# bioinfologics/w2rap-contigger

Measured on AMD Instinct MI355X. Metric: step2_k60_canonical_kmers_per_s, higher is better.
Workload: dtype u64

## Files before the change

### w2rap_contigger_amd/csrc/ctx.h

```cpp
#pragma once
#include <hip/hip_runtime.h>
#include <stdint.h>
#include <stdio.h>
#include <stdlib.h>
#include <cstdlib>
#include <string>
#include <utility>
#include <vector>
#include "../../include/w2rap_step2.h"
#include "common.h"

namespace w2 {

struct Ctx;
}
struct w2rap_step2_ctx;
namespace w2 {
struct Ctx {
    int device = 0;
    hipStream_t stream = nullptr;
    hipStream_t stream2 = nullptr;
    unsigned long long* h_pinned = nullptr;
    std::string err;
    int sm_count = 256;

    uint64_t n = 0;
    const uint8_t* d_bases = nullptr;
    const uint64_t* d_boff = nullptr;
    const uint32_t* d_len = nullptr;
    const uint8_t* d_quals = nullptr;
    const uint64_t* d_qoff = nullptr;
    uint32_t max_len = 0;
    std::vector<void*> owned_reads;

    uint16_t* d_good = nullptr;
    uint32_t min_qual = 7, min_freq = 4;

    uint64_t M = 0, D = 0, S = 0;
    uint64_t hist[101] = {0};
    uint32_t NB = 0;
    uint32_t* d_bcount = nullptr;
    unsigned long long part_kmers[64] = {0};
    uint64_t* d_bbase = nullptr;
    uint32_t* d_recs = nullptr;
    uint64_t nrec = 0;
    uint64_t solid_cap = 0;
    uint64_t* d_shi = nullptr;
    uint64_t* d_slo = nullptr;
    uint32_t* d_scc = nullptr;
    Slot* d_table = nullptr;
    uint64_t tcap = 0;
    unsigned long long* d_filter32 = nullptr;
    uint64_t f32words = 0;
    uint8_t* d_sctx = nullptr;
    void* d_nbr = nullptr;
    bool wide_ids = false;
    uint64_t* d_chunk_start = nullptr;
    uint32_t* d_chunk_cnt = nullptr;
    uint64_t nchunks = 0;
    KRec* d_srec = nullptr;
    bool use_index = false;
    uint4* d_index = nullptr;
    uint64_t index_cap = 0, index_entries = 0;
    uint4* d_xindex = nullptr; uint64_t xindex_cap = 0, xindex_kmers = 0;
    bool index_prebuilt = false, bits_ready = false, filter_prebuilt = false;
    unsigned cs_ns = 0;
    unsigned cs_planned = 0;
    uint32_t cs_nbl = 0, cs_nseg = 0; const uint32_t* cs_recs = nullptr;
    bool cs_short_first = false;
    hipEvent_t cs_ev[16] = {};
    unsigned long long* cs_cnt = nullptr;
    uint64_t* cs_off = nullptr;
    uint32_t cs_chunk_cap = 0;
    uint8_t* d_unres = nullptr;
    bool fused_prune = false;
    std::vector<std::pair<uint64_t, uint64_t>> unfused_chunks;
    uint32_t* cs_defer = nullptr;
    uint64_t* g_hi = nullptr; uint64_t* g_lo = nullptr; uint32_t* g_cc = nullptr;
    uint64_t* g_cstart = nullptr; uint32_t* g_ccnt = nullptr;
    uint64_t g_cap = 0, g_n = 0, g_ccap = 0, g_nc = 0;
    bool g_open = false;
    hipEvent_t g_copied = nullptr;
    bool quality_done = false, counted = false, graphed = false, pathed_done = false;
    bool table_built = false;

    uint64_t E = 0;
    uint64_t rank_ends = 0;
    uint32_t* d_edge_nk = nullptr;
    uint64_t* d_edge_off = nullptr;
    uint8_t* d_edge_codes = nullptr;
    uint8_t* d_edge_bits = nullptr;
    uint64_t edge_bases = 0;
    uint64_t NO = 0, NV = 0;
    int32_t* d_fwdX = nullptr;
    int32_t* d_revX = nullptr;
    uint32_t* d_obj_edge = nullptr;
    ObjRec* d_otab = nullptr;
    int32_t* d_left = nullptr;
    int32_t* d_right = nullptr;
    uint64_t* d_from_off = nullptr;
    int32_t* d_from_v = nullptr;
    int32_t* d_from_e = nullptr;
    uint64_t* d_to_off = nullptr;
    int32_t* d_to_v = nullptr;
    int32_t* d_to_e = nullptr;
    int32_t* d_path_offset = nullptr;
    uint64_t* d_path_off = nullptr;
    int32_t* d_path_edges = nullptr;
    uint64_t path_total = 0;
    uint64_t n_pathed = 0, n_multipathed = 0;
    float ms_count = 0, ms_graph = 0, ms_path = 0;

    uint64_t ld_done = 0;
    void* shard = nullptr;
    std::vector<void*> owned;
    void* pump = nullptr;
    const uint32_t* d_qmask = nullptr;
    int qmask_min_qual = -1;
    int hint_min_qual = -1;
    bool hint_graph_only = false;
    bool quals_absent = false;
    uint8_t* d_qring = nullptr;
    void* pump2 = nullptr;
    hipStream_t copy_stream = nullptr;
    void* quals_job = nullptr;
    void* mask_job = nullptr; void* h_mask = nullptr; size_t h_mask_bytes = 0;
    uint32_t n_passes = 0;
    unsigned pass = 0, npass = 1;
    unsigned long long* pass_cnt = nullptr;

    struct ProfEv { const char* name; hipEvent_t a, b; };
    struct ProfSum { std::string name; double ms = 0; uint64_t launches = 0; };
    std::vector<ProfEv> prof_pending;
    std::vector<ProfSum> prof_sums;
    bool profiling = true;
    void pbegin(const char* name, hipStream_t st = nullptr) {
        if (!profiling) return;
        ProfEv e{name, nullptr, nullptr};
        (void)hipEventCreate(&e.a); (void)hipEventCreate(&e.b);
        (void)hipEventRecord(e.a, st ? st : stream);
        prof_pending.push_back(e);
    }
    void pend(hipStream_t st = nullptr) {
        if (!profiling || prof_pending.empty()) return;
        (void)hipEventRecord(prof_pending.back().b, st ? st : stream);
    }
    void presolve() {
        for (auto& e : prof_pending) {
            float ms = 0;
            if (hipEventElapsedTime(&ms, e.a, e.b) == hipSuccess) {
                ProfSum* s = nullptr;
                for (auto& x : prof_sums) if (x.name == e.name) { s = &x; break; }
                if (!s) { prof_sums.push_back(ProfSum{e.name, 0, 0}); s = &prof_sums.back(); }
                s->ms += ms; s->launches += 1;
            }
            (void)hipEventDestroy(e.a); (void)hipEventDestroy(e.b);
        }
        prof_pending.clear();
    }

    std::vector<std::pair<size_t, void*>> parked;
    std::vector<std::pair<void*, size_t>> sizes;
    int mem_trace = -1; uint64_t traced_peak = 0;
    uint64_t live_bytes = 0, peak_bytes = 0;
    static size_t size_class(size_t bytes) {
        size_t g = 256;
        if (bytes < (256u << 20)) { while ((g << 5) <= bytes) g <<= 1; }
        else { g = 1u << 20; while ((g << 8) <= bytes) g <<= 1; }
        return (bytes + g - 1) & ~(g - 1);
    }
    void trim() {
        for (auto& b : parked) (void)hipFree(b.second);
        parked.clear();
    }
    template <class T>
    T* alloc(size_t count, bool track = true) {
        void* p = nullptr;
        size_t bytes = (count ? count : 1) * sizeof(T);
        bytes = size_class(bytes);
        for (size_t i = 0; i < parked.size(); ++i)
            if (parked[i].first == bytes) { p = parked[i].second; parked[i] = parked.back(); parked.pop_back(); break; }
        if (!p) {
            hipError_t e = hipMalloc(&p, bytes);
            if (e != hipSuccess) { (void)hipGetLastError(); trim(); e = hipMalloc(&p, bytes); }
            if (e != hipSuccess) { (void)hipGetLastError(); if (w2rap_step2_trim_cached() > 0) { (void)hipSetDevice(device); e = hipMalloc(&p, bytes); } }
            if (e != hipSuccess) {
                err = std::string("hipMalloc(") + std::to_string(bytes) + " B): " + hipGetErrorString(e);
                return nullptr;
            }
        }
        sizes.emplace_back(p, bytes);
        live_bytes += bytes;
        if (live_bytes > peak_bytes) {
            peak_bytes = live_bytes;
            if (mem_trace < 0) mem_trace = getenv("W2RAP_TRACE_MEM") ? 1 : 0;
            if (mem_trace && live_bytes > traced_peak + (1ull << 30)) {
                traced_peak = live_bytes;
                std::string l;
                for (auto& x : sizes) if (x.second >= (64u << 20)) l += " " + std::to_string(x.second >> 20);
                fprintf(stderr, "[w2rap] device memory: new peak %.2f GB live; blocks (MiB):%s\n", live_bytes / 1e9, l.c_str());
            }
        }
        if (track) owned.push_back(p);
        return (T*)p;
    }
    void park(void* p) {
        for (size_t i = 0; i < sizes.size(); ++i)
            if (sizes[i].first == p) { live_bytes -= sizes[i].second; parked.emplace_back(sizes[i].second, p); sizes[i] = sizes.back(); sizes.pop_back(); return; }
        (void)hipFree(p);
    }
    void release(void* p) {
        if (!p) return;
        for (size_t i = 0; i < owned.size(); ++i)
            if (owned[i] == p) { owned[i] = owned.back(); owned.pop_back(); break; }
        park(p);
    }
    void free_all() {
        for (void* p : owned) park(p);
        owned.clear();
    }

    struct Kept3 {
        bool valid = false;
        unsigned K2 = 0; uint64_t E = 0, NV = 0, n = 0, path_ints = 0, edge_bytes = 0;
        uint8_t* ebits = nullptr;
        uint64_t* ebyte = nullptr; uint32_t* elen = nullptr;
        int32_t* left = nullptr; int32_t* right = nullptr;
        uint64_t* from_off = nullptr; int32_t* from_v = nullptr; int32_t* from_e = nullptr;
        uint64_t* to_off = nullptr; int32_t* to_v = nullptr; int32_t* to_e = nullptr;
        int32_t* inv2 = nullptr;
        int32_t* p_offset = nullptr; uint64_t* p_off = nullptr; int32_t* p_edges = nullptr;
        std::vector<void*> blocks() const {
            return {ebits, ebyte, elen, left, right, from_off, from_v, from_e, to_off, to_v, to_e, inv2, p_offset, p_off, p_edges};
        }
    };
    Kept3 kept;
    void drop_kept() {
        if (!kept.valid) return;
        for (void* p : kept.blocks()) release(p);
        kept = Kept3{};
    }
};

inline bool test_hook(const char* name) {
    if (!getenv(name)) return false;
    fprintf(stderr, "[w2rap] WARNING: test hook %s is set -- this is not a production configuration\n", name);
    return true;
}

#define W2_HIP(call)                                                                         \
    do {                                                                                     \
        hipError_t e__ = (call);                                                             \
        if (e__ != hipSuccess) {                                                             \
            c.err = std::string(#call) + ": " + hipGetErrorString(e__) + " (" + __FILE__ + ":" + \
                    std::to_string(__LINE__) + ")";                                          \
            return W2RAP_E_HIP;                                                              \
        }                                                                                    \
    } while (0)
#define W2_ALLOC(ptr, T, count)                          \
    do {                                                 \
        ptr = c.alloc<T>(count);                         \
        if (!ptr) return W2RAP_E_HIP;                    \
    } while (0)
#define W2_TRY(expr)                   \
    do {                               \
        int rc__ = (expr);             \
        if (rc__) return rc__;         \
    } while (0)

#define LAUNCH(c, name, kern, grid, block, lds, ...)                          \
    do {                                                                      \
        (c).pbegin(name);                                                     \
        hipLaunchKernelGGL(kern, grid, block, lds, (c).stream, __VA_ARGS__);  \
        (c).pend();                                                           \
    } while (0)

struct Timer {
    hipEvent_t a = nullptr, b = nullptr; hipStream_t st;
    explicit Timer(hipStream_t s) : st(s) { (void)hipEventCreate(&a); (void)hipEventCreate(&b); (void)hipEventRecord(a, st); }
    float stop() { float ms = 0; (void)hipEventRecord(b, st); (void)hipEventSynchronize(b); (void)hipEventElapsedTime(&ms, a, b); return ms; }
    ~Timer() { (void)hipEventDestroy(a); (void)hipEventDestroy(b); }
    Timer(const Timer&) = delete; Timer& operator=(const Timer&) = delete;
};
void* host_result_alloc(size_t bytes);
template <class T>
inline int dl(Ctx& c, T** host, const T* dev, uint64_t n) {
    *host = (T*)host_result_alloc((n ? n : 1) * sizeof(T));
    if (!*host) { c.err = "out of host memory"; return W2RAP_E_HIP; }
    if (n * sizeof(T) >= (8u << 20)) return pump_download(c, *host, dev, n * sizeof(T));
    if (n) W2_HIP(hipMemcpyAsync(*host, dev, n * sizeof(T), hipMemcpyDeviceToHost, c.stream));
    return 0;
}
template <class T>
inline int up_pooled(Ctx& c, T** dev, const T* host, uint64_t n, uint64_t pad = 0) {
    T* p = c.alloc<T>(n + pad + 1);
    if (!p) return W2RAP_E_HIP;
    W2_HIP(hipMemsetAsync(p + n, 0, (pad + 1) * sizeof(T), c.stream));
    if (n && !host) { c.err = "null host array"; return W2RAP_E_ARG; }
    if (host) { if (n) W2_HIP(hipMemcpyAsync(p, host, n * sizeof(T), hipMemcpyHostToDevice, c.stream)); }
    else W2_HIP(hipMemsetAsync(p, 0, sizeof(T), c.stream));
    *dev = p;
    return 0;
}

#define LAUNCH_ON(c, st, name, kern, grid, block, lds, ...)                   \
    do {                                                                      \
        (c).pbegin(name, st);                                                 \
        hipLaunchKernelGGL(kern, grid, block, lds, st, __VA_ARGS__);          \
        (c).pend(st);                                                         \
    } while (0)

int device_copy_async(Ctx& c, void* dst, const void* src, uint64_t nbytes, hipStream_t st);
int pump_upload(Ctx& c, void* d, const void* h, size_t bytes);
int pump_download(Ctx& c, void* h, const void* d, size_t bytes);
void pump_free(Ctx& c);
int quality_mask_begin(Ctx& c, const uint8_t* h_quals, uint64_t nq, uint32_t min_qual);
int quality_mask_upload(Ctx& c, uint32_t* d_mask);
void quality_mask_cancel(Ctx& c);
int quals_upload_begin(Ctx& c, uint8_t* d_quals, const uint8_t* h_quals, uint64_t nq, uint64_t prefix_bytes, uint64_t prefix_reads);
int quals_wait_prefix(Ctx& c, uint64_t* reads_covered);
int quals_wait(Ctx& c);
}
#include <functional>
namespace w2 {
void host_parallel_for(size_t n, const std::function<void(size_t)>& f);

int phase_count(Ctx& c, uint32_t min_qual, uint32_t min_freq);
int count_quality(Ctx& c, uint32_t min_qual);
uint32_t default_buckets(uint64_t total_kmers, uint32_t multiple_of);
int count_partition(Ctx& c, uint32_t nb, uint32_t n_parts, uint32_t pb_lo, uint32_t pb_hi);
int count_buckets(Ctx& c, uint32_t min_freq, uint32_t nbl, uint32_t nseg, const uint32_t* d_recs, const uint32_t* d_counts, uint64_t total_kmers,
                  bool build_table = false);
int count_buckets_launch(Ctx& c, uint32_t min_freq, uint32_t nbl, uint32_t nseg, const uint32_t* d_recs, const uint32_t* d_counts, uint64_t total_kmers,
                         unsigned n_slices, bool deferred);
int count_buckets_launch_slice(Ctx& c, unsigned k);
void count_slice_bounds(const Ctx& c, unsigned k, uint32_t* b_lo, uint32_t* b_hi);
int count_buckets_slice(Ctx& c, unsigned k, uint64_t* n_solid, uint64_t* n_chunks);
int count_buckets_finish(Ctx& c);
int dict_begin(Ctx& c, uint64_t kmer_cap, uint64_t chunk_cap);
int dict_append(Ctx& c, const uint64_t* d_hi, const uint64_t* d_lo, const uint32_t* d_cc, uint64_t n, const uint64_t* d_cstart, const uint32_t* d_ccnt, uint64_t nc,
                uint64_t chunk_bias = 0);
int dict_end(Ctx& c);
void dict_abort(Ctx& c);
int count_table(Ctx& c);
int phase_graph(Ctx& c, const w2rap_edge_hint* hint);
int phase_path(Ctx& c);
int local_dict_slice(Ctx& c, uint64_t n_solid, uint64_t expected_total);
int shard_begin(Ctx& c, unsigned rank, unsigned world, const uint64_t* solid_per_rank, uint32_t n_buckets, uint32_t n_passes, const w2rap_edge_hint* hint);
int shard_next(Ctx& c, w2rap_xchg* x);
int shard_recv(Ctx& c, const uint64_t* recv_count, uint32_t elem_bytes, void** d_recv);
int shard_host_words(Ctx& c, const uint64_t* words);
int shard_info(Ctx& c, uint64_t out[8]);
void shard_free(Ctx& c);
int index_hard_slice(Ctx& c, const uint4* d_all, uint64_t n_all, unsigned rank, unsigned world, uint4** d_hard, uint64_t* n_hard);
int index_hard_apply(Ctx& c, const uint4* d_hard, uint64_t n_hard);
int index_harden(Ctx& c);
int build_index(Ctx& c);
int index_entries_slice(Ctx& c, unsigned rank, unsigned world, uint4** d_list, uint64_t* n_list);
int index_from_entries(Ctx& c, const uint4* d_all, uint64_t n_all, bool harden = true);
uint64_t filter32_words(const Ctx& c);
int filter32_slice(Ctx& c, unsigned rank, unsigned world, unsigned long long** d_slice, uint64_t* n_words);
EdgeIndex edge_index(const Ctx& c);
int index_probe_all(Ctx& c, int32_t* d_edge, uint32_t* d_off);
int run_ranking(Ctx& c, uint64_t N, const uint32_t* nxt0, uint32_t* nxt, uint32_t* rnk, unsigned long long* w, uint8_t* cyc, uint8_t* mid,
                uint32_t* d_flags, const uint64_t* shi, const uint64_t* slo, bool use_chunks);
int decode_pq(Ctx& c, const uint8_t* d_pq, const uint64_t* d_pqoff, uint8_t* d_quals, const uint64_t* d_qoff);

int sort_pairs_u64(Ctx& c, uint64_t* keys, uint32_t* vals, uint64_t n, int begin_bit, int end_bit);
int exclusive_scan_u32_to_u64(Ctx& c, const uint32_t* in, uint64_t* out, uint64_t n);
int exclusive_scan_packed_bytes(Ctx& c, const uint32_t* len, uint64_t* out, uint64_t n);
int exclusive_scan_u64(Ctx& c, const uint64_t* in, uint64_t* out, uint64_t n);
int exclusive_scan_is_self(Ctx& c, const uint32_t* a, uint64_t* out, uint64_t n);
int max_u32(Ctx& c, const uint32_t* in, uint64_t n, uint32_t* result);
int inclusive_max_scan_u32(Ctx& c, const uint32_t* in, uint32_t* out, uint64_t n);

}

struct w2rap_step2_ctx { w2::Ctx c; };
extern "C" w2rap_step2_ctx* w2rap_step2_acquire(int device, char* err, size_t errlen);
extern "C" void w2rap_step2_release(w2rap_step2_ctx*);
```

### w2rap_contigger_amd/csrc/step2_capi.hip

```cpp
#include <algorithm>
#include <chrono>
#include <cstdlib>
#include <cstring>
#include "ctx.h"

using namespace w2;


namespace {

void set_err(char* err, size_t errlen, const std::string& m) {
    if (err && errlen) { std::snprintf(err, errlen, "%s", m.c_str()); }
}


__global__ void __launch_bounds__(256) k_obj_len(uint64_t NO, const uint32_t* __restrict__ obj_edge, const uint32_t* __restrict__ edge_nk,
                                                  uint32_t* __restrict__ len, uint32_t* __restrict__ nbytes) {
    uint64_t o = (uint64_t)blockIdx.x * blockDim.x + threadIdx.x;
    if (o >= NO) return;
    uint32_t l = edge_nk[obj_edge[o] >> 1] + (K - 1);
    len[o] = l; nbytes[o] = (l + 3) >> 2;
}
__global__ void __launch_bounds__(256) k_pack_objs(uint64_t total_bytes, uint64_t NO, const uint64_t* __restrict__ byte_off,
                                                    const uint32_t* __restrict__ obj_edge, const uint32_t* __restrict__ edge_nk,
                                                    const uint64_t* __restrict__ edge_off, const uint8_t* __restrict__ codes,
                                                    uint8_t* __restrict__ out) {
    uint64_t i = (uint64_t)blockIdx.x * blockDim.x + threadIdx.x;
    if (i >= total_bytes) return;
    uint64_t lo = 0, hi = NO;
    while (hi - lo > 1) { uint64_t m = (lo + hi) >> 1; if (byte_off[m] <= i) lo = m; else hi = m; }
    uint32_t oe = obj_edge[lo], e = oe >> 1; bool rc = oe & 1;
    uint32_t len = edge_nk[e] + (K - 1);
    uint64_t eo = edge_off[e];
    uint32_t t0 = (uint32_t)(i - byte_off[lo]) * 4;
    unsigned v = 0;
    for (unsigned j = 0; j < 4; ++j) {
        uint32_t t = t0 + j;
        if (t < len) {
            unsigned b = rc ? 3u - codes[eo + (len - 1 - t)] : codes[eo + t];
            v |= b << (2 * j);
        }
    }
    out[i] = (uint8_t)v;
}


}
namespace w2 {
void drop_reads(Ctx& c) {
    (void)quals_wait(c);
    if (c.copy_stream) (void)hipStreamSynchronize(c.copy_stream);
    c.d_qmask = nullptr; c.qmask_min_qual = -1; c.quals_absent = false;
    for (void* p : c.owned_reads) c.park(p);
    c.owned_reads.clear();
    c.d_bases = nullptr; c.d_boff = nullptr; c.d_len = nullptr; c.d_quals = nullptr; c.d_qoff = nullptr; c.n = 0;
}
void drop_results(Ctx& c) {
    if (c.stream) (void)hipStreamSynchronize(c.stream);
    if (c.stream2) (void)hipStreamSynchronize(c.stream2);
    shard_free(c);
    c.drop_kept();
    c.free_all();
    c.d_good = nullptr; c.d_bcount = nullptr; c.d_bbase = nullptr; c.d_recs = nullptr; c.d_shi = c.d_slo = nullptr; c.d_scc = nullptr;
    c.d_table = nullptr; c.d_filter32 = nullptr; c.f32words = 0; c.d_sctx = nullptr; c.d_nbr = nullptr; c.d_srec = nullptr; c.d_index = nullptr; c.index_cap = 0; c.d_xindex = nullptr; c.xindex_cap = 0; c.d_unres = nullptr; c.fused_prune = false; c.unfused_chunks.clear();
    c.d_chunk_start = nullptr; c.d_chunk_cnt = nullptr; c.nchunks = 0;
    for (unsigned k = 0; k < c.cs_ns; ++k) (void)hipEventDestroy(c.cs_ev[k]);
    c.cs_ns = 0; c.cs_planned = 0; c.cs_cnt = nullptr; c.cs_off = nullptr; c.cs_defer = nullptr; c.pass = 0; c.npass = 1; c.pass_cnt = nullptr;
    c.g_hi = c.g_lo = nullptr; c.g_cc = nullptr; c.g_cstart = nullptr; c.g_ccnt = nullptr; c.g_open = false; c.g_n = c.g_nc = 0;
    c.d_edge_nk = nullptr; c.d_edge_off = nullptr; c.d_edge_codes = nullptr; c.d_edge_bits = nullptr; c.d_fwdX = c.d_revX = nullptr; c.d_obj_edge = nullptr;
    c.d_otab = nullptr; c.d_left = c.d_right = nullptr; c.d_from_off = c.d_to_off = nullptr; c.d_from_v = c.d_from_e = c.d_to_v = c.d_to_e = nullptr;
    c.d_path_offset = nullptr; c.d_path_off = nullptr; c.d_path_edges = nullptr;
    c.quality_done = c.counted = c.graphed = c.pathed_done = false; c.table_built = false;
    c.M = c.D = c.S = c.E = c.NO = c.NV = 0; c.path_total = 0; c.n_pathed = c.n_multipathed = 0;
}
}
namespace {

template <class T>
int up(Ctx& c, const T** dev, const T* host, uint64_t n, uint64_t pad = 0) {
    T* p = c.alloc<T>(n + pad + 1, false);
    if (!p) return W2RAP_E_HIP;
    c.owned_reads.push_back(p);
    W2_HIP(hipMemsetAsync(p + n, 0, (pad + 1) * sizeof(T), c.stream));
    if (n) W2_TRY(pump_upload(c, p, host, n * sizeof(T)));
    *dev = (const T*)p;
    return 0;
}

}

extern "C" {

int w2rap_step2_abi_version(void) { return W2RAP_STEP2_ABI_VERSION; }

int w2rap_step2_device_count(void) {
    int n = 0;
    if (hipGetDeviceCount(&n) != hipSuccess) return 0;
    return n;
}

w2rap_step2_ctx* w2rap_step2_create(int device, char* err, size_t errlen) {
    int n = 0;
    if (hipGetDeviceCount(&n) != hipSuccess || n <= 0) { set_err(err, errlen, "no HIP device (libw2rap_step2 has no CPU fallback)"); return nullptr; }
    if (device < 0 || device >= n) { set_err(err, errlen, "device ordinal out of range"); return nullptr; }
    hipDeviceProp_t prop;
    if (hipGetDeviceProperties(&prop, device) != hipSuccess) { set_err(err, errlen, "hipGetDeviceProperties failed"); return nullptr; }
    if (std::strncmp(prop.gcnArchName, "gfx950", 6) != 0) {
        set_err(err, errlen, std::string("device is ") + prop.gcnArchName + "; this library is built for gfx950 (MI355X) only");
        return nullptr;
    }
    if (hipSetDevice(device) != hipSuccess) { set_err(err, errlen, "hipSetDevice failed"); return nullptr; }
    auto* h = new w2rap_step2_ctx;
    h->c.device = device;
    h->c.sm_count = prop.multiProcessorCount;
    int prio_lo = 0, prio_hi = 0;
    (void)hipDeviceGetStreamPriorityRange(&prio_lo, &prio_hi);
    if (hipStreamCreateWithPriority(&h->c.stream, hipStreamNonBlocking, prio_hi) != hipSuccess ||
        hipStreamCreateWithPriority(&h->c.stream2, hipStreamNonBlocking, prio_lo) != hipSuccess ||
        hipHostMalloc((void**)&h->c.h_pinned, 64 * sizeof(unsigned long long), hipHostMallocDefault) != hipSuccess) {
        set_err(err, errlen, "hipStreamCreate / hipHostMalloc failed"); delete h; return nullptr;
    }
    return h;
}

void w2rap_step2_destroy(w2rap_step2_ctx* h) {
    if (!h) return;
    (void)hipSetDevice(h->c.device);
    (void)hipStreamSynchronize(h->c.stream);
    if (h->c.stream2) (void)hipStreamSynchronize(h->c.stream2);
    drop_results(h->c);
    drop_reads(h->c);
    h->c.trim();
    pump_free(h->c);
    (void)hipStreamDestroy(h->c.stream);
    if (h->c.g_copied) (void)hipEventDestroy(h->c.g_copied);
    if (h->c.stream2) (void)hipStreamDestroy(h->c.stream2);
    if (h->c.h_pinned) (void)hipHostFree(h->c.h_pinned);
    delete h;
}

const char* w2rap_step2_last_error(const w2rap_step2_ctx* h) { return h ? h->c.err.c_str() : "null context"; }
void* w2rap_step2_stream(w2rap_step2_ctx* h) { return h ? (void*)h->c.stream : nullptr; }

int w2rap_step2_set_reads(w2rap_step2_ctx* h, const w2rap_reads* r) {
    if (!h || !r) return W2RAP_E_ARG;
    Ctx& c = h->c;
    W2_HIP(hipSetDevice(c.device));
    drop_results(c);
    drop_reads(c);
    const uint64_t n = r->n_reads;
    if (n && (!r->bases_packed || !r->base_byte_off || !r->read_len)) { c.err = "set_reads: null base arrays"; return W2RAP_E_ARG; }
    const bool raw = r->quals && r->qual_off, pq = r->pq && r->pq_off;
    if (n && raw == pq) { c.err = "set_reads: give exactly one of (quals, qual_off) and (pq, pq_off)"; return W2RAP_E_ARG; }
    if (r->mem == W2RAP_MEM_DEVICE) {
        W2_HIP(hipDeviceSynchronize());
        c.d_bases = r->bases_packed; c.d_boff = r->base_byte_off; c.d_len = r->read_len;
        if (raw || !n) { c.d_quals = r->quals; c.d_qoff = r->qual_off; }
        else {
            uint64_t* qoff = nullptr; W2_HIP(hipMalloc((void**)&qoff, (n + 1) * 8)); c.owned_reads.push_back(qoff);
            W2_TRY(exclusive_scan_u32_to_u64(c, c.d_len, qoff, n));
            uint64_t total = 0;
            W2_HIP(hipMemcpy(&total, qoff + n, 8, hipMemcpyDeviceToHost));
            uint8_t* q = nullptr; W2_HIP(hipMalloc((void**)&q, total ? total : 1)); c.owned_reads.push_back(q);
            c.n = n;
            W2_TRY(decode_pq(c, r->pq, r->pq_off, q, qoff));
            c.d_quals = q; c.d_qoff = qoff;
        }
    } else if (r->mem == W2RAP_MEM_HOST) {
        {
            const size_t nblk = (size_t)std::min<uint64_t>(64, (n + 65535) / 65536);
            std::vector<uint64_t> bad(nblk ? nblk : 1, ~0ull); std::vector<int> why(nblk ? nblk : 1, 0);
            host_parallel_for(nblk, [&](size_t b) {
                const uint64_t lo = n * b / nblk, hi = n * (b + 1) / nblk;
                for (uint64_t i = lo; i < hi; ++i) {
                    const uint64_t nb = r->base_byte_off[i + 1] - r->base_byte_off[i];
                    int w = 0;
                    if (r->base_byte_off[i + 1] < r->base_byte_off[i] || nb != ((uint64_t)r->read_len[i] + 3) / 4) w = 1;
                    else if (raw && (r->qual_off[i + 1] < r->qual_off[i] || r->qual_off[i + 1] - r->qual_off[i] != r->read_len[i])) w = 2;
                    else if (!raw && r->pq_off[i + 1] <= r->pq_off[i]) w = 3;
                    else if (r->read_len[i] > 65535u) w = 4;
                    if (w) { bad[b] = i; why[b] = w; return; }
                }
            });
            for (size_t b = 0; b < nblk; ++b) if (bad[b] != ~0ull) {
                const std::string at = " (read " + std::to_string(bad[b]);
                if (why[b] == 4) { c.err = "a read of more than 65,535 bases" + at + "): good lengths are 16-bit words"; return W2RAP_E_LIMIT; }
                c.err = why[b] == 1 ? "set_reads: base_byte_off does not match read_len" + at + ")" : why[b] == 2 ? "set_reads: qual_off does not match read_len" + at + ")"
                                    : "set_reads: pq_off is not ascending" + at + "; every PQVec ends with a 0 byte)";
                return W2RAP_E_ARG;
            }
        }
        if (n && (r->base_byte_off[0] != 0 || (raw ? r->qual_off[0] : r->pq_off[0]) != 0)) { c.err = "set_reads: offsets must start at 0"; return W2RAP_E_ARG; }
        const uint64_t nbytes = n ? r->base_byte_off[n] : 0;
        auto derived = [&](const uint64_t** dev, bool packed) -> int {
            uint64_t* p = c.alloc<uint64_t>(n + 2, false);
            if (!p) return W2RAP_E_HIP;
            c.owned_reads.push_back(p);
            W2_TRY(packed ? exclusive_scan_packed_bytes(c, c.d_len, p, n) : exclusive_scan_u32_to_u64(c, c.d_len, p, n));
            *dev = p;
            return 0;
        };
        const uint64_t nq_raw = (raw && n) ? r->qual_off[n] : 0;
        const bool late_quals = raw && c.hint_min_qual >= 0 && nq_raw >= (64ull << 20) && !getenv("W2RAP_NO_UPLOAD_OVERLAP");
        if (late_quals) W2_TRY(quality_mask_begin(c, r->quals, nq_raw, (uint32_t)c.hint_min_qual));
        struct MaskGuard { Ctx& c; ~MaskGuard() { quality_mask_cancel(c); } } mask_guard{c};
        const bool tr = getenv("W2RAP_TRACE") != nullptr;
        auto tnow = [] { return std::chrono::duration<double, std::milli>(std::chrono::steady_clock::now().time_since_epoch()).count(); };
        const double t_a = tnow();
        W2_TRY(up(c, &c.d_len, r->read_len, n));
        W2_TRY(up(c, &c.d_bases, r->bases_packed, nbytes, 32));
        W2_TRY(derived(&c.d_boff, true));
        const double t_b = tnow();
        if (raw || !n) {
            const uint64_t nq = n ? r->qual_off[n] : 0;
            if (late_quals) {
                uint8_t* q = c.alloc<uint8_t>(nq + 33, false);
                uint32_t* m = c.alloc<uint32_t>((nq + 31) / 32 + 17, false);
                if (!q || !m) return W2RAP_E_HIP;
                c.owned_reads.push_back(q); c.owned_reads.push_back(m);
                W2_HIP(hipMemsetAsync(q + nq, 0, 33, c.stream));
// ... 608 lines not shown
```

### w2rap_contigger_amd/csrc/step2_count.hip

```cpp
#include <algorithm>
#include <chrono>
#include <cstdlib>
#include <cstring>
#include <type_traits>
#include "ctx.h"

namespace w2 {

constexpr unsigned QSLOTS = 256;
template <bool MASK>
__global__ void __launch_bounds__(256) k_good_len(uint64_t n, const uint8_t* __restrict__ quals, const uint32_t* __restrict__ qmask,
                                                   const uint64_t* __restrict__ qoff, const uint32_t* __restrict__ len,
                                                   uint32_t min_qual, uint16_t* __restrict__ good,
                                                   unsigned long long* __restrict__ total_kmers,
                                                   uint32_t* __restrict__ max_len) {
    constexpr unsigned CH = 4096;
    __shared__ __attribute__((aligned(16))) uint16_t gbits[CH + 16];
    __shared__ unsigned long long s_sum[4];
    __shared__ uint32_t s_max[4];
    const uint64_t r0 = (uint64_t)blockIdx.x * blockDim.x;
    const uint64_t r = r0 + threadIdx.x;
    const uint64_t rend = r0 + blockDim.x < n ? r0 + blockDim.x : n;
    const uint64_t base0 = qoff[r0], endo = qoff[rend];
    const unsigned shift = MASK ? (unsigned)(base0 & 31) : (unsigned)((reinterpret_cast<uintptr_t>(quals) + base0) & 15);
// ... 130 lines not shown
    __shared__ uint2 dbuf_[4][128];
    __shared__ uint32_t spart_[4][64];
    const unsigned lane = threadIdx.x & 63, wv_ = threadIdx.x >> 6;
    if (part_kmers) { spart_[wv_][lane] = 0; wave_lds_fence(); }
    uint2* dbuf = dbuf_[wv_];
    auto win_load = [&](uint64_t first_byte, unsigned nbytes) -> uint32_t {
        const uintptr_t a = reinterpret_cast<uintptr_t>(bases) + first_byte;
        const unsigned sb = (unsigned)(a & 3);
        return 4 * lane < sb + nbytes ? reinterpret_cast<const uint32_t*>(a & ~uintptr_t(3))[lane & 15u] : 0u;
    };
    const uint64_t stride = 1;
    uint64_t r = ((uint64_t)blockIdx.x * 4 + wv_) * chunk;
    const uint64_t r_end = r + chunk < n ? r + chunk : n;
    unsigned gl_c = 0, gl_n = 0; uint64_t off_c = 0, off_n = 0; uint32_t win_c = 0;
    if (r < r_end) { gl_c = good[r]; off_c = boff[r]; }
    if (r + stride < r_end) { gl_n = good[r + stride]; off_n = boff[r + stride]; }
    if (r < r_end && lane < 16 && gl_c > K) win_c = win_load(off_c, (gl_c + 3) >> 2);
    for (; r < r_end; r += stride) {
        const unsigned gl = gl_c;
        const uint64_t off_cur = off_c;
        const uint32_t win0 = win_c;
        unsigned gl_nn = 0; uint64_t off_nn = 0;
        if (r + 2 * stride < r_end) { gl_nn = good[r + 2 * stride]; off_nn = boff[r + 2 * stride]; }
        win_c = 0;
        if (r + stride < r_end && lane < 16 && gl_n > K) win_c = win_load(off_n, (gl_n + 3) >> 2);
        gl_c = gl_n; off_c = off_n; gl_n = gl_nn; off_n = off_nn;
        if (gl <= K) continue;
        const unsigned nk_total = gl - (K - 1);
        const unsigned nbytes_read = (gl + 3) >> 2;
        for (unsigned c0 = 0; c0 < nk_total; c0 += 128) {
            const unsigned first_base = c0 ? c0 - 1 : 0;
            const unsigned b0a = (first_base >> 2) & ~3u;
            uint32_t wdw = win0;
            if (c0) wdw = lane < 16 ? win_load(off_cur + b0a, nbytes_read - b0a) : 0u;
            const unsigned sbit = 8u * (unsigned)((reinterpret_cast<uintptr_t>(bases) + off_cur) & 3);
            const unsigned sbase = 4 * b0a;
            uint32_t k0, k1, k2;
            {
                uint32_t kk[3];
#pragma unroll
                for (int h = 0; h < 3; ++h) {
                    const unsigned j = c0 + h * 64 + lane;
                    uint32_t key = 0xFFFFFFFFu;
                    const bool has = j + MMER <= gl && (h < 2 || lane < WIN - 1);
                    const unsigned o = has ? sbit + 2 * (j - sbase) : 0u, wi = o >> 5, sh = o & 31;
                    const uint32_t w0 = (uint32_t)__builtin_amdgcn_ds_bpermute((int)(wi << 2), (int)wdw);
                    const uint32_t w1 = (uint32_t)__builtin_amdgcn_ds_bpermute((int)((wi + 1) << 2), (int)wdw);
                    if (has) {
                        const uint32_t f = __funnelshift_r(w0, w1, sh) & 0x3FFFFFFFu;
                        uint32_t rc = __brev(~f & 0x3FFFFFFFu);
                        rc = (((rc & 0x55555555u) << 1) | ((rc >> 1) & 0x55555555u)) >> 2;
                        key = mmer_key(f < rc ? f : rc);
                    }
                    kk[h] = key;
                }
                k0 = kk[0]; k1 = kk[1]; k2 = kk[2];
            }
            constexpr uint32_t INF = 0xFFFFFFFFu;
            auto row_pref = [](uint32_t x) {
                x = min(x, (uint32_t)__builtin_amdgcn_update_dpp((int)0xFFFFFFFFu, (int)x, 0x111, 0xF, 0xF, false));
                x = min(x, (uint32_t)__builtin_amdgcn_update_dpp((int)0xFFFFFFFFu, (int)x, 0x112, 0xF, 0xF, false));
                x = min(x, (uint32_t)__builtin_amdgcn_update_dpp((int)0xFFFFFFFFu, (int)x, 0x114, 0xF, 0xF, false));
                x = min(x, (uint32_t)__builtin_amdgcn_update_dpp((int)0xFFFFFFFFu, (int)x, 0x118, 0xF, 0xF, false));
                return x;
            };
            auto row_suff = [](uint32_t x) {
                x = min(x, (uint32_t)__builtin_amdgcn_update_dpp((int)0xFFFFFFFFu, (int)x, 0x101, 0xF, 0xF, false));
                x = min(x, (uint32_t)__builtin_amdgcn_update_dpp((int)0xFFFFFFFFu, (int)x, 0x102, 0xF, 0xF, false));
                x = min(x, (uint32_t)__builtin_amdgcn_update_dpp((int)0xFFFFFFFFu, (int)x, 0x104, 0xF, 0xF, false));
                x = min(x, (uint32_t)__builtin_amdgcn_update_dpp((int)0xFFFFFFFFu, (int)x, 0x108, 0xF, 0xF, false));
                return x;
            };
            const uint32_t P0 = row_pref(k0), P1 = row_pref(k1), P2 = row_pref(k2), S0 = row_suff(k0), S1 = row_suff(k1);
            uint32_t F[12];
#pragma unroll
            for (int R = 0; R < 4; ++R) {
                F[R] = (uint32_t)__builtin_amdgcn_readlane((int)P0, 16 * R + 15);
                F[4 + R] = (uint32_t)__builtin_amdgcn_readlane((int)P1, 16 * R + 15);
                F[8 + R] = (uint32_t)__builtin_amdgcn_readlane((int)P2, 16 * R + 15);
            }
            const unsigned rowi = lane >> 4;
            const bool two = (lane & 15u) >= 3;
            uint32_t mkh[2];
#pragma unroll
            for (int h = 0; h < 2; ++h) {
                const uint32_t g1a = F[4 * h + 1], g1b = F[4 * h + 2], g1c = F[4 * h + 3], g1d = F[4 * h + 4];
                const uint32_t g2a = min(g1a, F[4 * h + 2]), g2b = min(g1b, F[4 * h + 3]), g2c = min(g1c, F[4 * h + 4]), g2d = min(g1d, F[4 * h + 5]);
                const uint32_t one_row = rowi == 0 ? g1a : rowi == 1 ? g1b : rowi == 2 ? g1c : g1d;
                const uint32_t two_rows = rowi == 0 ? g2a : rowi == 1 ? g2b : rowi == 2 ? g2c : g2d;
                const uint32_t pend = h ? lane_shift(P1, P2, lane, WIN - 1) : lane_shift(P0, P1, lane, WIN - 1);
                mkh[h] = min(min(h ? S1 : S0, pend), two ? two_rows : one_row);
            }
            const uint32_t mk0 = mkh[0], mk1 = mkh[1];
            unsigned nkh[2] = {0, 0}; uint32_t bkh[2] = {0, 0}; bool sth[2] = {false, false};
#pragma unroll
            for (int h = 0; h < 2; ++h) {
                const unsigned cc0 = c0 + 64 * h;
                const unsigned p = cc0 + lane;
                const bool valid = p < nk_total;
                const uint32_t bkt = valid ? bucket_of(h ? mk1 : mk0, nb) : 0xFFFFFFFFu;
                const uint32_t prev = (uint32_t)__builtin_amdgcn_update_dpp(0, (int)bkt, 0x138, 0xF, 0xF, false);
                bool start = valid && (lane == 0 || prev != bkt);
                unsigned long long smask = __ballot(start);
                unsigned nvalid = cc0 < nk_total ? nk_total - cc0 : 0; if (nvalid > 64) nvalid = 64;
                if (REC_MAXK < 64 && smask == 1ull && nvalid == 64) { start |= lane == 63; smask |= 1ull << 63; }
                unsigned long long rest = lane < 63 ? (smask >> (lane + 1)) : 0ull;
                unsigned nxt = rest ? lane + 1 + __builtin_ctzll(rest) : nvalid;
                const bool mine = bkt - pb_lo < pb_hi - pb_lo;
                sth[h] = start && mine; bkh[h] = bkt - pb_lo; nkh[h] = start ? nxt - lane : 0;
            }
            unsigned cnt = 0;
            const uint64_t slot0 = (pass_off[r] + c0 / 128) * spp;
            uint32_t rk[2] = {0, 0};
#pragma unroll
            for (int h = 0; h < 2; ++h) {
                if (sth[h]) {
                    rk[h] = atomicAdd(&bcount[bkh[h]], 1u);
                    if (part_kmers) {
                        uint32_t pt = nbl_part > 1 ? __umulhi(bkh[h], inv_nbl) : bkh[h];
                        if ((pt + 1) * nbl_part <= bkh[h]) ++pt;
                        atomicAdd(&spart_[wv_][pt & 63], nkh[h]);
                    }
                }
            }
#pragma unroll
            for (int h = 0; h < 2; ++h) {
                const unsigned long long m = __ballot(sth[h]);
                if (sth[h]) {
                    const unsigned p = c0 + 64 * h + lane, nk = nkh[h];
                    const uint32_t meta = p | ((nk - 1) << 16) | (p > 0 ? 1u << 22 : 0u) | ((p + nk - 1) < (nk_total - 1) ? 1u << 23 : 0u);
                    const unsigned j = cnt + (unsigned)__builtin_popcountll(m & ((1ull << lane) - 1));
                    if (j < spp && rk[h] < 65536u) dbuf[j] = make_uint2(bkh[h] | (rk[h] << 24), meta | ((rk[h] >> 8) << 24));
                    else {
                        if (j < spp) dbuf[j] = make_uint2(0u, NONE32);
                        const unsigned long long o = atomicAdd(ov_cursor, 1ull);
                        if (o < ov_cap) { o_read[o] = (uint32_t)r; o_bkt[o] = bkh[h]; o_meta[o] = meta; o_rank[o] = rk[h]; }
                    }
                }
                cnt += (unsigned)__builtin_popcountll(m);
            }
            wave_lds_fence();
            for (unsigned i = lane; i < spp; i += 64) s_desc[slot0 + i] = i < cnt ? dbuf[i] : make_uint2(0u, NONE32);
            wave_lds_fence();
        }
    }
    if (part_kmers) {
        wave_lds_fence();
        const uint32_t v = spart_[wv_][lane];
        if (v) atomicAdd(&part_kmers[(blockIdx.x & 63u) * 64u + lane], (unsigned long long)v);
    }
}


template <unsigned SMAX, bool ALIGN64>
__global__ void __launch_bounds__(256, 4) k_superkmers_lane(uint64_t n, const uint8_t* __restrict__ bases, const uint64_t* __restrict__ boff,
                                                            const uint16_t* __restrict__ good, uint32_t nb, uint32_t pb_lo, uint32_t pb_hi,
                                                            uint32_t* __restrict__ bcount, uint32_t nbl_part, uint32_t inv_nbl,
                                                            unsigned long long* __restrict__ part_kmers, uint2* __restrict__ s_desc, uint32_t S,
                                                            uint32_t* __restrict__ o_read, uint32_t* __restrict__ o_bkt, uint32_t* __restrict__ o_meta,
                                                            uint32_t* __restrict__ o_rank, uint64_t ov_cap, unsigned long long* __restrict__ ov_cursor) {
    __shared__ uint2 stage_[4][64 * SMAX];
    __shared__ uint32_t spart_[4][64];
    const unsigned lane = threadIdx.x & 63, wv_ = threadIdx.x >> 6;
    const uint64_t r0 = ((uint64_t)blockIdx.x * 4 + wv_) * 64;
    if (r0 >= n) return;
    uint2* stage = stage_[wv_];
    if (part_kmers) spart_[wv_][lane] = 0;
    for (unsigned u = 0; u < S; ++u) stage[lane + 64 * u] = make_uint2(0u, NONE32);
    wave_lds_fence();
    constexpr uint32_t INF = 0xFFFFFFFFu;
    const uint64_t r = r0 + lane;
    unsigned gl = r < n ? good[r] : 0;
    if (gl <= K) gl = 0;
    const unsigned nk = gl ? gl - (K - 1) : 0;
    unsigned maxgl = gl;
#pragma unroll
    for (int d = 32; d; d >>= 1) maxgl = max(maxgl, (unsigned)__shfl_xor((int)maxgl, d));
    maxgl = (unsigned)__builtin_amdgcn_readfirstlane((int)maxgl);
    if (maxgl) {
        const uint64_t off = gl ? boff[r] : 0;
        const unsigned mis = (unsigned)((reinterpret_cast<uintptr_t>(bases) + off) & 3);
        const unsigned sb8 = 8u * mis;
        const uint32_t* q = reinterpret_cast<const uint32_t*>(bases + ((int64_t)off - (int64_t)mis));
        const unsigned ulast = gl ? (mis + ((gl + 3) >> 2) - 1) >> 2 : 0;
        uint32_t dA, dB, W; unsigned un = 3;
        { const uint32_t d0 = q[0]; dA = q[min(1u, ulast)]; dB = q[min(2u, ulast)]; W = __funnelshift_r(d0, dA, sb8); }
        uint32_t f = 0, rc = 0;
        auto roll = [&]() {
            const uint32_t b = W & 3u; W >>= 2;
            f = (f >> 2) | (b << 28);
            rc = ((rc << 2) & 0x3FFFFFFFu) | (b ^ 3u);
        };
#pragma unroll
        for (unsigned s = 0; s < MMER - 1; ++s) roll();
        uint32_t X3[16], X2[16], X1[16], C[16];
#pragma unroll
        for (int t = 0; t < 16; ++t) { X3[t] = INF; X2[t] = INF; X1[t] = INF; C[t] = INF; }
        uint32_t cur = 0;
        unsigned p0 = 0, jrec = 0;
        auto block = [&](auto first, unsigned jb) {
            constexpr int FIRST = decltype(first)::value;
            uint32_t pref = INF;
            const uint32_t w21 = min(X2[0], X1[0]);
            uint32_t bk[16];
#pragma unroll
            for (int i = 0; i < 16; ++i) {
                const unsigned s = jb + (MMER - 1) + i;
                if (i == 2) { W = __funnelshift_r(dA, dB, sb8); dA = dB; dB = q[min(un, ulast)]; ++un; }
                roll();
                const uint32_t key = s < gl ? mmer_key(f < rc ? f : rc) : INF;
                C[i] = key; pref = min(pref, key);
                bk[i] = 0;
                if (i >= FIRST) {
                    const uint32_t mk = i <= 12 ? min(min(X3[i <= 12 ? i + 3 : 0], w21), pref) : min(min(X2[i >= 13 ? i - 13 : 0], X1[0]), pref);
                    bk[i] = bucket_of(mk, nb);
                }
            }
#pragma unroll
            for (int i = FIRST; i < 16; ++i) {
                const unsigned p = jb + i - (WIN - 1);
                const bool isk = p < nk;
                const uint32_t bkt = bk[i];
                const bool brk = isk && (!p || bkt != cur || (ALIGN64 ? !(p & 63u) || (REC_MAXK < 64 && p - p0 == REC_MAXK) : p - p0 == REC_MAXK));
                if ((brk && p) || (p == nk && nk)) {
                    const uint32_t rb = cur - pb_lo;
                    if (rb < pb_hi - pb_lo) {
                        const uint32_t meta = p0 | ((p - p0 - 1) << 16) | (p0 ? 1u << 22 : 0u) | (isk ? 1u << 23 : 0u);
                        if (jrec < S) stage[lane * S + jrec] = make_uint2(rb, meta);
                        else {
                            const uint32_t rk = atomicAdd(&bcount[rb], 1u);
                            if (part_kmers) {
                                uint32_t pt = nbl_part > 1 ? __umulhi(rb, inv_nbl) : rb;
                                if ((pt + 1) * nbl_part <= rb) ++pt;
                                atomicAdd(&spart_[wv_][pt & 63], p - p0);
                            }
                            const unsigned long long o = atomicAdd(ov_cursor, 1ull);
                            if (o < ov_cap) { o_read[o] = (uint32_t)r; o_bkt[o] = rb; o_meta[o] = meta; o_rank[o] = rk; }
                        }
                        ++jrec;
                    }
                }
                if (brk) { p0 = p; cur = bkt; }
            }
#pragma unroll
            for (int t = 14; t >= 0; --t) C[t] = min(C[t], C[t + 1]);
#pragma unroll
            for (int t = 0; t < 16; ++t) { X3[t] = X2[t]; X2[t] = X1[t]; X1[t] = C[t]; }
        };
        block(std::integral_constant<int, 16>{}, 0);
        block(std::integral_constant<int, 16>{}, 16);
        block(std::integral_constant<int, 13>{}, 32);
        for (unsigned jb = 48; jb + (MMER - 1) <= maxgl; jb += 16) block(std::integral_constant<int, 0>{}, jb);
    }
    wave_lds_fence();
    const uint64_t nflat = (uint64_t)((n - r0 < 64 ? n - r0 : 64)) * S;
    for (unsigned u0 = 0; u0 < S; u0 += 8) {
        uint2 d[8]; uint32_t rk[8];
#pragma unroll
        for (unsigned k = 0; k < 8; ++k) {
            const unsigned i = lane + 64 * (u0 + k);
            d[k] = u0 + k < S ? stage[i] : make_uint2(0u, NONE32);
            rk[k] = 0;
            if (d[k].y != NONE32) {
                rk[k] = atomicAdd(&bcount[d[k].x], 1u);
                if (part_kmers) {
                    uint32_t pt = nbl_part > 1 ? __umulhi(d[k].x, inv_nbl) : d[k].x;
                    if ((pt + 1) * nbl_part <= d[k].x) ++pt;
                    atomicAdd(&spart_[wv_][pt & 63], ((d[k].y >> 16) & 63u) + 1u);
                }
            }
        }
#pragma unroll
        for (unsigned k = 0; k < 8; ++k) {
            const unsigned i = lane + 64 * (u0 + k);
            if (u0 + k < S && i < nflat) {
                uint2 out = make_uint2(0u, NONE32);
                if (d[k].y != NONE32) {
                    if (rk[k] < 65536u) out = make_uint2(d[k].x | (rk[k] << 24), d[k].y | ((rk[k] >> 8) << 24));
                    else {
                        const unsigned long long o = atomicAdd(ov_cursor, 1ull);
                        if (o < ov_cap) { o_read[o] = (uint32_t)(r0 + i / S); o_bkt[o] = d[k].x; o_meta[o] = d[k].y; o_rank[o] = rk[k]; }
                    }
                }
                s_desc[r0 * S + i] = out;
            }
        }
    }
    if (part_kmers) {
        wave_lds_fence();
        const uint32_t v = spart_[wv_][lane];
        if (v) atomicAdd(&part_kmers[(blockIdx.x & 63u) * 64u + lane], (unsigned long long)v);
    }
}

template <bool PASS_OFF>
__global__ void __launch_bounds__(256) k_scatter_records(uint64_t nslots, uint32_t slots_per_read, const uint64_t* __restrict__ pass_off, uint64_t nreads,
                                                          const uint2* __restrict__ s_desc,
                                                          uint64_t nov, const uint32_t* __restrict__ o_read,
                                                          const uint32_t* __restrict__ o_bkt, const uint32_t* __restrict__ o_meta,
                                                          const uint32_t* __restrict__ o_rank,
                                                          const uint8_t* __restrict__ bases,
                                                          const uint64_t* __restrict__ boff, uint64_t bases_bytes,
                                                          const uint64_t* __restrict__ bbase,
                                                          uint32_t* __restrict__ recs) {
    __shared__ __attribute__((aligned(16))) uint32_t s_rec[4][64 * REC_DWORDS];
    __shared__ uint64_t s_dst[4][64];
    const unsigned lane = threadIdx.x & 63, wv = threadIdx.x >> 6;
    const uint64_t i = (uint64_t)blockIdx.x * blockDim.x + threadIdx.x;
    uint32_t r = 0, b = 0, meta = NONE32, slot = 0;
    if (i < nslots) {
        const uint2 d = s_desc[i];
        if (d.y != NONE32) { meta = d.y & 0xFFFFFFu; b = d.x & 0xFFFFFFu; slot = (d.x >> 24) | ((d.y >> 24) << 8); }
        if (PASS_OFF) {
            const uint64_t ps = i / slots_per_read;
            uint64_t lo = 0, hi = nreads;
            while (hi - lo > 1) { const uint64_t mid = (lo + hi) >> 1; if (pass_off[mid] <= ps) lo = mid; else hi = mid; }
            r = (uint32_t)lo;
        } else r = (uint32_t)(i / slots_per_read);
    } else if (i - nslots < nov) { r = o_read[i - nslots]; b = o_bkt[i - nslots]; meta = o_meta[i - nslots]; slot = o_rank[i - nslots]; }
    const bool valid = meta != NONE32;
    uint64_t dst = ~0ull;
    uint32_t out[REC_DWORDS] = {};
    if (valid) {
        const uint64_t base = bbase[b];
        const unsigned p = meta & 0xFFFFu, nk = ((meta >> 16) & 63u) + 1u;
        const bool hasL = (meta >> 22) & 1u, hasR = (meta >> 23) & 1u;
        const uint64_t ro = boff[r];
        const unsigned q = p ? p - 1 : 0;
        const uint64_t byte0 = ro + ((2 * q) >> 3);
        const unsigned sh = (2 * q) & 7;
        uint64_t W[5];
#pragma unroll
        for (unsigned j = 0; j < 5; ++j) {
            const uint64_t a = byte0 + 8 * j;
            uint64_t w = 0;
            if (a + 8 <= bases_bytes) w = reinterpret_cast<const U64u*>(bases + a)->v;
            else for (unsigned t = 0; t < 8; ++t) if (a + t < bases_bytes) w |= (uint64_t)bases[a + t] << (8 * t);
            W[j] = w;
        }
        uint64_t O[4];
#pragma unroll
        for (unsigned j = 0; j < 4; ++j) O[j] = sh ? (W[j] >> sh) | (W[j + 1] << (64 - sh)) : W[j];
        if (!p) {
            O[3] = (O[3] << 2) | (O[2] >> 62); O[2] = (O[2] << 2) | (O[1] >> 62); O[1] = (O[1] << 2) | (O[0] >> 62); O[0] <<= 2;
        }
        unsigned nbits = 2 * (nk + 61);
        if (!hasR) nbits -= 2;
#pragma unroll
        for (unsigned j = 0; j < 4; ++j) {
            if (nbits <= 64 * j) O[j] = 0;
            else if (nbits < 64 * (j + 1)) O[j] &= (1ull << (nbits - 64 * j)) - 1;
        }
        const uint32_t hdr = (nk - 1) | (hasL ? 64u : 0u) | (hasR ? 128u : 0u);
        if constexpr (REC_HB == 8) {
            O[3] = (O[3] << 8) | (O[2] >> 56); O[2] = (O[2] << 8) | (O[1] >> 56); O[1] = (O[1] << 8) | (O[0] >> 56);
            O[0] = (O[0] << 8) | (uint64_t)hdr;
#pragma unroll
            for (unsigned j = 0; j < 4; ++j) { out[2 * j] = (uint32_t)O[j]; out[2 * j + 1] = (uint32_t)(O[j] >> 32); }
        } else {
            out[0] = hdr;
#pragma unroll
            for (unsigned j = 0; j < 4; ++j) { out[(1 + 2 * j) % REC_DWORDS] = (uint32_t)O[j]; out[(2 + 2 * j) % REC_DWORDS] = (uint32_t)(O[j] >> 32); }
        }
        dst = (base + slot) * REC_DWORDS;
    }
    if constexpr (REC_DWORDS == 8) {
        reinterpret_cast<uint4*>(s_rec[wv])[2 * lane] = make_uint4(out[0], out[1], out[2], out[3]);
        reinterpret_cast<uint4*>(s_rec[wv])[2 * lane + 1] = make_uint4(out[4], out[5], out[6], out[7]);
    } else {
#pragma unroll
        for (unsigned j = 0; j < REC_DWORDS; ++j) s_rec[wv][lane * REC_DWORDS + j] = out[j];
    }
    s_dst[wv][lane] = dst;
    wave_lds_fence();
    if constexpr (REC_DWORDS == 8) {
#pragma unroll
        for (unsigned j = 0; j < 2; ++j) {
            const unsigned idx = j * 64 + lane, rec = idx >> 1;
            const uint64_t d = s_dst[wv][rec];
            if (d != ~0ull) reinterpret_cast<uint4*>(recs + d)[idx & 1u] = reinterpret_cast<const uint4*>(s_rec[wv])[idx];
        }
    } else {
#pragma unroll
        for (unsigned j = 0; j < REC_DWORDS; ++j) {
            const unsigned idx = j * 64 + lane, rec = idx / REC_DWORDS, qd = idx - rec * REC_DWORDS;
            const uint64_t d = s_dst[wv][rec];
            if (d != ~0ull) recs[d + qd] = s_rec[wv][idx];
        }
    }
}

template <unsigned CAP, unsigned THREADS, bool PARK = true>
struct K3Cfg {
    static constexpr unsigned NW = THREADS / 64;
    static constexpr unsigned RPL = !PARK ? 16 : NW >= 16 ? 32 : 64;
    static constexpr unsigned TILE = NW * RPL;
    static constexpr unsigned NPF = (TILE * REC_DWORDS + THREADS - 1) / THREADS;
    static constexpr unsigned SC = CAP / 8;
    static constexpr unsigned QCAP = PARK ? 128 : 0;
    static constexpr unsigned MAXSEG = 64;
    static constexpr unsigned LIMIT = CAP - THREADS - 8;
    static constexpr unsigned PER = CAP / THREADS;
    static constexpr unsigned LDS = CAP * 16 + SC * 16 + 3 * MAXSEG * 8 + NW * QCAP * 16 +
                                    (CAP + SC + TILE * REC_DWORDS + 4 + 3 * TILE + NW + NW * QCAP + 3 * (MAXSEG + 1) + 4 + 104 + 16 + 40 + 2 + 128) * 4;
};
enum { K3_FILL = 0, K3_OVF, K3_DEPTH, K3_CNT, K3_NPREV, K3_BASELO, K3_BASEHI, K3_B2LO, K3_B2HI, K3_WIN = 11  };

__device__ inline uint32_t ld32(const uint32_t* p) { return __hip_atomic_load(p, __ATOMIC_RELAXED, __HIP_MEMORY_SCOPE_WORKGROUP); }
__device__ inline void st32(uint32_t* p, uint32_t v) { __hip_atomic_store(p, v, __ATOMIC_RELAXED, __HIP_MEMORY_SCOPE_WORKGROUP); }
__device__ inline uint64_t ld64(const uint64_t* p) { return __hip_atomic_load(p, __ATOMIC_RELAXED, __HIP_MEMORY_SCOPE_WORKGROUP); }
__device__ inline void st64(uint64_t* p, uint64_t v) { __hip_atomic_store(p, v, __ATOMIC_RELAXED, __HIP_MEMORY_SCOPE_WORKGROUP); }
__device__ inline uint32_t row_scan16(uint32_t x) {
    x += (uint32_t)__builtin_amdgcn_update_dpp(0, (int)x, 0x111, 0xF, 0xF, false);
    x += (uint32_t)__builtin_amdgcn_update_dpp(0, (int)x, 0x112, 0xF, 0xF, false);
    x += (uint32_t)__builtin_amdgcn_update_dpp(0, (int)x, 0x114, 0xF, 0xF, false);
    x += (uint32_t)__builtin_amdgcn_update_dpp(0, (int)x, 0x118, 0xF, 0xF, false);
    return x;
}
__device__ inline uint32_t half_scan32(uint32_t x) {
    x = row_scan16(x);
    x += (uint32_t)__builtin_amdgcn_update_dpp(0, (int)x, 0x142, 0xA, 0xF, false);
    return x;
}
__device__ inline uint32_t wave_scan64(uint32_t x) {
    x = half_scan32(x);
    x += (uint32_t)__builtin_amdgcn_update_dpp(0, (int)x, 0x143, 0xC, 0xF, false);
    return x;
}
typedef uint32_t u32x4 __attribute__((ext_vector_type(4)));
__device__ inline u32x4 lds_read_b128(const uint32_t* p) {
    u32x4 v;
    const uint32_t a = (uint32_t)(uintptr_t)p;
    asm volatile("ds_read_b128 %0, %1\n\ts_waitcnt lgkmcnt(0)" : "=&v"(v) : "v"(a) : "memory");
    return v;
}

template <unsigned CAP, unsigned THREADS, bool PROF = false, bool PARK = true, unsigned MINW = 1>
__global__ void __launch_bounds__(THREADS, MINW) k_count_buckets(uint32_t nb, uint32_t b_lo, uint32_t b_hi ,
                                                            uint32_t nseg, const uint64_t* __restrict__ roff,
                                                            const uint32_t* __restrict__ recs, uint32_t min_freq,
                                                            uint32_t* __restrict__ queue,
                                                            uint64_t* __restrict__ shi, uint64_t* __restrict__ slo,
                                                            uint32_t* __restrict__ scc, uint64_t solid_cap,
                                                            unsigned long long* __restrict__ counters ,
                                                            unsigned long long* __restrict__ ghist,
                                                            uint64_t* __restrict__ chunk_start, uint32_t* __restrict__ chunk_cnt, uint32_t chunk_cap,
                                                            const uint32_t* __restrict__ blist , uint32_t blist_cap) {
    constexpr unsigned long long SMASK = (1ull << 40) - 1;
    using C = K3Cfg<CAP, THREADS, PARK>;
    constexpr unsigned NW = C::NW, RPL = C::RPL, TILE = C::TILE, NPF = C::NPF, SC = C::SC, MAXSEG = C::MAXSEG, PER = C::PER, QCAP = C::QCAP;
    constexpr unsigned LOG_CAP = CAP == 4096 ? 12 : CAP == 2048 ? 11 : CAP == 1024 ? 10 : 13;
    static_assert((1u << LOG_CAP) == CAP, "CAP");
    constexpr uint64_t EMPTY = ~0ull;
    extern __shared__ __attribute__((aligned(16))) unsigned char smem[];
    uint64_t* keys = reinterpret_cast<uint64_t*>(smem);
    uint64_t* sthi = keys + 2 * CAP;
    uint64_t* stlo = sthi + SC;
    uint64_t* segbase = stlo + SC;
    uint64_t* qhi = segbase + 3 * MAXSEG + (threadIdx.x >> 6) * QCAP;
    uint64_t* qlo = qhi + NW * QCAP;
    uint32_t* cc = reinterpret_cast<uint32_t*>(segbase + 3 * MAXSEG + 2 * NW * QCAP);
    uint32_t* stcc = cc + CAP;
    uint32_t* tile = stcc + SC;
    uint32_t* bv32 = tile + TILE * REC_DWORDS + 4;
    uint32_t* Bw = bv32 + 2 * TILE;
    uint32_t* wtot = Bw + TILE;
    uint32_t* qmeta = wtot + NW + (threadIdx.x >> 6) * QCAP;
    uint32_t* segdpre = wtot + NW + NW * QCAP;
    uint32_t* bq = segdpre + 3 * (MAXSEG + 1);
    uint32_t* lhist = bq + 4;
    uint32_t* misc = lhist + 104;
    uint32_t* stk = misc + 16;
    uint64_t* dummy64 = reinterpret_cast<uint64_t*>((reinterpret_cast<uintptr_t>(stk + 40) + 7) & ~uintptr_t(7));
    const unsigned tid = threadIdx.x, lane = tid & 63, wv = tid >> 6;
    const uint32_t nlist = blist ? (blist[0] < blist_cap ? blist[0] : blist_cap) : 0u;
    auto ticket = [&](uint32_t t) -> uint32_t { return blist ? (t < nlist ? blist[2 + t] : NONE32) : (t < b_hi - b_lo ? b_lo + t : NONE32); };

    auto seg_load = [&](uint32_t bb, uint64_t& r0, uint32_t& cnt) {
        r0 = 0; cnt = 0;
        if (tid < nseg && bb < b_hi) {
            const uint64_t a = roff[(uint64_t)tid * nb + bb], e = roff[(uint64_t)tid * nb + bb + 1];
            r0 = a; cnt = (uint32_t)(e - a);
            if (e - a >= (1ull << 26)) { cnt = 0; counters[3] = 2; }
        }
    };
    auto seg_store = [&](unsigned q, uint64_t r0, uint32_t cnt) {
        uint32_t incl = cnt;
#pragma unroll
        for (int o = 1; o < 64; o <<= 1) { uint32_t v = __shfl_up(incl, o); if ((int)lane >= o) incl += v; }
        uint32_t tot = (uint32_t)__builtin_amdgcn_readlane((int)incl, 63);
        if (tot >= (1u << 26)) { tot = 0; incl = 0; cnt = 0; if (lane == 0) counters[3] = 2; }
        const uint32_t ex = incl - cnt;
        if (lane < nseg) { segdpre[q * (MAXSEG + 1) + lane] = ex * REC_DWORDS; segbase[q * MAXSEG + lane] = (r0 - ex) * REC_DWORDS; }
        if (lane == 0) segdpre[q * (MAXSEG + 1) + nseg] = tot * REC_DWORDS;
    };
    auto tile_load = [&](unsigned q, uint32_t t, uint32_t (&v)[NPF]) {
        const uint32_t* dp = segdpre + q * (MAXSEG + 1);
        const uint32_t dall = dp[nseg];
        const uint32_t d0 = t * (TILE * REC_DWORDS);
        const uint32_t dend = dall - d0 < TILE * REC_DWORDS ? dall : d0 + TILE * REC_DWORDS;
        constexpr unsigned NB_REG = 7;
        uint32_t bnd[NB_REG];
#pragma unroll
        for (unsigned i = 0; i < NB_REG; ++i) bnd[i] = (i + 1 < nseg && nseg <= NB_REG + 1) ? dp[i + 1] : 0xFFFFFFFFu;
#pragma unroll
        for (unsigned j = 0; j < NPF; ++j) {
            const uint32_t d = d0 + j * THREADS + tid;
            uint32_t x = 0;
            if (d0 < dall && d < dend) {
                unsigned s = 0;
                if (nseg <= NB_REG + 1) {
#pragma unroll
                    for (unsigned i = 0; i < NB_REG; ++i) s += d >= bnd[i] ? 1u : 0u;
                } else while (d >= dp[s + 1]) ++s;
                x = recs[segbase[q * MAXSEG + s] + d];
            }
            v[j] = x;
        }
    };
    auto tile_store = [&](const uint32_t (&v)[NPF]) {
#pragma unroll
        for (unsigned j = 0; j < NPF; ++j) { const unsigned i = j * THREADS + tid; if (i < TILE * REC_DWORDS) tile[i] = v[j]; }
    };

    for (unsigned i = tid; i < CAP; i += THREADS) { keys[2 * i] = EMPTY; keys[2 * i + 1] = EMPTY; cc[i] = 0; }
    for (unsigned i = tid; i < 104; i += THREADS) lhist[i] = 0;
    if (tid < 4) tile[TILE * REC_DWORDS + tid] = 0;
    if (tid < 16) misc[tid] = 0;
    if (tid == 0) { const uint32_t t0 = atomicAdd(queue, 3u); bq[0] = ticket(t0); bq[1] = ticket(t0 + 1); bq[2] = ticket(t0 + 2); bq[3] = NONE32; }
    __syncthreads();
    if (wv == 0) {
        uint64_t r0; uint32_t cnt;
        seg_load(bq[0], r0, cnt); seg_store(0, r0, cnt);
        seg_load(bq[1], r0, cnt); seg_store(1, r0, cnt);
    }
    __syncthreads();
    uint32_t pf[NPF];
    tile_load(0, 0, pf);
    unsigned long long pend_base = 0, my_distinct = 0;
    unsigned long long pt[6] = {0, 0, 0, 0, 0, 0}, tp = 0, ptmax = 0, wt[5] = {0, 0, 0, 0, 0}, wtp = 0, wcount = 0;
    auto wtick = [&](int ph) { if (PROF && wv == 0) { const unsigned long long now = __builtin_amdgcn_s_memtime(); if (ph >= 0) wt[ph] += now - wtp; wtp = now; } };
    auto tick = [&](int ph) { if (PROF) { const unsigned long long now = __builtin_amdgcn_s_memtime(); if (ph >= 0) pt[ph] += now - tp; tp = now; } };

    unsigned qn = 0;
    bool big = false;
    auto probe = [&](bool live, Kmer k, unsigned s, unsigned ctx) -> bool {
        bool isnew = false;
        if (live) {
            bool ok = false;
            int budget = 2 * (int)CAP;
            for (;;) {
                bool emp;
                for (;;) {
                    const uint64_t khi = ld64(&keys[2 * s]), klo = ld64(&keys[2 * s + 1]);
                    const bool same_hi = khi == k.hi;
                    emp = khi == EMPTY;
                    const bool hit = same_hi & (klo == k.lo), busy = same_hi & (klo == EMPTY);
                    --budget;
                    if (hit | emp | (budget <= 0)) break;
                    s = busy ? s : ((s + 1) & (CAP - 1));
                }
                if (budget <= 0) break;
                if (!emp) { ok = true; break; }
                const uint64_t old = atomicCAS(reinterpret_cast<unsigned long long*>(&keys[2 * s]), (unsigned long long)EMPTY,
                                               (unsigned long long)k.hi);
                if (old == EMPTY) { st64(&keys[2 * s + 1], k.lo); isnew = true; ok = true; break; }
            }
            if (ok) {
                if (!big || (ld32(&cc[s]) & 0xFFFFFFu) < 0xFFF000u) atomicAdd(&cc[s], 1u);
                atomicOr(&cc[s], ctx << 24);
            } else st32(&misc[K3_OVF], 1u);
        }
        return isnew;
    };
    auto drain = [&](unsigned cnt) -> unsigned {
        wave_lds_fence();
        bool isnew = false;
        if (PARK) {
            const bool live = lane < cnt;
            const unsigned e = live ? qn - cnt + lane : 0u;
            Kmer k{0, 0}; uint32_t meta = 0;
            if (live) { k = Kmer{qhi[e], qlo[e]}; meta = qmeta[e]; }
            isnew = probe(live, k, meta & 0xFFFFu, meta >> 16);
        }
        qn -= cnt;
        wave_lds_fence();
        return (unsigned)__builtin_popcountll(__ballot(isnew));
    };

    for (uint32_t it = 0;; ++it) {
        const uint32_t b = (uint32_t)__builtin_amdgcn_readfirstlane((int)ld32(&bq[it & 3]));
        if (b >= b_hi) break;
        const unsigned q = it % 3;
        tick(-1);
        const uint32_t nrec = (uint32_t)__builtin_amdgcn_readfirstlane((int)segdpre[q * (MAXSEG + 1) + nseg]) / REC_DWORDS;
        const uint32_t ntiles = (nrec + TILE - 1) / TILE;
        big = nrec >= (1u << 18);
        tile_store(pf);
        uint32_t la_b = 0;
        if (tid == 0) la_b = ticket(atomicAdd(queue, 1u));
        uint64_t la_r0 = 0; uint32_t la_cnt = 0;
        if (wv == 0) seg_load(ld32(&bq[(it + 2) & 3]), la_r0, la_cnt);
        tile_load((it + 1) % 3, 0, pf);
        if (tid == 0) { stk[0] = 0; stk[1] = 1; misc[K3_DEPTH] = 1; }
        bool first_pass = true;
        __syncthreads();
        tick(0);
        unsigned long long tp0 = 0; if (PROF) tp0 = __builtin_amdgcn_s_memtime();
        for (;;) {
            const unsigned sp = ld32(&misc[K3_DEPTH]) - 1;
            const uint32_t cls = stk[2 * sp], P = stk[2 * sp + 1];
            for (uint32_t t = 0; t < ntiles; ++t) {
                if (t > 0 || (!first_pass && ntiles > 1)) {
                    uint32_t tmp[NPF];
                    tile_load(q, t, tmp);
                    __syncthreads();
                    tile_store(tmp);
                    __syncthreads();
                }
                const unsigned nrec_tile = nrec - t * TILE < TILE ? nrec - t * TILE : TILE;
                const unsigned myrec = wv * RPL + lane;
                const unsigned nk = (lane < RPL && myrec < nrec_tile) ? (tile[myrec * REC_DWORDS] & 63u) + 1u : 0u;
                const unsigned incl = RPL == 32 ? half_scan32(nk) : wave_scan64(nk);
                if (lane == RPL - 1) wtot[wv] = incl;
                for (unsigned i = tid; i < 2 * TILE; i += THREADS) bv32[i] = 0;
                if (tid == 0) misc[K3_WIN] = 2 * NW;
                __syncthreads();
                const unsigned wsum = lane < NW ? wtot[lane] : 0u, wsc = row_scan16(wsum);
                const int wvu = __builtin_amdgcn_readfirstlane((int)wv);
                const unsigned base = (unsigned)__builtin_amdgcn_readlane((int)wsc, wvu) - (unsigned)__builtin_amdgcn_readlane((int)wsum, wvu);
                const unsigned total = (unsigned)__builtin_amdgcn_readlane((int)wsc, NW - 1);
                if (nk) {
                    const unsigned e = base + incl - nk;
                    atomicOr(&bv32[e >> 5], 1u << (e & 31));
// ... 133 lines not shown
                const unsigned i = j * THREADS + tid;
                const uint32_t v = cc[i];
                const bool occ = (v & 0xFFFFFFu) != 0;
                uint32_t cnt = v & 0xFFFFFFu; if (cnt > 255) cnt = 255;
                const unsigned long long m1 = __ballot(occ && cnt == 1);
                if (m1 && lane == (unsigned)__builtin_ctzll(m1)) atomicAdd(&lhist[1], (uint32_t)__builtin_popcountll(m1));
                if (occ && cnt != 1) atomicAdd(&lhist[cnt > 100 ? 100 : cnt], 1u);
                if (occ) ++my_distinct;
                const bool solid = occ && cnt >= min_freq;
                if (occ) { cc[i] = 0; }
                if (occ && !solid) { keys[2 * i] = EMPTY; keys[2 * i + 1] = EMPTY; }
                vals[j] = solid ? (cnt | ((v >> 24) << 8) | 0x80000000u) : 0u;
                sm[j] = __ballot(solid);
                nsolid += (unsigned)__builtin_popcountll(sm[j]);
            }
            uint32_t wbase = 0;
            if (nsolid && lane == 0) wbase = atomicAdd(&misc[K3_CNT], nsolid);
            wbase = (uint32_t)__builtin_amdgcn_readfirstlane((int)wbase);
            tick(3);
            __syncthreads();
            tick(4);
            const uint32_t tot = ld32(&misc[K3_CNT]);
            if (tot <= SC) {
                if (tid == 0) {
                    misc[K3_NPREV] = tot; misc[K3_FILL] = 0; misc[K3_DEPTH] = sp;
                    pend_base = tot ? atomicAdd(&counters[0], (1ull << 40) | tot) : 0ull;
                }
                unsigned run = wbase;
#pragma unroll
                for (unsigned j = 0; j < PER; ++j) {
                    if (vals[j] >> 31) {
                        const unsigned i = j * THREADS + tid;
                        const unsigned pos = run + (unsigned)__builtin_popcountll(sm[j] & ((1ull << lane) - 1));
                        sthi[pos] = keys[2 * i]; stlo[pos] = keys[2 * i + 1]; stcc[pos] = vals[j] & 0xFFFFu;
                        keys[2 * i] = EMPTY; keys[2 * i + 1] = EMPTY;
                    }
                    run += (unsigned)__builtin_popcountll(sm[j]);
                }
            } else {
                if (tid == 0) {
                    const unsigned long long pk = atomicAdd(&counters[0], (1ull << 40) | tot), base = pk & SMASK;
                    if (chunk_start && (pk >> 40) < chunk_cap) { chunk_start[pk >> 40] = base; chunk_cnt[pk >> 40] = tot; }
                    misc[K3_B2LO] = (uint32_t)base; misc[K3_B2HI] = (uint32_t)(base >> 32);
                    misc[K3_NPREV] = 0; misc[K3_FILL] = 0; misc[K3_DEPTH] = sp; pend_base = 0;
                }
                __syncthreads();
                const unsigned long long gb = (unsigned long long)misc[K3_B2LO] | ((unsigned long long)misc[K3_B2HI] << 32);
                unsigned run = wbase;
#pragma unroll
                for (unsigned j = 0; j < PER; ++j) {
                    if (vals[j] >> 31) {
                        const unsigned i = j * THREADS + tid;
                        const unsigned long long pos = gb + run + (unsigned)__builtin_popcountll(sm[j] & ((1ull << lane) - 1));
                        if (pos < solid_cap) { shi[pos] = keys[2 * i]; slo[pos] = keys[2 * i + 1]; scc[pos] = vals[j] & 0xFFFFu; }
                        keys[2 * i] = EMPTY; keys[2 * i + 1] = EMPTY;
                    }
                    run += (unsigned)__builtin_popcountll(sm[j]);
                }
            }
            tick(5);
            if (sp == 0) break;
            __syncthreads();
        }
    }
    __syncthreads();
    if (tid == 0) { misc[K3_BASELO] = (uint32_t)pend_base; misc[K3_BASEHI] = (uint32_t)(pend_base >> 32); }
    __syncthreads();
    {
        const uint32_t nprev = misc[K3_NPREV];
        const unsigned long long pk = (unsigned long long)misc[K3_BASELO] | ((unsigned long long)misc[K3_BASEHI] << 32);
        const unsigned long long gb = pk & SMASK;
        for (unsigned i = tid; i < nprev; i += THREADS)
            if (gb + i < solid_cap) { shi[gb + i] = sthi[i]; slo[gb + i] = stlo[i]; scc[gb + i] = stcc[i]; }
        if (tid == 0 && nprev && chunk_start && (pk >> 40) < chunk_cap) { chunk_start[pk >> 40] = gb; chunk_cnt[pk >> 40] = nprev; }
    }
    for (unsigned i = tid; i < 101; i += THREADS) if (lhist[i]) atomicAdd(&ghist[i], (unsigned long long)lhist[i]);
    for (int o = 32; o > 0; o >>= 1) my_distinct += __shfl_down(my_distinct, o);
    if (lane == 0 && my_distinct) atomicAdd(&counters[1], my_distinct);
    if (PROF && tid == 0) { for (int i = 0; i < 6; ++i) atomicAdd(&counters[106 + i], pt[i]); atomicAdd(&counters[112], ptmax);
                            for (int i = 0; i < 5; ++i) atomicAdd(&counters[113 + i], wt[i]); }
    if (PROF && lane == 0) atomicAdd(&counters[124 + wv], wcount);
}

#ifdef W2RAP_FP_TS9
constexpr unsigned FP_TS = REC_DWORDS | 1u;
#else
constexpr unsigned FP_TS = REC_DWORDS;
#endif
__device__ inline unsigned fp_tile_index(unsigned d) { return FP_TS == REC_DWORDS ? d : d + d / REC_DWORDS; }
template <unsigned THREADS, unsigned TILE_, unsigned SC_>
struct FpCfg {
    static constexpr unsigned CAP = 4096, LOG_CAP = 12, NW = THREADS / 64;
    static constexpr unsigned TILE = TILE_;
    static constexpr unsigned ROUNDS = (TILE + THREADS - 1) / THREADS;
    static constexpr unsigned MAXK = 16384, MAXWIN = MAXK / 64;
    static constexpr unsigned PFREC = TILE < 512 ? TILE : 512;
    static constexpr unsigned NPF = (PFREC * REC_DWORDS + THREADS - 1) / THREADS;
    static constexpr unsigned SC = SC_;
    static constexpr unsigned QCAP = 128;
    static constexpr unsigned MAXSEG = 16;
    static constexpr unsigned LIMIT = CAP - THREADS - 8 < 3072 ? CAP - THREADS - 8 : 3072;
    static constexpr unsigned PER = CAP / THREADS;
    static constexpr unsigned OCAP = CAP;
    static constexpr unsigned LDS = 3 * MAXSEG * 8 +
                                    (2 * CAP + TILE * FP_TS + 8 + MAXK / 32 + 2 + MAXWIN + 2 + 2 * SC + NW * QCAP + 3 * (MAXSEG + 1) + 32 + 4 + 104 + 16 + 40 + (OCAP + 1) / 2) * 4;
    static_assert(TILE < 1023 && ROUNDS * NW <= 16 && (1u << LOG_CAP) == CAP, "FpCfg");
};
enum { FP_FILL = 0, FP_OVF, FP_CNT, FP_BASELO, FP_BASEHI, FP_WIN, FP_DEPTH };
#ifndef W2RAP_FP_TICKETS
#define W2RAP_FP_TICKETS 4
#endif
constexpr uint32_t FP_TICKETS = W2RAP_FP_TICKETS;
static_assert((FP_TICKETS & (FP_TICKETS - 1)) == 0, "FP_TICKETS");

struct FpInst {
    uint32_t s[4];
    uint32_t e0, e3;
};
__device__ inline FpInst fp_fetch(const uint32_t* tile, unsigned rec, unsigned idx) {
    const uint32_t* wp = tile + rec * FP_TS;
    const unsigned q0 = (idx + REC_HB / 2) >> 4, sh = ((idx + REC_HB / 2) & 15u) * 2u;
    const uint32_t d0 = wp[q0], d1 = wp[1 + q0], d2 = wp[2 + q0], d3 = wp[3 + q0], d4 = wp[4 + q0];
    FpInst x;
    const uint32_t e0 = __funnelshift_r(d0, d1, sh), e1 = __funnelshift_r(d1, d2, sh), e2 = __funnelshift_r(d2, d3, sh), e3 = __funnelshift_r(d3, d4, sh);
    x.s[0] = __funnelshift_r(e0, e1, 2); x.s[1] = (e1 >> 2) & 0x0FFFFFFFu;
    x.s[2] = __funnelshift_r(e1, e2, 30); x.s[3] = __funnelshift_r(e2, e3, 30) & 0x0FFFFFFFu;
    x.e0 = e0; x.e3 = e3;
    return x;
}
struct FpKey { uint64_t hi, lo; bool rc; uint32_t f[4]; };
__device__ inline FpKey fp_key(const FpInst& x) {
    auto rev2_32 = [](uint32_t v) { v = __brev(v); return ((v & 0x55555555u) << 1) | ((v >> 1) & 0x55555555u); };
    const uint32_t a0 = rev2_32(x.s[0]), b0 = rev2_32(x.s[1]), a1 = rev2_32(x.s[2]), b1 = rev2_32(x.s[3]);
    FpKey k;
    k.f[0] = a0 >> 4; k.f[1] = __funnelshift_r(b0, a0, 4); k.f[2] = a1 >> 4; k.f[3] = __funnelshift_r(b1, a1, 4);
    const uint64_t khi_f = ((uint64_t)k.f[0] << 32) | k.f[1], klo_f = ((uint64_t)k.f[2] << 32) | k.f[3];
    const uint64_t khi_r = ((uint64_t)(~x.s[3] & 0x0FFFFFFFu) << 32) | (uint32_t)~x.s[2], klo_r = ((uint64_t)(~x.s[1] & 0x0FFFFFFFu) << 32) | (uint32_t)~x.s[0];
    k.rc = khi_r != khi_f ? khi_r < khi_f : klo_r < klo_f;
    k.hi = k.rc ? khi_r : khi_f; k.lo = k.rc ? klo_r : klo_f;
    return k;
}
__device__ inline uint32_t fp_hash(const FpKey& k) {
    const uint32_t fa = (uint32_t)k.hi ^ (uint32_t)(k.lo >> 32), fb = (uint32_t)(k.hi >> 32) ^ (uint32_t)k.lo;
    return (fa + ((fb << 16) | (fb >> 16))) * 0x9E3779B1u;
}
__device__ inline bool fp_same(const uint32_t* tile, unsigned ref, const FpInst& x, const FpKey& k) {
    const FpInst r = fp_fetch(tile, ref >> 6, ref & 63u);
    const uint32_t same = (r.s[0] ^ x.s[0]) | (r.s[1] ^ x.s[1]) | (r.s[2] ^ x.s[2]) | (r.s[3] ^ x.s[3]);
    const uint32_t opp = ((r.s[3] ^ k.f[0]) | 0xF0000000u) & (r.s[2] ^ k.f[1]) & ((r.s[1] ^ k.f[2]) | 0xF0000000u) & (r.s[0] ^ k.f[3]);
    return same == 0u || opp == 0xFFFFFFFFu;
}

template <unsigned THREADS, unsigned MINW, unsigned TILE_, unsigned SC_>
__global__ void __launch_bounds__(THREADS, MINW) k_count_fp(uint32_t nb, uint32_t b_lo, uint32_t b_hi, uint32_t nseg, const uint64_t* __restrict__ roff,
                                                            const uint32_t* __restrict__ recs, uint32_t min_freq, uint32_t* __restrict__ queue,
                                                            uint64_t* __restrict__ shi, uint64_t* __restrict__ slo, uint32_t* __restrict__ scc, uint64_t solid_cap,
                                                            unsigned long long* __restrict__ counters, unsigned long long* __restrict__ ghist,
                                                            uint64_t* __restrict__ chunk_start, uint32_t* __restrict__ chunk_cnt, uint32_t chunk_cap,
                                                            uint32_t* __restrict__ defer , uint32_t defer_cap,
                                                            uint32_t fill_limit , uint32_t solid_limit ,
                                                            uint8_t* __restrict__ sctx, uint8_t* __restrict__ unres, uint32_t* __restrict__ nbr ) {
    constexpr unsigned long long SMASK = (1ull << 40) - 1;
    using C = FpCfg<THREADS, TILE_, SC_>;
    constexpr unsigned CAP = C::CAP, NW = C::NW, TILE = C::TILE, ROUNDS = C::ROUNDS, NPF = C::NPF, SC = C::SC, MAXSEG = C::MAXSEG, PER = C::PER, QCAP = C::QCAP,
                       MAXK = C::MAXK, MAXWIN = C::MAXWIN;
    constexpr uint32_t EMPTY = 0xFFFFFFFFu;
    extern __shared__ __attribute__((aligned(16))) unsigned char smem[];
    uint64_t* segbase = reinterpret_cast<uint64_t*>(smem);
    uint32_t* tab = reinterpret_cast<uint32_t*>(segbase + 3 * MAXSEG);
    uint32_t* cc = tab + CAP;
    uint32_t* tile = cc + CAP;
    uint32_t* bv32 = tile + TILE * FP_TS + 8;
    uint32_t* Bw = bv32 + MAXK / 32 + 2;
    uint32_t* stcc = Bw + MAXWIN + 2;
    uint32_t* stref = stcc + SC;
    uint32_t* qref = stref + SC + (threadIdx.x >> 6) * QCAP;
    uint32_t* segdpre = stref + SC + NW * QCAP;
    uint32_t* wtot = segdpre + 3 * (MAXSEG + 1);
    uint32_t* bq = wtot + 32;
    uint32_t* lhist = bq + 4;
    uint32_t* misc = lhist + 104;
    uint32_t* stk = misc + 16;
    uint16_t* olist = reinterpret_cast<uint16_t*>(stk + 40);
    const unsigned tid = threadIdx.x, lane = tid & 63, wv = tid >> 6;

    auto seg_load = [&](uint32_t bb, uint64_t& r0, uint32_t& cnt) {
        r0 = 0; cnt = 0;
        if (tid < nseg && bb < b_hi) {
            const uint64_t a = roff[(uint64_t)tid * nb + bb], e = roff[(uint64_t)tid * nb + bb + 1];
            r0 = a; cnt = e - a < (1ull << 20) ? (uint32_t)(e - a) : (1u << 20);
        }
    };
    auto seg_store = [&](unsigned q, uint64_t r0, uint32_t cnt) {
        uint32_t incl = cnt;
#pragma unroll
        for (int o = 1; o < 64; o <<= 1) { uint32_t v = __shfl_up(incl, o); if ((int)lane >= o) incl += v; }
        const uint32_t tot = (uint32_t)__builtin_amdgcn_readlane((int)incl, 63);
        const uint32_t ex = incl - cnt;
        if (lane < nseg) { segdpre[q * (MAXSEG + 1) + lane] = ex * REC_DWORDS; segbase[q * MAXSEG + lane] = (r0 - ex) * REC_DWORDS; }
        if (lane == 0) segdpre[q * (MAXSEG + 1) + nseg] = tot * REC_DWORDS;
    };
    auto stream_dword = [&](unsigned q, const uint32_t* dp, const uint32_t (&bnd)[7], uint32_t d) -> uint32_t {
        unsigned s = 0;
        if (nseg <= 8) {
#pragma unroll
            for (unsigned i = 0; i < 7; ++i) s += d >= bnd[i] ? 1u : 0u;
        } else while (d >= dp[s + 1]) ++s;
        return recs[segbase[q * MAXSEG + s] + d];
    };
    auto tile_load = [&](unsigned q, uint32_t (&v)[NPF]) {
        const uint32_t* dp = segdpre + q * (MAXSEG + 1);
        const uint32_t dall = dp[nseg];
        const uint32_t dend = dall < C::PFREC * REC_DWORDS ? dall : C::PFREC * REC_DWORDS;
        uint32_t bnd[7];
#pragma unroll
        for (unsigned i = 0; i < 7; ++i) bnd[i] = (i + 1 < nseg && nseg <= 8) ? dp[i + 1] : 0xFFFFFFFFu;
#pragma unroll
        for (unsigned j = 0; j < NPF; ++j) {
            const uint32_t d = j * THREADS + tid;
            v[j] = d < dend ? stream_dword(q, dp, bnd, d) : 0u;
        }
    };
    auto tile_store = [&](const uint32_t (&v)[NPF]) {
#pragma unroll
        for (unsigned j = 0; j < NPF; ++j) { const unsigned i = j * THREADS + tid; if (i < C::PFREC * REC_DWORDS) tile[fp_tile_index(i)] = v[j]; }
    };
    auto tile_rest = [&](unsigned q) {
        if (TILE <= C::PFREC) return;
        const uint32_t* dp = segdpre + q * (MAXSEG + 1);
        const uint32_t dall = dp[nseg];
        const uint32_t dend = dall < TILE * REC_DWORDS ? dall : TILE * REC_DWORDS;
        uint32_t bnd[7];
#pragma unroll
        for (unsigned i = 0; i < 7; ++i) bnd[i] = (i + 1 < nseg && nseg <= 8) ? dp[i + 1] : 0xFFFFFFFFu;
        for (uint32_t d = C::PFREC * REC_DWORDS + tid; d < dend; d += THREADS) tile[fp_tile_index(d)] = stream_dword(q, dp, bnd, d);
    };
    auto ctx_of = [&](const FpInst& x, bool rc, uint32_t hdr, unsigned idx) -> unsigned {
        const unsigned rnk_ = (hdr & 63u) + 1u;
        const bool hasp = (idx > 0) | ((hdr & 64u) != 0), hass = (idx + 1 < rnk_) | ((hdr & 128u) != 0);
        const unsigned shl_p = (x.e0 & 3u) ^ (rc ? 3u : 4u), shl_s = ((x.e3 >> 26) & 3u) ^ (rc ? 7u : 0u);
        return (hasp ? 1u << shl_p : 0u) | (hass ? 1u << shl_s : 0u);
    };

    for (unsigned i = tid; i < CAP; i += THREADS) { tab[i] = EMPTY; cc[i] = 0; }
    for (unsigned i = tid; i < MAXK / 32 + 2; i += THREADS) bv32[i] = 0;
    for (unsigned i = tid; i < TILE * FP_TS + 8; i += THREADS) tile[i] = 0;
    for (unsigned i = tid; i < 104; i += THREADS) lhist[i] = 0;
    if (tid < 16) misc[tid] = 0;
    if (tid == 0) {
        const uint32_t t0 = atomicAdd(queue, 3u), nbk = b_hi - b_lo;
        bq[0] = t0 < nbk ? b_lo + t0 : NONE32; bq[1] = t0 + 1 < nbk ? b_lo + t0 + 1 : NONE32; bq[2] = t0 + 2 < nbk ? b_lo + t0 + 2 : NONE32; bq[3] = NONE32;
    }
    __syncthreads();
    if (wv == 0) {
        uint64_t r0; uint32_t cnt;
        seg_load(bq[0], r0, cnt); seg_store(0, r0, cnt);
        seg_load(bq[1], r0, cnt); seg_store(1, r0, cnt);
    }
    __syncthreads();
    uint32_t pf[NPF];
    tile_load(0, pf);
    unsigned long long my_distinct = 0;
    unsigned qn = 0;
    uint32_t tick4 = 0;

    auto drain = [&](unsigned cnt) -> unsigned {
        wave_lds_fence();
        const bool live = lane < cnt;
        const unsigned ref = live ? qref[qn - cnt + lane] : 0u;
        const unsigned rec = ref >> 6, idx = ref & 63u;
        const FpInst x = fp_fetch(tile, rec, idx);
        const FpKey k = fp_key(x);
        const unsigned ctx = ctx_of(x, k.rc, tile[rec * FP_TS], idx);
        const uint32_t h1 = fp_hash(k), tag = (h1 >> 5) & 0xFFFFu;
        unsigned s = (h1 >> (33 - C::LOG_CAP)) << 1;
        bool isnew = false;
        if (live) {
            bool ok = false;
            int budget = (int)CAP;
            for (;;) {
                uint32_t a = ld32(&tab[s]);
                if (a == EMPTY) {
                    a = atomicCAS(&tab[s], EMPTY, (tag << 16) | ref);
                    if (a == EMPTY) { isnew = true; ok = true; break; }
                }
                if ((a >> 16) == tag && fp_same(tile, a & 0xFFFFu, x, k)) { ok = true; break; }
                s = (s + 1) & (CAP - 1);
                if (--budget <= 0) break;
            }
            if (ok) { atomicAdd(&cc[s], 1u); atomicOr(&cc[s], ctx << 24); }
            else st32(&misc[FP_OVF], 1u);
        }
        qn -= cnt;
        wave_lds_fence();
        return (unsigned)__builtin_popcountll(__ballot(isnew));
    };

    for (uint32_t it = 0;; ++it) {
        const uint32_t b = (uint32_t)__builtin_amdgcn_readfirstlane((int)ld32(&bq[it & 3]));
        if (b >= b_hi) break;
        const unsigned q = it % 3;
        const uint32_t nrec = (uint32_t)__builtin_amdgcn_readfirstlane((int)segdpre[q * (MAXSEG + 1) + nseg]) / REC_DWORDS;
        bool skip = nrec > TILE;
        tile_store(pf);
        if (!skip) tile_rest(q);
        uint32_t la_b = 0;
        if (tid == 0) {
            if ((it & (FP_TICKETS - 1u)) == 0) tick4 = atomicAdd(queue, FP_TICKETS);
            const uint32_t t = tick4 + (it & (FP_TICKETS - 1u));
            la_b = t < b_hi - b_lo ? b_lo + t : NONE32;
        }
        uint64_t la_r0 = 0; uint32_t la_cnt = 0;
        if (wv == 0) seg_load(ld32(&bq[(it + 2) & 3]), la_r0, la_cnt);
        tile_load((it + 1) % 3, pf);
        __syncthreads();
        unsigned nkr[ROUNDS], inclr[ROUNDS];
#pragma unroll
        for (unsigned r = 0; r < ROUNDS; ++r) {
            const unsigned rec = r * THREADS + tid;
            nkr[r] = (!skip && rec < nrec) ? (tile[rec * FP_TS] & 63u) + 1u : 0u;
            inclr[r] = wave_scan64(nkr[r]);
            if (lane == 63) wtot[r * NW + wv] = inclr[r];
        }
        if (tid == 0) { misc[FP_WIN] = 2 * NW; stk[0] = 0; stk[1] = 1; misc[FP_DEPTH] = 1; }
        __syncthreads();
        const unsigned wsum = lane < ROUNDS * NW ? wtot[lane] : 0u, wsc = row_scan16(wsum);
        const int wvu = __builtin_amdgcn_readfirstlane((int)wv);
        const unsigned total = (unsigned)__builtin_amdgcn_readlane((int)wsc, ROUNDS * NW - 1);
        skip |= total > MAXK;
#pragma unroll
        for (unsigned r = 0; r < ROUNDS; ++r) {
            const unsigned base = (unsigned)__builtin_amdgcn_readlane((int)wsc, r * NW + wvu) - (unsigned)__builtin_amdgcn_readlane((int)wsum, r * NW + wvu);
            if (nkr[r] && !skip) {
                const unsigned e = base + inclr[r] - nkr[r], rec = r * THREADS + tid;
                atomicOr(&bv32[e >> 5], 1u << (e & 31));
                const unsigned w1 = (e + 63) >> 6;
                if (64 * w1 < e + nkr[r]) Bw[w1] = (rec << 16) | e;
            }
        }
        __syncthreads();
        const unsigned nwin = skip ? 0u : (total + 63) / 64;
        bool first_pass = true;
// ... 226 lines not shown
    uint64_t s = h & mask;
    while (atomicCAS(&table[s], SLOT_EMPTY, v) != SLOT_EMPTY) s = (s + 1) & mask;
}

template <unsigned U> struct PlCfg { static constexpr unsigned CAP = 256 * U, SLOTS = 512 * U, BITS = U == 2 ? 10 : U == 4 ? 11 : 12; };
template <unsigned BITS>
__device__ inline unsigned pl_hash(Kmer k) {
    const uint32_t fa = (uint32_t)k.hi ^ (uint32_t)(k.lo >> 32), fb = (uint32_t)(k.hi >> 32) ^ (uint32_t)k.lo;
    return ((fa + ((fb << 16) | (fb >> 16))) * 0x9E3779B1u) >> (32 - BITS);
}
template <class Id, unsigned U = 2>
__global__ void __launch_bounds__(256) k_prune_local(uint64_t nchunks, const uint64_t* __restrict__ cstart, const uint32_t* __restrict__ ccnt,
                                                      const uint64_t* __restrict__ shi, const uint64_t* __restrict__ slo,
                                                      const uint32_t* __restrict__ scc, uint8_t* __restrict__ sctx,
                                                      Id* __restrict__ nbr, uint8_t* __restrict__ unres) {
    constexpr Id NONE = NodeId<Id>::NONE, PAL = NodeId<Id>::PAL;
    constexpr unsigned PL_CAP = PlCfg<U>::CAP, PL_SLOTS = PlCfg<U>::SLOTS, PL_BITS = PlCfg<U>::BITS;
    __shared__ uint64_t khi[PL_SLOTS], klo[PL_SLOTS];
    __shared__ uint16_t kix[PL_SLOTS];
    const unsigned tid = threadIdx.x;
    auto load_desc = [&](uint64_t ch, uint64_t& st_, uint32_t& cn_) {
        st_ = 0; cn_ = 0;
        if (ch < nchunks) { st_ = cstart[ch]; cn_ = ccnt[ch]; if (cn_ > PL_CAP) cn_ = 0; }
    };
    auto load_keys = [&](uint64_t st_, uint32_t cn_, Kmer (&k_)[U], unsigned (&c_)[U]) {
#pragma unroll
        for (unsigned u = 0; u < U; ++u) {
            const unsigned j = tid + 256 * u;
            k_[u] = Kmer{0, 0}; c_[u] = 0;
            if (j < cn_) { k_[u] = Kmer{shi[st_ + j], slo[st_ + j]}; c_[u] = (scc[st_ + j] >> 8) & 0xFF; }
        }
    };
    uint64_t st_c, st_n; uint32_t cn_c, cn_n;
    Kmer nx[U]; unsigned ncx[U];
    load_desc(blockIdx.x, st_c, cn_c);
    load_keys(st_c, cn_c, nx, ncx);
    load_desc((uint64_t)blockIdx.x + gridDim.x, st_n, cn_n);
    for (uint64_t ch = blockIdx.x; ch < nchunks; ch += gridDim.x) {
        const uint64_t start = st_c;
        const uint32_t cnt = cn_c;
        Kmer mine[U]; unsigned cm[U];
#pragma unroll
        for (unsigned u = 0; u < U; ++u) { mine[u] = nx[u]; cm[u] = ncx[u]; }
        st_c = st_n; cn_c = cn_n;
        load_keys(st_c, cn_c, nx, ncx);
        load_desc(ch + 2 * (uint64_t)gridDim.x, st_n, cn_n);
        if (cnt == 0) continue;
        __syncthreads();
        for (unsigned s = tid; s < PL_SLOTS; s += 256) khi[s] = EMPTY_HI;
        __syncthreads();
#pragma unroll
        for (unsigned u = 0; u < U; ++u) {
            const unsigned j = tid + 256 * u;
            if (j < cnt) {
                unsigned s = pl_hash<PL_BITS>(mine[u]);
                for (;;) {
                    const unsigned long long old = atomicCAS(reinterpret_cast<unsigned long long*>(&khi[s]), (unsigned long long)EMPTY_HI,
                                                             (unsigned long long)mine[u].hi);
                    if (old == EMPTY_HI) { klo[s] = mine[u].lo; kix[s] = (uint16_t)j; break; }
                    s = (s + 1) & (PL_SLOTS - 1);
                }
            }
        }
        __syncthreads();
        auto find = [&](Kmer nk) -> int {
            unsigned s = pl_hash<PL_BITS>(nk);
            for (;;) {
                const uint64_t h = khi[s];
                if (h == EMPTY_HI) return -1;
                if (h == nk.hi && klo[s] == nk.lo) return (int)kix[s];
                s = (s + 1) & (PL_SLOTS - 1);
            }
        };
#pragma unroll
        for (unsigned u = 0; u < U; ++u) {
            if (256 * u + (tid & ~63u) >= cnt) continue;
            const unsigned j = tid + 256 * u;
            const Kmer k = mine[u];
            const unsigned c = j < cnt ? cm[u] : 0;
            unsigned un = 0;
            Id ns = NONE, np = NONE;
            const Kmer rk = kmer_rc(k);
            for (unsigned rest = c; __any(rest != 0);) {
                if (rest) {
                    const unsigned t = (unsigned)__builtin_ctz(rest);
                    rest &= rest - 1;
                    const unsigned b = t & 3;
                    const Kmer fw = t < 4 ? kmer_succ(k, b) : kmer_pred(k, b);
                    const Kmer rv = t < 4 ? kmer_pred(rk, 3u - b) : kmer_succ(rk, 3u - b);
                    const bool r = kmer_lt(rv, fw);
                    const Kmer nk = r ? rv : fw;
                    const int f = find(nk);
                    if (f < 0) un |= 1u << t;
                    else {
                        const Id id = kmer_eq(rv, fw) ? PAL : (Id)(2 * (start + (unsigned)f) + (r ? 1u : 0u));
                        if (t < 4) ns = id; else np = id;
                    }
                }
            }
            if (j < cnt) {
                const uint64_t i = start + j;
                sctx[i] = (uint8_t)c; unres[i] = (uint8_t)un;
                nbr[2 * i] = (!(un & 15u) && popc4(c & 15) != 1) ? NONE : ns;
                nbr[2 * i + 1] = (!(un >> 4) && popc4(c >> 4) != 1) ? NONE : np;
            }
        }
    }
}
#define PL_LAUNCH(c, IdT, gl, S_, nch_, ...)                                                                                          \
    do {                                                                                                                              \
        unsigned u__ = (nch_) ? ((S_) / (nch_) > 600 ? 8u : (S_) / (nch_) > 300 ? 4u : 2u) : 2u;                                       \
        if (const char* v__ = getenv("W2RAP_PL_U")) { const int x__ = atoi(v__); if (x__ == 2 || x__ == 4 || x__ == 8) u__ = (unsigned)x__; }  \
        if (u__ == 8) LAUNCH(c, "k_prune_local", (k_prune_local<IdT, 8>), dim3(gl), dim3(256), 0, nch_, __VA_ARGS__);                  \
        else if (u__ == 4) LAUNCH(c, "k_prune_local", (k_prune_local<IdT, 4>), dim3(gl), dim3(256), 0, nch_, __VA_ARGS__);             \
        else LAUNCH(c, "k_prune_local", (k_prune_local<IdT, 2>), dim3(gl), dim3(256), 0, nch_, __VA_ARGS__);                           \
    } while (0)
template <class Id>
__global__ void __launch_bounds__(256) k_prune(uint64_t i0, uint64_t S , const uint64_t* __restrict__ shi, const uint64_t* __restrict__ slo,
                                                const uint32_t* __restrict__ scc, const Slot* __restrict__ table, uint64_t mask,
                                                uint8_t* __restrict__ sctx, Id* __restrict__ nbr, const uint8_t* __restrict__ unres) {
    constexpr Id NONE = NodeId<Id>::NONE, PAL = NodeId<Id>::PAL;
    uint64_t i = i0 + (uint64_t)blockIdx.x * blockDim.x + threadIdx.x;
    if (i >= S) return;
    unsigned c, todo;
    Id ns = NONE, np = NONE;
    if (unres) {
        todo = unres[i];
        if (!todo) return;
        if (todo == 0xFFu && sctx[i] == 0xFFu) { c = (scc[i] >> 8) & 0xFF; todo = c; }
        else { c = sctx[i]; ns = nbr[2 * i]; np = nbr[2 * i + 1]; }
    } else { c = (scc[i] >> 8) & 0xFF; todo = c; }
    const Kmer k{shi[i], slo[i]}, rk = kmer_rc(k);
    for (unsigned rest = todo; rest;) {
        const unsigned t = (unsigned)__builtin_ctz(rest);
        rest &= rest - 1;
        const unsigned b = t & 3;
        const Kmer fw = t < 4 ? kmer_succ(k, b) : kmer_pred(k, b);
        const Kmer rv = t < 4 ? kmer_pred(rk, 3u - b) : kmer_succ(rk, 3u - b);
        const bool r = kmer_lt(rv, fw);
        const Kmer nk = r ? rv : fw;
        const int64_t s = table_find(table, mask, shi, slo, nk);
        if (s < 0) c &= ~(1u << t);
        else {
            const Id id = kmer_eq(rv, fw) ? PAL : (Id)(2 * (uint64_t)s + (r ? 1u : 0u));
            if (t < 4) ns = id; else np = id;
        }
    }
    sctx[i] = (uint8_t)c;
    nbr[2 * i] = popc4(c & 15) == 1 ? ns : NONE;
    nbr[2 * i + 1] = popc4(c >> 4) == 1 ? np : NONE;
}

static constexpr unsigned COUNT_CAP = 4096, COUNT_THREADS = 1024;
static constexpr unsigned KMERS_PER_BUCKET = 4500;

int count_quality(Ctx& c, uint32_t min_qual) {
    c.min_qual = min_qual;
    c.counted = false;
    hipStream_t st = c.stream;
    const uint64_t n = c.n;
    if (c.d_good) c.release(c.d_good);
    W2_ALLOC(c.d_good, uint16_t, n);
    unsigned long long* d_cnt = nullptr;
    W2_ALLOC(d_cnt, unsigned long long, 2 * QSLOTS);
    W2_HIP(hipMemsetAsync(d_cnt, 0, 2 * QSLOTS * sizeof(unsigned long long), st));
    const bool masked = c.d_qmask && c.qmask_min_qual == (int)std::min<uint32_t>(min_qual, 255u);
    if (!masked && c.quals_absent) { c.err = "quality windows: the reads were installed by a graph-only call for another min_qual, their raw qualities were not uploaded"; return W2RAP_E_STATE; }
    if (!masked) W2_TRY(quals_wait(c));
    if (n) {
        if (masked) LAUNCH(c, "k_good_len", k_good_len<true>, dim3((unsigned)((n + 255) / 256)), dim3(256), 0, n, c.d_quals, c.d_qmask, c.d_qoff, c.d_len, min_qual,
                           c.d_good, d_cnt, reinterpret_cast<uint32_t*>(d_cnt + QSLOTS));
        else LAUNCH(c, "k_good_len", k_good_len<false>, dim3((unsigned)((n + 255) / 256)), dim3(256), 0, n, c.d_quals, (const uint32_t*)nullptr, c.d_qoff, c.d_len, min_qual,
                    c.d_good, d_cnt, reinterpret_cast<uint32_t*>(d_cnt + QSLOTS));
        W2_HIP(hipGetLastError());
    }
    unsigned long long h_cnt[2 * QSLOTS];
    W2_HIP(hipMemcpyAsync(h_cnt, d_cnt, sizeof(h_cnt), hipMemcpyDeviceToHost, st));
    W2_HIP(hipStreamSynchronize(st));
    c.M = 0; c.max_len = 0;
    for (unsigned i = 0; i < QSLOTS; ++i) {
        c.M += h_cnt[i];
        const uint32_t* mx = reinterpret_cast<const uint32_t*>(h_cnt + QSLOTS);
        c.max_len = std::max(c.max_len, mx[i]);
    }
    c.release(d_cnt);
    if (c.max_len > 65535u) { c.err = "a read of more than 65,535 bases: good lengths are 16-bit words"; return W2RAP_E_LIMIT; }
    c.quality_done = true;
    return 0;
}

uint32_t default_buckets(uint64_t total_kmers, uint32_t multiple_of) {
    const char* v = getenv("W2RAP_KPB");
    uint64_t kpb = v ? (uint64_t)atoll(v) : KMERS_PER_BUCKET;
    uint64_t nb64 = total_kmers / kpb + 1;
    if (nb64 > (1u << 24)) nb64 = 1u << 24;
    if (multiple_of > 1) nb64 = (nb64 + multiple_of - 1) / multiple_of * multiple_of;
    return (uint32_t)nb64;
}

static uint32_t k1_chunk_reads() {
    const char* v = getenv("W2RAP_K1_CHUNK");
    const int x = v ? atoi(v) : 16;
    return x > 0 ? (uint32_t)x : 16;
}


static bool k1_wave(uint32_t spp, uint32_t npass) {
    const char* k1v = getenv("W2RAP_K1");
    return (k1v && !strcmp(k1v, "wave")) || spp * npass > 16;
}

__global__ void __launch_bounds__(256) k_k1_passes(uint64_t n, const uint16_t* __restrict__ good, uint32_t* __restrict__ np) {
    const uint64_t r = (uint64_t)blockIdx.x * blockDim.x + threadIdx.x;
    if (r >= n) return;
    const uint32_t g = good[r];
    np[r] = g > K ? (g - (K - 1) + 127) / 128 : 0;
}

static int k1_pass_offsets(Ctx& c, uint64_t nr, const uint16_t* good, uint64_t* pass_off, uint64_t* total) {
    *total = 0;
    if (!nr) return 0;
    uint32_t* np = nullptr;
    W2_ALLOC(np, uint32_t, nr);
    LAUNCH(c, "k_k1_passes", k_k1_passes, dim3((unsigned)((nr + 255) / 256)), dim3(256), 0, nr, good, np);
    W2_HIP(hipGetLastError());
    W2_TRY(exclusive_scan_u32_to_u64(c, np, pass_off, nr));
    W2_HIP(hipMemcpyAsync(total, pass_off + nr, 8, hipMemcpyDeviceToHost, c.stream));
    W2_HIP(hipStreamSynchronize(c.stream));
    c.release(np);
    return 0;
}

static int launch_k1(Ctx& c, uint64_t nr, const uint64_t* boff, const uint16_t* good, uint32_t pb_lo, uint32_t pb_hi, uint32_t* bcount,
                     uint32_t nbl_part, uint32_t inv_nbl, unsigned long long* d_part, uint2* s_desc, uint32_t spp, uint32_t npass,
                     const uint64_t* pass_off ,
                     uint32_t* o_read, uint32_t* o_bkt, uint32_t* o_meta, uint32_t* o_rank, uint64_t ov_cap, unsigned long long* d_ov_cur) {
    if (getenv("W2RAP_TRACE"))
        fprintf(stderr, "[w2rap] K1 route: %s, npass %u, spp %u, %llu reads, longest %u\n", k1_wave(spp, npass) ? "wave" : "lane",
                npass, spp, (unsigned long long)nr, c.max_len);
    if (!k1_wave(spp, npass)) {
        const bool a64 = getenv("W2RAP_K1_ALIGN64") != nullptr;
        const dim3 grid((unsigned)((nr + 255) / 256));
#define W2_K1L(A64) LAUNCH(c, "k_superkmers_lane", (k_superkmers_lane<16, A64>), grid, dim3(256), 0, nr, c.d_bases, boff, good, c.NB, pb_lo, pb_hi, bcount, \
                           nbl_part, inv_nbl, d_part, s_desc, spp * npass, o_read, o_bkt, o_meta, o_rank, ov_cap, d_ov_cur)
        if (a64) W2_K1L(true); else W2_K1L(false);
#undef W2_K1L
        W2_HIP(hipGetLastError());
        return 0;
    }
    const uint32_t k1_chunk = k1_chunk_reads();
    const unsigned grid = (unsigned)((nr + 4ull * k1_chunk - 1) / (4ull * k1_chunk) + 1);
    static const int k1_minw = getenv("W2RAP_K1_MINW") ? atoi(getenv("W2RAP_K1_MINW")) : 8;
    if (k1_minw == 6)
        LAUNCH(c, "k_superkmers", k_superkmers<6>, dim3(grid), dim3(256), 0, nr, k1_chunk, c.d_bases, boff, good, c.NB, pb_lo, pb_hi, bcount, nbl_part, inv_nbl, d_part,
               s_desc, spp, npass, pass_off, o_read, o_bkt, o_meta, o_rank, ov_cap, d_ov_cur);
    else if (k1_minw == 7)
        LAUNCH(c, "k_superkmers", k_superkmers<7>, dim3(grid), dim3(256), 0, nr, k1_chunk, c.d_bases, boff, good, c.NB, pb_lo, pb_hi, bcount, nbl_part, inv_nbl, d_part,
               s_desc, spp, npass, pass_off, o_read, o_bkt, o_meta, o_rank, ov_cap, d_ov_cur);
    else
        LAUNCH(c, "k_superkmers", k_superkmers<8>, dim3(grid), dim3(256), 0, nr, k1_chunk, c.d_bases, boff, good, c.NB, pb_lo, pb_hi, bcount, nbl_part, inv_nbl, d_part,
               s_desc, spp, npass, pass_off, o_read, o_bkt, o_meta, o_rank, ov_cap, d_ov_cur);
    W2_HIP(hipGetLastError());
    return 0;
}

int count_partition(Ctx& c, uint32_t nb, uint32_t n_parts, uint32_t pb_lo, uint32_t pb_hi) {
    if (pb_hi > nb || pb_lo >= pb_hi) { c.err = "partition: bad bucket range"; return W2RAP_E_ARG; }
    const uint32_t nbr = pb_hi - pb_lo;
    if (!c.quality_done) { c.err = "partition before quality_windows"; return W2RAP_E_STATE; }
    hipStream_t st = c.stream;
    const uint64_t n = c.n;
    if (n >= (1ull << 32)) { c.err = "more than 2^32 reads on one GPU (32-bit read ids in the record descriptors)"; return W2RAP_E_LIMIT; }
    c.NB = nb;
    if (c.d_bcount) c.release(c.d_bcount);
    if (c.d_bbase) c.release(c.d_bbase);
    if (c.d_recs) c.release(c.d_recs);
    W2_ALLOC(c.d_bcount, uint32_t, nbr);
    W2_ALLOC(c.d_bbase, uint64_t, (uint64_t)nbr + 1);
    unsigned long long* d_ov_cur = nullptr;
    W2_ALLOC(d_ov_cur, unsigned long long, 2);
    unsigned long long* d_part = nullptr;
    if (n_parts > 64 || (n_parts && nbr % n_parts)) { c.err = "partition: at most 64 parts, dividing the bucket count"; return W2RAP_E_LIMIT; }
    if (n_parts) W2_ALLOC(d_part, unsigned long long, 64 * 64);
    const uint32_t nbl_part = n_parts ? nbr / n_parts : 0, inv_nbl = nbl_part > 1 ? (uint32_t)((1ull << 32) / nbl_part) : 0;
    const char* sv = getenv("W2RAP_SPP");
    uint32_t spp = sv ? (uint32_t)atoi(sv) : 8;
    const uint32_t npass = c.max_len > K + 127 ? (c.max_len - (K - 1) + 127) / 128 : 1;
    uint2* s_desc = nullptr; uint32_t *o_read = nullptr, *o_bkt = nullptr, *o_meta = nullptr, *o_rank = nullptr;
    uint64_t ov_cap = n / 8 + 1024;
    W2_ALLOC(o_read, uint32_t, ov_cap); W2_ALLOC(o_bkt, uint32_t, ov_cap); W2_ALLOC(o_meta, uint32_t, ov_cap); W2_ALLOC(o_rank, uint32_t, ov_cap);
    uint64_t nslots = 0, nov = 0, npass_tot = 0;
    uint64_t* pass_off = nullptr;
    bool wave = false;
    for (;;) {
        wave = k1_wave(spp, npass);
        if (wave && !pass_off) { W2_ALLOC(pass_off, uint64_t, n + 1); W2_TRY(k1_pass_offsets(c, n, c.d_good, pass_off, &npass_tot)); }
        nslots = wave ? npass_tot * spp : n * npass * spp;
        W2_ALLOC(s_desc, uint2, nslots);
        W2_HIP(hipMemsetAsync(c.d_bcount, 0, (size_t)nbr * 4, st));
        W2_HIP(hipMemsetAsync(d_ov_cur, 0, 16, st));
        if (d_part) W2_HIP(hipMemsetAsync(d_part, 0, 64 * 64 * 8, st));
        if (n) W2_TRY(launch_k1(c, n, c.d_boff, c.d_good, pb_lo, pb_hi, c.d_bcount, nbl_part, inv_nbl, d_part, s_desc, spp, npass, pass_off, o_read, o_bkt, o_meta, o_rank, ov_cap, d_ov_cur));
        W2_TRY(exclusive_scan_u32_to_u64(c, c.d_bcount, c.d_bbase, nbr));
        unsigned long long h_ov = 0;
        W2_HIP(hipMemcpyAsync(&c.nrec, c.d_bbase + nbr, 8, hipMemcpyDeviceToHost, st));
        W2_HIP(hipMemcpyAsync(&h_ov, d_ov_cur, 8, hipMemcpyDeviceToHost, st));
        unsigned long long h_part[64 * 64];
        if (d_part) W2_HIP(hipMemcpyAsync(h_part, d_part, sizeof(h_part), hipMemcpyDeviceToHost, st));
        W2_HIP(hipStreamSynchronize(st));
        if (d_part) for (unsigned g = 0; g < 64; ++g) { c.part_kmers[g] = 0; for (unsigned k = 0; k < 64; ++k) c.part_kmers[g] += h_part[k * 64 + g]; }
        nov = h_ov;
        if (nov <= ov_cap) break;
        c.release(s_desc);
        if (nov > n && spp < 128) spp *= 2;
        for (uint32_t* q : {o_read, o_bkt, o_meta, o_rank}) c.release(q);
        ov_cap = nov + nov / 8 + 1024;
        W2_ALLOC(o_read, uint32_t, ov_cap); W2_ALLOC(o_bkt, uint32_t, ov_cap); W2_ALLOC(o_meta, uint32_t, ov_cap); W2_ALLOC(o_rank, uint32_t, ov_cap);
    }
    W2_ALLOC(c.d_recs, uint32_t, c.nrec * REC_DWORDS);
    if (c.nrec) {
        uint64_t bases_bytes = 0;
        W2_HIP(hipMemcpy(&bases_bytes, c.d_boff + n, 8, hipMemcpyDeviceToHost));
        const uint64_t nthreads = nslots + nov;
        if (wave)
            LAUNCH(c, "k_scatter_records", k_scatter_records<true>, dim3((unsigned)((nthreads + 255) / 256)), dim3(256), 0, nslots, spp, pass_off, n, s_desc,
                   nov, o_read, o_bkt, o_meta, o_rank, c.d_bases, c.d_boff, bases_bytes, c.d_bbase, c.d_recs);
        else
        LAUNCH(c, "k_scatter_records", k_scatter_records<false>, dim3((unsigned)((nthreads + 255) / 256)), dim3(256), 0, nslots, npass * spp, nullptr, 0, s_desc,
               nov, o_read, o_bkt, o_meta, o_rank, c.d_bases, c.d_boff, bases_bytes, c.d_bbase, c.d_recs);
        W2_HIP(hipGetLastError());
    }
    W2_HIP(hipStreamSynchronize(st));
    if (pass_off) c.release(pass_off);
    c.release(d_ov_cur); if (d_part) c.release(d_part); c.release(s_desc); c.release(o_read); c.release(o_bkt); c.release(o_meta); c.release(o_rank);
    return 0;
}

int count_partition_batched(Ctx& c, uint32_t nb, unsigned n_batches, unsigned* n_seg, uint32_t pb_lo, uint32_t pb_hi) {
    const uint32_t nbl = pb_hi - pb_lo;
    if (!c.quality_done) { c.err = "partition before quality_windows"; return W2RAP_E_STATE; }
    hipStream_t st = c.stream, st2 = c.stream2;
    const uint64_t n = c.n;
    if (n >= (1ull << 32)) { c.err = "more than 2^32 reads on one GPU (32-bit read ids in the record descriptors)"; return W2RAP_E_LIMIT; }
    if (n_batches < 1) n_batches = 1; if (n_batches > 16) n_batches = 16;
    if (n < (1u << 20) || !st2) n_batches = 1;
    c.NB = nb;
    if (c.d_bcount) c.release(c.d_bcount);
    if (c.d_bbase) { c.release(c.d_bbase); c.d_bbase = nullptr; }
    if (c.d_recs) c.release(c.d_recs);
    c.d_recs = nullptr;
    W2_ALLOC(c.d_bcount, uint32_t, (uint64_t)n_batches * nbl);
    uint64_t* d_bbase[2] = {nullptr, nullptr};
    uint2* s_desc[2] = {nullptr, nullptr};
    uint32_t *o_read[2] = {nullptr, nullptr}, *o_bkt[2] = {nullptr, nullptr}, *o_meta[2] = {nullptr, nullptr}, *o_rank[2] = {nullptr, nullptr};
    unsigned long long* d_ov_cur = nullptr;
    W2_ALLOC(d_ov_cur, unsigned long long, 2);
    const char* sv = getenv("W2RAP_SPP");
    uint32_t spp = sv ? (uint32_t)atoi(sv) : 8;
    const uint32_t npass = c.max_len > K + 127 ? (c.max_len - (K - 1) + 127) / 128 : 1;
    const double last_frac = getenv("W2RAP_LAST_BATCH") ? std::min(1.0, std::max(0.1, atof(getenv("W2RAP_LAST_BATCH")))) : 1.0;
    const uint64_t per_batch = n_batches > 1 ? (((uint64_t)((double)n / ((double)n_batches - 1.0 + last_frac)) + 2) & ~1ull) : ((n + 1) & ~1ull);
    uint64_t ov_cap[2] = {per_batch / 8 + 1024, per_batch / 8 + 1024};
    uint64_t slots_alloc[2] = {0, 0};
    uint64_t* pass_off[2] = {nullptr, nullptr};
    uint64_t pass_k[2] = {~0ull, ~0ull}, npass_tot[2] = {0, 0};
    for (int b = 0; b < 2; ++b) {
        W2_ALLOC(d_bbase[b], uint64_t, (uint64_t)nbl + 1);
        W2_ALLOC(o_read[b], uint32_t, ov_cap[b]); W2_ALLOC(o_bkt[b], uint32_t, ov_cap[b]); W2_ALLOC(o_meta[b], uint32_t, ov_cap[b]);
        W2_ALLOC(o_rank[b], uint32_t, ov_cap[b]);
    }
    uint64_t bases_bytes = 0;
    if (n) W2_HIP(hipMemcpy(&bases_bytes, c.d_boff + n, 8, hipMemcpyDeviceToHost));
    hipEvent_t ev_k2[16] = {};
    uint64_t rec_cap = 0, seg_base = 0;
    c.nrec = 0;
    unsigned nseg = 0;
    for (unsigned k = 0; k < n_batches; ++k) {
        const uint64_t r0 = std::min<uint64_t>(n, k * per_batch), r1 = std::min<uint64_t>(n, r0 + per_batch), nr = r1 - r0;
        const int b = k & 1;
        uint32_t* bcount = c.d_bcount + (uint64_t)k * nbl;
        if (k >= 2) W2_HIP(hipEventSynchronize(ev_k2[k - 2]));
        uint64_t nslots = 0, nov = 0, nrec_k = 0;
        bool wave = false;
        for (;;) {
            wave = k1_wave(spp, npass);
            if (wave && pass_k[b] != k) {
                if (!pass_off[b]) W2_ALLOC(pass_off[b], uint64_t, per_batch + 1);
                W2_TRY(k1_pass_offsets(c, nr, c.d_good + r0, pass_off[b], &npass_tot[b]));
                pass_k[b] = k;
            }
            nslots = wave ? npass_tot[b] * spp : nr * npass * spp;
            if (slots_alloc[b] < nslots) { if (s_desc[b]) c.release(s_desc[b]); W2_ALLOC(s_desc[b], uint2, nslots); slots_alloc[b] = nslots; }
            W2_HIP(hipMemsetAsync(bcount, 0, (size_t)nbl * 4, st));
            W2_HIP(hipMemsetAsync(d_ov_cur, 0, 16, st));
            if (nr) W2_TRY(launch_k1(c, nr, c.d_boff + r0, c.d_good + r0, pb_lo, pb_hi, bcount, 0u, 0u, nullptr, s_desc[b], spp, npass, wave ? pass_off[b] : nullptr, o_read[b], o_bkt[b], o_meta[b], o_rank[b], ov_cap[b], d_ov_cur));
            W2_TRY(exclusive_scan_u32_to_u64(c, bcount, d_bbase[b], nbl));
            unsigned long long h_ov = 0;
            W2_HIP(hipMemcpyAsync(&nrec_k, d_bbase[b] + nbl, 8, hipMemcpyDeviceToHost, st));
            W2_HIP(hipMemcpyAsync(&h_ov, d_ov_cur, 8, hipMemcpyDeviceToHost, st));
            W2_HIP(hipStreamSynchronize(st));
            nov = h_ov;
            if (nov <= ov_cap[b]) break;
            if (nov > nr && spp < 128) spp *= 2;
            for (uint32_t* q : {o_read[b], o_bkt[b], o_meta[b], o_rank[b]}) c.release(q);
            ov_cap[b] = nov + nov / 8 + 1024;
            W2_ALLOC(o_read[b], uint32_t, ov_cap[b]); W2_ALLOC(o_bkt[b], uint32_t, ov_cap[b]); W2_ALLOC(o_meta[b], uint32_t, ov_cap[b]);
            W2_ALLOC(o_rank[b], uint32_t, ov_cap[b]);
        }
        if (seg_base + nrec_k > rec_cap) {
            const uint64_t want = k == 0 ? (uint64_t)((double)nrec_k * ((double)n / (double)std::max<uint64_t>(nr, 1))) + nrec_k / 16 + (1u << 20) : (seg_base + nrec_k) * 2;
            uint32_t* bigger = c.alloc<uint32_t>(want * REC_DWORDS);
            if (!bigger) return W2RAP_E_HIP;
            if (c.d_recs) {
                W2_HIP(hipStreamSynchronize(st2));
                W2_HIP(hipMemcpyAsync(bigger, c.d_recs, seg_base * REC_BYTES, hipMemcpyDeviceToDevice, st2));
                W2_HIP(hipStreamSynchronize(st2));
                c.release(c.d_recs);
            }
            c.d_recs = bigger; rec_cap = want;
        }
        hipStream_t sk = n_batches > 1 ? st2 : st;
        if (nrec_k) {
            const uint64_t nthreads = nslots + nov;
            if (wave)
                LAUNCH_ON(c, sk, "k_scatter_records", k_scatter_records<true>, dim3((unsigned)((nthreads + 255) / 256)), dim3(256), 0, nslots, spp, pass_off[b], nr, s_desc[b],
                          nov, o_read[b], o_bkt[b], o_meta[b], o_rank[b], c.d_bases, c.d_boff + r0, bases_bytes, d_bbase[b], c.d_recs + seg_base * REC_DWORDS);
            else
            LAUNCH_ON(c, sk, "k_scatter_records", k_scatter_records<false>, dim3((unsigned)((nthreads + 255) / 256)), dim3(256), 0, nslots, npass * spp, nullptr, 0, s_desc[b],
                      nov, o_read[b], o_bkt[b], o_meta[b], o_rank[b], c.d_bases, c.d_boff + r0, bases_bytes, d_bbase[b], c.d_recs + seg_base * REC_DWORDS);
            W2_HIP(hipGetLastError());
        }
        W2_HIP(hipEventCreateWithFlags(&ev_k2[k], hipEventDisableTiming));
        W2_HIP(hipEventRecord(ev_k2[k], sk));
        seg_base += nrec_k;
        nseg = k + 1;
    }
    for (unsigned k = 0; k < nseg; ++k) { W2_HIP(hipEventSynchronize(ev_k2[k])); (void)hipEventDestroy(ev_k2[k]); }
    c.nrec = seg_base;
    if (!c.d_recs) W2_ALLOC(c.d_recs, uint32_t, REC_DWORDS);
    for (int b = 0; b < 2; ++b) {
        c.release(d_bbase[b]); if (s_desc[b]) c.release(s_desc[b]); if (pass_off[b]) c.release(pass_off[b]);
        c.release(o_read[b]); c.release(o_bkt[b]); c.release(o_meta[b]); c.release(o_rank[b]);
    }
    c.release(d_ov_cur);
    *n_seg = nseg;
    return 0;
}

static void table_geometry(uint64_t S, uint64_t& tcap) {
    const char* lf = getenv("W2RAP_TABLE_X");
    const uint64_t mult10 = lf ? 10 * (uint64_t)atoll(lf) : (S < (1ull << 30) ? 40 : 13);
    tcap = 1024;
    while (10 * tcap < mult10 * S) tcap <<= 1;
}

int count_buckets_launch(Ctx& c, uint32_t min_freq, uint32_t nbl, uint32_t nseg, const uint32_t* d_recs, const uint32_t* d_counts,
                         uint64_t total_kmers, unsigned NS, bool deferred) {
    hipStream_t st = c.stream;
    if (c.cs_planned) { c.err = "count_records_begin: a sliced count is already pending"; return W2RAP_E_STATE; }
    c.min_freq = min_freq;
    if (!c.pass) c.table_built = false;
    if (NS < 1) NS = 1; if (NS > 16) NS = 16;
    if (nbl < 4096) NS = 1;
    if (nseg > 64) { c.err = "count_records: more than 64 segments"; return W2RAP_E_LIMIT; }
    const uint64_t nflat = (uint64_t)nbl * nseg;
    uint64_t* d_off = nullptr;
    W2_ALLOC(d_off, uint64_t, nflat + 1);
    W2_TRY(exclusive_scan_u32_to_u64(c, d_counts, d_off, nflat));
    unsigned long long* d_cnt = c.pass ? c.pass_cnt : nullptr;
    uint32_t chunk_cap = c.pass ? c.cs_chunk_cap : 0;
    if (!c.pass) {
        W2_ALLOC(d_cnt, unsigned long long, 160);
        W2_HIP(hipMemsetAsync(d_cnt, 0, 160 * sizeof(unsigned long long), st));
        c.solid_cap = total_kmers / (min_freq ? min_freq : 1) + 1;
        for (void* p : {(void*)c.d_shi, (void*)c.d_slo, (void*)c.d_scc}) if (p) c.release(p);
        W2_ALLOC(c.d_shi, uint64_t, c.solid_cap);
        W2_ALLOC(c.d_slo, uint64_t, c.solid_cap);
        W2_ALLOC(c.d_scc, uint32_t, c.solid_cap);
        if (c.d_chunk_start) { c.release(c.d_chunk_start); c.release(c.d_chunk_cnt); c.d_chunk_start = nullptr; c.d_chunk_cnt = nullptr; }
        c.nchunks = 0;
        if (!getenv("W2RAP_NO_LOCAL_PRUNE")) {
            const uint64_t nb_all = c.npass > 1 ? c.NB : nbl;
            chunk_cap = (uint32_t)std::min<uint64_t>(nb_all * 2 + 4096, 1u << 24);
            W2_ALLOC(c.d_chunk_start, uint64_t, chunk_cap);
            W2_ALLOC(c.d_chunk_cnt, uint32_t, chunk_cap);
            W2_HIP(hipMemsetAsync(c.d_chunk_cnt, 0, (size_t)chunk_cap * 4, st));
        }
    }
    c.cs_cnt = d_cnt; c.cs_off = d_off; c.cs_chunk_cap = chunk_cap;
    W2_ALLOC(c.cs_defer, uint32_t, (uint64_t)nbl + 2);
    c.cs_planned = NS; c.cs_ns = 0; c.cs_nbl = nbl; c.cs_nseg = nseg; c.cs_recs = d_recs;
    c.cs_short_first = deferred && NS >= 3;
    if (!deferred) for (unsigned k = 0; k < NS; ++k) W2_TRY(count_buckets_launch_slice(c, k));
    return 0;
}

void count_slice_bounds(const Ctx& c, unsigned k, uint32_t* b_lo, uint32_t* b_hi) {
    const uint64_t NS = c.cs_planned, nbl = c.cs_nbl;
    auto cut = [&](uint64_t j) -> uint32_t {
        if (!c.cs_short_first) return (uint32_t)(nbl * j / NS);
        return (uint32_t)(j == 0 ? 0 : nbl * (2 * j - 1) / (2 * NS - 1));
    };
    *b_lo = cut(k); *b_hi = cut(k + 1);
}

int count_buckets_launch_slice(Ctx& c, unsigned k) {
    hipStream_t st = c.stream;
    if (!c.cs_planned || k != c.cs_ns || k >= c.cs_planned) { c.err = "count_records_launch: slices are launched once each, in order"; return W2RAP_E_STATE; }
    const unsigned NS = c.cs_planned;
    const uint32_t nbl = c.cs_nbl, nseg = c.cs_nseg;
    unsigned long long* d_cnt = c.cs_cnt;
#ifndef W2RAP_QUEUE_AT
#define W2RAP_QUEUE_AT 144
#endif
    uint32_t* d_queue = reinterpret_cast<uint32_t*>(d_cnt + W2RAP_QUEUE_AT);
    uint32_t b_lo, b_hi;
    count_slice_bounds(c, k, &b_lo, &b_hi);
    auto slice_done = [&]() -> int {
        W2_HIP(hipMemcpyAsync(c.h_pinned + k, d_cnt + 4, 8, hipMemcpyDeviceToHost, st));
        W2_HIP(hipEventCreateWithFlags(&c.cs_ev[k], hipEventDisableTiming));
        W2_HIP(hipEventRecord(c.cs_ev[k], st));
        c.cs_ns = k + 1;
        return 0;
    };
    auto launch = [&](auto kern, unsigned lds, unsigned threads, unsigned blocks_per_cu) -> int {
        W2_HIP(hipFuncSetAttribute(reinterpret_cast<const void*>(kern), hipFuncAttributeMaxDynamicSharedMemorySize, lds));
        unsigned grid = (unsigned)std::min<uint64_t>(b_hi - b_lo, (uint64_t)c.sm_count * blocks_per_cu);
        if (k || c.pass) W2_HIP(hipMemsetAsync(d_queue, 0, 4, st));
        LAUNCH(c, "k_count_buckets", kern, dim3(grid ? grid : 1), dim3(threads), lds, nbl, b_lo, b_hi, nseg, c.cs_off, c.cs_recs, c.min_freq, d_queue,
               c.d_shi, c.d_slo, c.d_scc, c.solid_cap, d_cnt + 4, d_cnt + 8, c.d_chunk_start, c.d_chunk_cnt, c.cs_chunk_cap, (const uint32_t*)nullptr, 0u);
        W2_HIP(hipGetLastError());
        return slice_done();
    };
    auto launch_fp = [&](auto kern, unsigned lds, unsigned threads, unsigned blocks_per_cu, uint32_t fp_limit, uint32_t fp_sc) -> int {
        W2_HIP(hipFuncSetAttribute(reinterpret_cast<const void*>(kern), hipFuncAttributeMaxDynamicSharedMemorySize, lds));
        auto list_kern = k_count_buckets<COUNT_CAP, COUNT_THREADS>;
        W2_HIP(hipFuncSetAttribute(reinterpret_cast<const void*>(list_kern), hipFuncAttributeMaxDynamicSharedMemorySize, (int)K3Cfg<COUNT_CAP, COUNT_THREADS>::LDS));
        const unsigned grid = (unsigned)std::min<uint64_t>(b_hi - b_lo, (uint64_t)c.sm_count * blocks_per_cu);
        if (k || c.pass) W2_HIP(hipMemsetAsync(d_queue, 0, 4, st));
        if (k == 0) W2_HIP(hipMemsetAsync(c.cs_defer, 0, 8, st));
        uint32_t fill_limit = fp_limit, solid_limit = fp_sc;
        if (const char* t = getenv("W2RAP_TEST_FP_LIMIT")) { if (test_hook("W2RAP_TEST_FP_LIMIT")) fill_limit = std::min<uint32_t>(fill_limit, (uint32_t)std::max(1, atoi(t))); }
        if (const char* t = getenv("W2RAP_TEST_FP_SC")) { if (test_hook("W2RAP_TEST_FP_SC")) solid_limit = std::min<uint32_t>(solid_limit, (uint32_t)std::max(1, atoi(t))); }
        LAUNCH(c, "k_count_fp", kern, dim3(grid ? grid : 1), dim3(threads), lds, nbl, b_lo, b_hi, nseg, c.cs_off, c.cs_recs, c.min_freq, d_queue,
               c.d_shi, c.d_slo, c.d_scc, c.solid_cap, d_cnt + 4, d_cnt + 8, c.d_chunk_start, c.d_chunk_cnt, c.cs_chunk_cap, c.cs_defer, nbl, fill_limit, solid_limit,
               c.fused_prune ? c.d_sctx : (uint8_t*)nullptr, c.fused_prune ? c.d_unres : (uint8_t*)nullptr, c.fused_prune ? (uint32_t*)c.d_nbr : (uint32_t*)nullptr);
        W2_HIP(hipGetLastError());
        if (k + 1 == NS && c.fused_prune) W2_HIP(hipMemcpyAsync(c.h_pinned + 20, d_cnt + 4, 8, hipMemcpyDeviceToHost, st));
        if (k + 1 == NS) {
            const unsigned lgrid = (unsigned)std::min<uint64_t>(nbl, (uint64_t)c.sm_count);
            constexpr unsigned list_lds = K3Cfg<COUNT_CAP, COUNT_THREADS>::LDS;
            LAUNCH(c, "k_count_buckets", list_kern, dim3(lgrid ? lgrid : 1), dim3(COUNT_THREADS), list_lds, nbl, 0u, nbl, nseg, c.cs_off,
                   c.cs_recs, c.min_freq, c.cs_defer + 1, c.d_shi, c.d_slo, c.d_scc, c.solid_cap, d_cnt + 4, d_cnt + 8, c.d_chunk_start, c.d_chunk_cnt, c.cs_chunk_cap,
                   (const uint32_t*)c.cs_defer, nbl);
            W2_HIP(hipGetLastError());
        }
        return slice_done();
    };
    const char* v = getenv("W2RAP_K3");
    int cfg = v ? atoi(v) : 22;
    if (cfg >= 20 && nseg > FpCfg<512, 512, 1024>::MAXSEG) cfg = 0;
    if (cfg == 20) W2_TRY(launch_fp(k_count_fp<512, 4, 640, 768>, FpCfg<512, 640, 768>::LDS, 512, 2, FpCfg<512, 640, 768>::LIMIT, 768));
    else if (cfg == 21) W2_TRY(launch_fp(k_count_fp<1024, 8, 576, 512>, FpCfg<1024, 576, 512>::LDS, 1024, 2, FpCfg<1024, 576, 512>::LIMIT, 512));
    else if (cfg == 22) W2_TRY(launch_fp(k_count_fp<512, 4, 512, 1024>, FpCfg<512, 512, 1024>::LDS, 512, 2, FpCfg<512, 512, 1024>::LIMIT, 1024));
    else if (cfg == 23) W2_TRY(launch_fp(k_count_fp<1024, 4, 576, 1024>, FpCfg<1024, 576, 1024>::LDS, 1024, 1, FpCfg<1024, 576, 1024>::LIMIT, 1024));
    else if (cfg == 24) W2_TRY(launch_fp(k_count_fp<512, 4, 576, 1024>, FpCfg<512, 576, 1024>::LDS, 512, 2, FpCfg<512, 576, 1024>::LIMIT, 1024));
    else if (cfg == 1) W2_TRY(launch(k_count_buckets<2048, 512>, K3Cfg<2048, 512>::LDS, 512, 2));
    else if (cfg == 2) W2_TRY(launch(k_count_buckets<4096, 512>, K3Cfg<4096, 512>::LDS, 512, 1));
    else if (cfg == 3) W2_TRY(launch(k_count_buckets<1024, 256>, K3Cfg<1024, 256>::LDS, 256, 4));
    else if (cfg == 5) W2_TRY(launch(k_count_buckets<2048, 1024, false, false, 8>, K3Cfg<2048, 1024, false>::LDS, 1024, 2));
    else if (cfg == 8) W2_TRY(launch(k_count_buckets<4096, 1024, false, false, 1>, K3Cfg<4096, 1024, false>::LDS, 1024, 1));
    else if (cfg == 9) W2_TRY(launch(k_count_buckets<COUNT_CAP, COUNT_THREADS, true>, K3Cfg<COUNT_CAP, COUNT_THREADS>::LDS, COUNT_THREADS, 1));
    else W2_TRY(launch(k_count_buckets<COUNT_CAP, COUNT_THREADS>, K3Cfg<COUNT_CAP, COUNT_THREADS>::LDS, COUNT_THREADS, 1));
    return 0;
}

int count_buckets_slice(Ctx& c, unsigned k, uint64_t* n_solid, uint64_t* n_chunks) {
    if (k >= c.cs_ns) { c.err = "count_records_slice: slice not launched"; return W2RAP_E_ARG; }
    W2_HIP(hipEventSynchronize(c.cs_ev[k]));
    const uint64_t w = c.h_pinned[k];
    if (n_solid) *n_solid = std::min<uint64_t>(w & ((1ull << 40) - 1), c.solid_cap);
    if (n_chunks) *n_chunks = std::min<uint64_t>(w >> 40, c.cs_chunk_cap);
    return 0;
}

int count_buckets_finish(Ctx& c) {
    hipStream_t st = c.stream;
    if (!c.cs_planned || c.cs_ns != c.cs_planned) { c.err = "count_records_end: not every slice has been launched"; return W2RAP_E_STATE; }
    unsigned long long h_all[160];
    W2_HIP(hipMemcpyAsync(h_all, c.cs_cnt, sizeof(h_all), hipMemcpyDeviceToHost, st));
    W2_HIP(hipStreamSynchronize(st));
    for (unsigned k = 0; k < c.cs_ns; ++k) (void)hipEventDestroy(c.cs_ev[k]);
    c.cs_ns = 0; c.cs_planned = 0;
    if (c.pass + 1 < c.npass) c.pass_cnt = c.cs_cnt;
    else { c.release(c.cs_cnt); c.pass_cnt = nullptr; c.pass = 0; c.npass = 1; }
    c.release(c.cs_off); c.cs_cnt = nullptr; c.cs_off = nullptr;
    if (getenv("W2RAP_TRACE") && c.cs_defer) {
        uint32_t nd = 0;
        (void)hipMemcpy(&nd, c.cs_defer, 4, hipMemcpyDeviceToHost);
        fprintf(stderr, "[w2rap] k_count_fp deferred %u buckets (all slices) to k_count_buckets\n", nd);
    }
    if (c.cs_defer) { c.release(c.cs_defer); c.cs_defer = nullptr; }
    if (getenv("W2RAP_TRACE") && h_all[111])
        fprintf(stderr, "[w2rap] k_count_buckets wave-0 clocks per block: stage-in %.0f, count %.0f, barrier A %.0f, flush+scan %.0f, barrier B %.0f, staging %.0f; slowest wave's count %.0f (x%u blocks, %u buckets)\n",
                (double)h_all[110] / c.sm_count, (double)h_all[111] / c.sm_count, (double)h_all[112] / c.sm_count, (double)h_all[113] / c.sm_count,
                (double)h_all[114] / c.sm_count, (double)h_all[115] / c.sm_count, (double)h_all[116] / c.sm_count, (unsigned)c.sm_count, 0u);
    if (getenv("W2RAP_TRACE") && h_all[128]) {
        fprintf(stderr, "[w2rap] k_count_buckets count-phase clocks per block, by wave:");
        for (int w = 0; w < 16; ++w) fprintf(stderr, " %.1fM", (double)h_all[128 + w] / c.sm_count / 1e6);
        fprintf(stderr, "\n");
    }
    if (getenv("W2RAP_TRACE") && h_all[121])
        fprintf(stderr, "[w2rap] k_count_buckets wave-0 clocks per window: loads %.0f, extract+hash %.0f, probe %.0f, atomics %.0f (%.0f windows per block)\n",
                (double)h_all[117] / h_all[121], (double)h_all[118] / h_all[121], (double)h_all[119] / h_all[121], (double)h_all[120] / h_all[121],
                (double)h_all[121] / c.sm_count);
    if (h_all[7]) { c.err = "k_count_buckets: a bucket did not fit the LDS table after 2^16-way splitting"; return W2RAP_E_LIMIT; }
    c.S = h_all[4] & ((1ull << 40) - 1); c.D = h_all[5];
    c.nchunks = c.cs_chunk_cap ? std::min<uint64_t>(h_all[4] >> 40, c.cs_chunk_cap) : 0;
    for (int i = 0; i < 101; ++i) c.hist[i] = h_all[8 + i];
    if (c.S > c.solid_cap) { c.err = "solid k-mer count exceeds its bound"; return W2RAP_E_LIMIT; }
    return 0;
}

static int table_alloc(Ctx& c, uint64_t S, hipStream_t on) {
    uint64_t tcap;
    table_geometry(S, tcap);
    c.tcap = tcap;
    W2_ALLOC(c.d_table, Slot, tcap);
    W2_HIP(hipMemsetAsync(c.d_table, 0xFF, tcap * sizeof(Slot), on));
    return 0;
}

int count_buckets(Ctx& c, uint32_t min_freq, uint32_t nbl, uint32_t nseg, const uint32_t* d_recs, const uint32_t* d_counts,
                  uint64_t total_kmers, bool build_table) {
    hipStream_t st2 = c.stream2;
    const char* nsv = getenv("W2RAP_SLICES");
    unsigned NS = (build_table && !getenv("W2RAP_NO_OVERLAP") && nbl >= 4096 && st2) ? (nsv ? (unsigned)atoi(nsv) : 4) : 1;
    {
        const char* fv = getenv("W2RAP_FUSED_PRUNE"); const char* kv = getenv("W2RAP_K3"); const char* wv = getenv("W2RAP_WIDE_IDS");
        const uint64_t cap = total_kmers / (min_freq ? min_freq : 1) + 1;
        c.fused_prune = build_table && fv && atoi(fv) == 1 && !(kv && atoi(kv) < 20) && !(wv && atoi(wv) != 0) && cap < (1ull << 31) - 1 && c.npass == 1 &&
                        nseg <= 16 && !getenv("W2RAP_NO_LOCAL_PRUNE");
        c.unfused_chunks.clear();
        if (c.fused_prune) {
            for (void* p : {(void*)c.d_sctx, (void*)c.d_nbr, (void*)c.d_unres}) if (p) c.release(p);
            W2_ALLOC(c.d_sctx, uint8_t, cap); W2_ALLOC(c.d_unres, uint8_t, cap);
            uint32_t* nb32 = nullptr; W2_ALLOC(nb32, uint32_t, 2 * cap); c.d_nbr = nb32;
            W2_HIP(hipMemsetAsync(c.d_sctx, 0xFF, cap, c.stream));
            W2_HIP(hipMemsetAsync(c.d_unres, 0xFF, cap, c.stream));
        }
    }
    W2_TRY(count_buckets_launch(c, min_freq, nbl, nseg, d_recs, d_counts, total_kmers, NS, false));
    NS = c.cs_ns;
    uint64_t s_cap = 0;
    if (NS > 1) {
        uint64_t s_prev = 0;
        for (unsigned k = 0; k < NS; ++k) {
            uint64_t s_k = 0;
            W2_TRY(count_buckets_slice(c, k, &s_k, nullptr));
            if (k == 0) {
                s_cap = s_k * NS + s_k / 2 + 1024;
                if (test_hook("W2RAP_TEST_SMALL_SCAP")) s_cap = s_k + 1;
                W2_TRY(table_alloc(c, s_k * NS, st2));
            }
            const uint64_t s_hi = s_k < s_cap ? s_k : s_cap;
            if (s_hi > s_prev) {
                LAUNCH_ON(c, st2, "k_table_insert", k_table_insert, dim3((unsigned)((s_hi - s_prev + 255) / 256)), dim3(256), 0, s_prev, s_hi,
                          c.d_shi, c.d_slo, c.d_table, c.tcap - 1);
                W2_HIP(hipGetLastError());
                s_prev = s_hi;
            }
        }
    }
    W2_TRY(count_buckets_finish(c));
    if (c.fused_prune) c.unfused_chunks.emplace_back(std::min<uint64_t>(c.h_pinned[20] >> 40, c.nchunks), c.nchunks);
    if (NS > 1) {
        if (c.S <= s_cap && 10 * c.tcap >= 13 * c.S) c.table_built = true;
        else {
            W2_HIP(hipStreamSynchronize(st2));
            c.release(c.d_table);
            c.d_table = nullptr;
        }
    }
    return 0;
}

__global__ void __launch_bounds__(256) k_shift_u64(uint64_t n, const uint64_t* __restrict__ in, uint64_t add, uint64_t* __restrict__ out) {
    uint64_t i = (uint64_t)blockIdx.x * blockDim.x + threadIdx.x;
    if (i < n) out[i] = in[i] + add;
}
void dict_abort(Ctx& c) {
    if (!c.g_open) return;
    if (c.stream2) (void)hipStreamSynchronize(c.stream2);
    for (void* p : {(void*)c.g_hi, (void*)c.g_lo, (void*)c.g_cc, (void*)c.g_cstart, (void*)c.g_ccnt, (void*)c.d_table}) if (p) c.release(p);
    c.g_hi = c.g_lo = nullptr; c.g_cc = nullptr; c.g_cstart = nullptr; c.g_ccnt = nullptr; c.d_table = nullptr;
    c.g_open = false; c.g_n = c.g_nc = 0;
}
int dict_begin(Ctx& c, uint64_t kmer_cap, uint64_t chunk_cap) {
    if (c.g_open) dict_abort(c);
    if (!c.stream2) { c.err = "dict_begin: no side stream"; return W2RAP_E_STATE; }
    if (kmer_cap >= MAX_SOLID_KMERS) { c.err = "more than 2^32 solid k-mers on one GPU"; return W2RAP_E_LIMIT; }
    if (c.d_table) c.release(c.d_table);
    c.d_table = nullptr;
    W2_ALLOC(c.g_hi, uint64_t, kmer_cap); W2_ALLOC(c.g_lo, uint64_t, kmer_cap); W2_ALLOC(c.g_cc, uint32_t, kmer_cap);
    c.g_cstart = nullptr; c.g_ccnt = nullptr;
    if (chunk_cap) { W2_ALLOC(c.g_cstart, uint64_t, chunk_cap); W2_ALLOC(c.g_ccnt, uint32_t, chunk_cap); }
    c.g_cap = kmer_cap; c.g_ccap = chunk_cap; c.g_n = 0; c.g_nc = 0;
    W2_TRY(table_alloc(c, kmer_cap, c.stream2));
    c.g_open = true;
    return 0;
}
int dict_append(Ctx& c, const uint64_t* d_hi, const uint64_t* d_lo, const uint32_t* d_cc, uint64_t n, const uint64_t* d_cstart, const uint32_t* d_ccnt,
                uint64_t nc, uint64_t chunk_bias) {
    hipStream_t st2 = c.stream2;
    if (!c.g_open) { c.err = "dict_append before dict_begin"; return W2RAP_E_STATE; }
    if (c.g_n + n > c.g_cap || (nc && c.g_nc + nc > c.g_ccap)) { c.err = "dict_append: capacity of dict_begin exceeded"; return W2RAP_E_LIMIT; }
    if (n) {
        W2_HIP(hipMemcpyAsync(c.g_hi + c.g_n, d_hi, n * 8, hipMemcpyDeviceToDevice, st2));
        W2_HIP(hipMemcpyAsync(c.g_lo + c.g_n, d_lo, n * 8, hipMemcpyDeviceToDevice, st2));
        W2_HIP(hipMemcpyAsync(c.g_cc + c.g_n, d_cc, n * 4, hipMemcpyDeviceToDevice, st2));
    }
    if (nc) {
        hipLaunchKernelGGL(k_shift_u64, dim3((unsigned)((nc + 255) / 256)), dim3(256), 0, st2, nc, d_cstart, c.g_n - chunk_bias, c.g_cstart + c.g_nc);
        W2_HIP(hipMemcpyAsync(c.g_ccnt + c.g_nc, d_ccnt, nc * 4, hipMemcpyDeviceToDevice, st2));
    }
    if (!c.g_copied) W2_HIP(hipEventCreateWithFlags(&c.g_copied, hipEventDisableTiming));
    W2_HIP(hipEventRecord(c.g_copied, st2));
    if (n) {
        LAUNCH_ON(c, st2, "k_table_insert", k_table_insert, dim3((unsigned)((n + 255) / 256)), dim3(256), 0, c.g_n, c.g_n + n,
                  c.g_hi, c.g_lo, c.d_table, c.tcap - 1);
        W2_HIP(hipGetLastError());
    }
    c.g_n += n; c.g_nc += nc;
    return 0;
}
int dict_end(Ctx& c) {
    if (!c.g_open) { c.err = "dict_end before dict_begin"; return W2RAP_E_STATE; }
    if (c.cs_planned) { c.err = "dict_end while a sliced count is pending (count_records_end first)"; return W2RAP_E_STATE; }
    for (void* p : {(void*)c.d_shi, (void*)c.d_slo, (void*)c.d_scc, (void*)c.d_recs, (void*)c.d_sctx, (void*)c.d_nbr, (void*)c.d_chunk_start, (void*)c.d_chunk_cnt})
        if (p) c.release(p);
    c.d_recs = nullptr; c.d_sctx = nullptr; c.d_nbr = nullptr;
    c.d_shi = c.g_hi; c.d_slo = c.g_lo; c.d_scc = c.g_cc; c.S = c.g_n; c.solid_cap = c.g_cap;
    c.d_chunk_start = c.g_cstart; c.d_chunk_cnt = c.g_ccnt; c.nchunks = c.g_nc;
    c.g_hi = c.g_lo = nullptr; c.g_cc = nullptr; c.g_cstart = nullptr; c.g_ccnt = nullptr; c.g_open = false;
    bool wait_copies = true;
#ifdef W2RAP_TESTING
    if (test_hook("W2RAP_TEST_NO_APPEND_WAIT")) wait_copies = false;
#endif
    if (c.g_copied && wait_copies) W2_HIP(hipStreamWaitEvent(c.stream, c.g_copied, 0));
    if (10 * c.tcap >= 13 * c.S) c.table_built = true;
    else {
        W2_HIP(hipStreamSynchronize(c.stream2));
        c.release(c.d_table);
        c.d_table = nullptr; c.table_built = false;
    }
    return count_table(c);
}

int table_build_plain(Ctx& c) {
    if (c.d_table) { c.release(c.d_table); c.d_table = nullptr; }
    W2_TRY(table_alloc(c, c.S, c.stream));
    if (c.S) {
        LAUNCH(c, "k_table_insert", k_table_insert, dim3((unsigned)((c.S + 255) / 256)), dim3(256), 0, (uint64_t)0, c.S, c.d_shi, c.d_slo, c.d_table, c.tcap - 1);
        W2_HIP(hipGetLastError());
    }
    c.table_built = false;
    return 0;
}
int local_dict_slice(Ctx& c, uint64_t n_solid, uint64_t expected_total) {
    if (!c.stream2) return 0;
    if (!c.table_built) {
        if (c.d_table) { c.release(c.d_table); c.d_table = nullptr; }
        W2_TRY(table_alloc(c, std::max<uint64_t>(expected_total, n_solid), c.stream2));
        c.table_built = true; c.ld_done = 0;
    }
    if (n_solid > c.solid_cap) n_solid = c.solid_cap;
    if (n_solid > c.ld_done && 10 * c.tcap >= 13 * n_solid) {
        LAUNCH_ON(c, c.stream2, "k_table_insert", k_table_insert, dim3((unsigned)((n_solid - c.ld_done + 255) / 256)), dim3(256), 0, c.ld_done, n_solid,
                  c.d_shi, c.d_slo, c.d_table, c.tcap - 1);
        W2_HIP(hipGetLastError());
        c.ld_done = n_solid;
    }
    return 0;
}
int prune_local_chunks64(Ctx& c, uint8_t* sctx, uint64_t* nbr, uint8_t* unres) {
    hipStream_t st = c.stream;
    W2_HIP(hipMemsetAsync(unres, 0xFF, c.S, st));
    W2_HIP(hipMemsetAsync(sctx, 0xFF, c.S, st));
    if (!c.nchunks || getenv("W2RAP_NO_LOCAL_PRUNE")) return 0;
    const unsigned gl = (unsigned)std::min<uint64_t>(c.nchunks, (uint64_t)c.sm_count * 64);
    PL_LAUNCH(c, uint64_t, gl, c.S, c.nchunks, c.d_chunk_start, c.d_chunk_cnt, c.d_shi, c.d_slo, c.d_scc, sctx, nbr, unres);
    W2_HIP(hipGetLastError());
    return 0;
}
int prune_local_chunks32(Ctx& c, uint8_t* sctx, uint32_t* nbr, uint8_t* unres) {
    hipStream_t st = c.stream;
    W2_HIP(hipMemsetAsync(unres, 0xFF, c.S, st));
    W2_HIP(hipMemsetAsync(sctx, 0xFF, c.S, st));
    if (!c.nchunks || getenv("W2RAP_NO_LOCAL_PRUNE")) return 0;
    const unsigned gl = (unsigned)std::min<uint64_t>(c.nchunks, (uint64_t)c.sm_count * 64);
    PL_LAUNCH(c, uint32_t, gl, c.S, c.nchunks, c.d_chunk_start, c.d_chunk_cnt, c.d_shi, c.d_slo, c.d_scc, sctx, nbr, unres);
    W2_HIP(hipGetLastError());
    return 0;
}

template <class Id>
static int count_table_t(Ctx& c) {
    hipStream_t st = c.stream;
    if (!c.table_built) W2_TRY(table_alloc(c, c.S, st));
    const bool fused = c.fused_prune && sizeof(Id) == 4 && c.d_sctx && c.d_nbr && c.d_unres;
    Id* nbr = nullptr;
    if (fused) nbr = reinterpret_cast<Id*>(c.d_nbr);
    else {
        for (void* p : {(void*)c.d_sctx, (void*)c.d_nbr, (void*)c.d_unres}) if (p) c.release(p);
        c.d_unres = nullptr;
        W2_ALLOC(c.d_sctx, uint8_t, c.S);
        W2_ALLOC(nbr, Id, 2 * c.S);
        c.d_nbr = nbr;
    }
    c.fused_prune = false;
    if (c.S) {
        unsigned g = (unsigned)((c.S + 255) / 256);
        if (!c.table_built) {
            LAUNCH(c, "k_table_insert", k_table_insert, dim3(g), dim3(256), 0, (uint64_t)0, c.S, c.d_shi, c.d_slo, c.d_table, c.tcap - 1);
            W2_HIP(hipGetLastError());
        }
        uint8_t* d_unres = nullptr;
        if (fused) {
            d_unres = c.d_unres; c.d_unres = nullptr;
            for (auto& rg : c.unfused_chunks) {
                const uint64_t nch = rg.second - rg.first;
                if (!nch) continue;
                const unsigned gl = (unsigned)std::min<uint64_t>(nch, (uint64_t)c.sm_count * 64);
                PL_LAUNCH(c, Id, gl, c.S, nch, c.d_chunk_start + rg.first, c.d_chunk_cnt + rg.first, c.d_shi, c.d_slo, c.d_scc, c.d_sctx, nbr, d_unres);
                W2_HIP(hipGetLastError());
            }
        } else if (c.nchunks) {
            W2_ALLOC(d_unres, uint8_t, c.S);
            W2_HIP(hipMemsetAsync(d_unres, 0xFF, c.S, st));
            W2_HIP(hipMemsetAsync(c.d_sctx, 0xFF, c.S, st));
            const unsigned gl = (unsigned)std::min<uint64_t>(c.nchunks, (uint64_t)c.sm_count * 64);
            PL_LAUNCH(c, Id, gl, c.S, c.nchunks, c.d_chunk_start, c.d_chunk_cnt, c.d_shi, c.d_slo, c.d_scc, c.d_sctx, nbr, d_unres);
            W2_HIP(hipGetLastError());
        }
        if (c.table_built && c.stream2) {
            hipEvent_t ev;
            W2_HIP(hipEventCreateWithFlags(&ev, hipEventDisableTiming));
            W2_HIP(hipEventRecord(ev, c.stream2));
            W2_HIP(hipStreamWaitEvent(st, ev, 0));
            (void)hipEventDestroy(ev);
        }
        LAUNCH(c, "k_prune", k_prune<Id>, dim3(g), dim3(256), 0, (uint64_t)0, c.S, c.d_shi, c.d_slo, c.d_scc, c.d_table, c.tcap - 1, c.d_sctx, nbr,
               (const uint8_t*)d_unres);
        W2_HIP(hipGetLastError());
        W2_HIP(hipStreamSynchronize(st));
        if (d_unres) c.release(d_unres);
    }
    W2_HIP(hipStreamSynchronize(st));
    if (c.stream2) W2_HIP(hipStreamSynchronize(c.stream2));
    c.table_built = false;
    c.counted = true;
    return 0;
}
int count_table(Ctx& c) {
    if (c.S >= MAX_SOLID_KMERS) { c.err = "more than 2^32 solid k-mers on one GPU"; return W2RAP_E_LIMIT; }
    const char* wv = getenv("W2RAP_WIDE_IDS");
    c.wide_ids = c.S >= (1ull << 31) - 1 || (wv && atoi(wv) != 0);
    return c.wide_ids ? count_table_t<uint64_t>(c) : count_table_t<uint32_t>(c);
}

static unsigned auto_passes(uint64_t M) {
    size_t free_b = 0, total_b = 0;
    if (hipMemGetInfo(&free_b, &total_b) != hipSuccess || !free_b) return 1;
    const double need = (double)M / 15.0 * REC_BYTES * 1.25;
    unsigned p = (unsigned)(need / ((double)free_b / 4.0)) + 1;
    return std::min(p, 64u);
}

int phase_count(Ctx& c, uint32_t min_qual, uint32_t min_freq) {
    const bool trace = getenv("W2RAP_TRACE") != nullptr;
    auto now = [] { return std::chrono::duration<double>(std::chrono::steady_clock::now().time_since_epoch()).count(); };
    double t0 = now();
    W2_TRY(count_quality(c, min_qual));
    double t1 = now();
    const char* bv = getenv("W2RAP_BATCHES");
    const char* pv = getenv("W2RAP_PASSES");
    unsigned P = pv ? (unsigned)atoi(pv) : c.n_passes;
    if (!P) P = auto_passes(c.M);
    const uint32_t NB = default_buckets(c.M, 1);
    if (P > NB) P = NB;
    if (P < 1) P = 1;
    c.npass = P;
    double t_part = 0, t_cnt = 0;
    for (unsigned p = 0; p < P; ++p) {
        const uint32_t lo = (uint32_t)((uint64_t)NB * p / P), hi = (uint32_t)((uint64_t)NB * (p + 1) / P);
        unsigned nseg = 1;
        c.pass = p;
        double a = now();
        W2_TRY(count_partition_batched(c, NB, bv ? (unsigned)atoi(bv) : 4, &nseg, lo, hi));
        double b = now();
        W2_TRY(count_buckets(c, min_freq, hi - lo, nseg, c.d_recs, c.d_bcount, c.M, P == 1));
        c.release(c.d_recs); c.d_recs = nullptr;
        t_part += b - a; t_cnt += now() - b;
    }
    c.pass = 0; c.npass = 1;
    double t3 = now();
    W2_TRY(count_table(c));
    double t4 = now();
    if (trace) fprintf(stderr, "[w2rap] count: quality %.1f ms, partition %.1f ms, buckets %.1f ms, table %.1f ms (%u pass%s)\n",
                       (t1 - t0) * 1e3, t_part * 1e3, t_cnt * 1e3, (t4 - t3) * 1e3, P, P == 1 ? "" : "es");
    return 0;
}

}
```

Baseline: 41.29 billion.

## Add slab partition route that writes super-k-mer records directly into per-bucket slabs

Adds a slab-based partitioning path where the super-k-mer kernel builds records in place and writes them to fixed-capacity per-bucket slabs. Records that exceed a slab go to an overflow list that is scattered afterward. Counting kernels now take separate begin/end ranges so they can read the non-contiguous slab layout. The intent is to skip the separate count/scan/scatter passes of the batched partition. In exchange it may over-allocate memory for the slabs and adds an overflow segment.

```diff
diff --git a/w2rap_contigger_amd/csrc/ctx.h b/w2rap_contigger_amd/csrc/ctx.h
--- a/w2rap_contigger_amd/csrc/ctx.h
+++ b/w2rap_contigger_amd/csrc/ctx.h
@@ -71,6 +71,7 @@
     hipEvent_t cs_ev[16] = {};
     unsigned long long* cs_cnt = nullptr;
     uint64_t* cs_off = nullptr;
+    const uint64_t* cs_beg = nullptr; const uint64_t* cs_end = nullptr;
     uint32_t cs_chunk_cap = 0;
     uint8_t* d_unres = nullptr;
     bool fused_prune = false;
@@ -330,9 +331,9 @@
 uint32_t default_buckets(uint64_t total_kmers, uint32_t multiple_of);
 int count_partition(Ctx& c, uint32_t nb, uint32_t n_parts, uint32_t pb_lo, uint32_t pb_hi);
 int count_buckets(Ctx& c, uint32_t min_freq, uint32_t nbl, uint32_t nseg, const uint32_t* d_recs, const uint32_t* d_counts, uint64_t total_kmers,
-                  bool build_table = false);
+                  bool build_table = false, const uint64_t* d_beg = nullptr, const uint64_t* d_end = nullptr);
 int count_buckets_launch(Ctx& c, uint32_t min_freq, uint32_t nbl, uint32_t nseg, const uint32_t* d_recs, const uint32_t* d_counts, uint64_t total_kmers,
-                         unsigned n_slices, bool deferred);
+                         unsigned n_slices, bool deferred, const uint64_t* d_beg = nullptr, const uint64_t* d_end = nullptr);
 int count_buckets_launch_slice(Ctx& c, unsigned k);
 void count_slice_bounds(const Ctx& c, unsigned k, uint32_t* b_lo, uint32_t* b_hi);
 int count_buckets_slice(Ctx& c, unsigned k, uint64_t* n_solid, uint64_t* n_chunks);
diff --git a/w2rap_contigger_amd/csrc/step2_capi.hip b/w2rap_contigger_amd/csrc/step2_capi.hip
--- a/w2rap_contigger_amd/csrc/step2_capi.hip
+++ b/w2rap_contigger_amd/csrc/step2_capi.hip
@@ -65,7 +65,7 @@
     c.d_table = nullptr; c.d_filter32 = nullptr; c.f32words = 0; c.d_sctx = nullptr; c.d_nbr = nullptr; c.d_srec = nullptr; c.d_index = nullptr; c.index_cap = 0; c.d_xindex = nullptr; c.xindex_cap = 0; c.d_unres = nullptr; c.fused_prune = false; c.unfused_chunks.clear();
     c.d_chunk_start = nullptr; c.d_chunk_cnt = nullptr; c.nchunks = 0;
     for (unsigned k = 0; k < c.cs_ns; ++k) (void)hipEventDestroy(c.cs_ev[k]);
-    c.cs_ns = 0; c.cs_planned = 0; c.cs_cnt = nullptr; c.cs_off = nullptr; c.cs_defer = nullptr; c.pass = 0; c.npass = 1; c.pass_cnt = nullptr;
+    c.cs_ns = 0; c.cs_planned = 0; c.cs_cnt = nullptr; c.cs_off = nullptr; c.cs_beg = nullptr; c.cs_end = nullptr; c.cs_defer = nullptr; c.pass = 0; c.npass = 1; c.pass_cnt = nullptr;
     c.g_hi = c.g_lo = nullptr; c.g_cc = nullptr; c.g_cstart = nullptr; c.g_ccnt = nullptr; c.g_open = false; c.g_n = c.g_nc = 0;
     c.d_edge_nk = nullptr; c.d_edge_off = nullptr; c.d_edge_codes = nullptr; c.d_edge_bits = nullptr; c.d_fwdX = c.d_revX = nullptr; c.d_obj_edge = nullptr;
     c.d_otab = nullptr; c.d_left = c.d_right = nullptr; c.d_from_off = c.d_to_off = nullptr; c.d_from_v = c.d_from_e = c.d_to_v = c.d_to_e = nullptr;
diff --git a/w2rap_contigger_amd/csrc/step2_count.hip b/w2rap_contigger_amd/csrc/step2_count.hip
--- a/w2rap_contigger_amd/csrc/step2_count.hip
+++ b/w2rap_contigger_amd/csrc/step2_count.hip
@@ -306,14 +306,85 @@
 }
 
 
-template <unsigned SMAX, bool ALIGN64>
+__device__ inline void store_records_via_lds(uint32_t* s_rec, uint64_t* s_dst, unsigned lane, const uint32_t (&out)[REC_DWORDS], uint64_t dst,
+                                             uint32_t* __restrict__ recs) {
+    if constexpr (REC_DWORDS == 8) {
+        reinterpret_cast<uint4*>(s_rec)[2 * lane] = make_uint4(out[0], out[1], out[2], out[3]);
+        reinterpret_cast<uint4*>(s_rec)[2 * lane + 1] = make_uint4(out[4], out[5], out[6], out[7]);
+    } else {
+#pragma unroll
+        for (unsigned j = 0; j < REC_DWORDS; ++j) s_rec[lane * REC_DWORDS + j] = out[j];
+    }
+    s_dst[lane] = dst;
+    wave_lds_fence();
+    if constexpr (REC_DWORDS == 8) {
+#pragma unroll
+        for (unsigned j = 0; j < 2; ++j) {
+            const unsigned idx = j * 64 + lane, rec = idx >> 1;
+            const uint64_t d = s_dst[rec];
+            if (d != ~0ull) reinterpret_cast<uint4*>(recs + d)[idx & 1u] = reinterpret_cast<const uint4*>(s_rec)[idx];
+        }
+    } else {
+#pragma unroll
+        for (unsigned j = 0; j < REC_DWORDS; ++j) {
+            const unsigned idx = j * 64 + lane, rec = idx / REC_DWORDS, qd = idx - rec * REC_DWORDS;
+            const uint64_t d = s_dst[rec];
+            if (d != ~0ull) recs[d + qd] = s_rec[idx];
+        }
+    }
+}
+
+__device__ inline void build_record(const uint8_t* __restrict__ bases, uint64_t bases_bytes, uint64_t ro, uint32_t meta, uint32_t (&out)[REC_DWORDS]) {
+    const unsigned p = meta & 0xFFFFu, nk = ((meta >> 16) & 63u) + 1u;
+    const bool hasL = (meta >> 22) & 1u, hasR = (meta >> 23) & 1u;
+    const unsigned q = p ? p - 1 : 0;
+    const uint64_t byte0 = ro + ((2 * q) >> 3);
+    const unsigned sh = (2 * q) & 7;
+    uint64_t W[5];
+#pragma unroll
+    for (unsigned j = 0; j < 5; ++j) {
+        const uint64_t a = byte0 + 8 * j;
+        uint64_t w = 0;
+        if (a + 8 <= bases_bytes) w = reinterpret_cast<const U64u*>(bases + a)->v;
+        else for (unsigned t = 0; t < 8; ++t) if (a + t < bases_bytes) w |= (uint64_t)bases[a + t] << (8 * t);
+        W[j] = w;
+    }
+    uint64_t O[4];
+#pragma unroll
+    for (unsigned j = 0; j < 4; ++j) O[j] = sh ? (W[j] >> sh) | (W[j + 1] << (64 - sh)) : W[j];
+    if (!p) {
+        O[3] = (O[3] << 2) | (O[2] >> 62); O[2] = (O[2] << 2) | (O[1] >> 62); O[1] = (O[1] << 2) | (O[0] >> 62); O[0] <<= 2;
+    }
+    unsigned nbits = 2 * (nk + 61);
+    if (!hasR) nbits -= 2;
+#pragma unroll
+    for (unsigned j = 0; j < 4; ++j) {
+        if (nbits <= 64 * j) O[j] = 0;
+        else if (nbits < 64 * (j + 1)) O[j] &= (1ull << (nbits - 64 * j)) - 1;
+    }
+    const uint32_t hdr = (nk - 1) | (hasL ? 64u : 0u) | (hasR ? 128u : 0u);
+    if constexpr (REC_HB == 8) {
+        O[3] = (O[3] << 8) | (O[2] >> 56); O[2] = (O[2] << 8) | (O[1] >> 56); O[1] = (O[1] << 8) | (O[0] >> 56);
+        O[0] = (O[0] << 8) | (uint64_t)hdr;
+#pragma unroll
+        for (unsigned j = 0; j < 4; ++j) { out[2 * j] = (uint32_t)O[j]; out[2 * j + 1] = (uint32_t)(O[j] >> 32); }
+    } else {
+        out[0] = hdr;
+#pragma unroll
+        for (unsigned j = 0; j < 4; ++j) { out[(1 + 2 * j) % REC_DWORDS] = (uint32_t)O[j]; out[(2 + 2 * j) % REC_DWORDS] = (uint32_t)(O[j] >> 32); }
+    }
+}
+
+template <unsigned SMAX, bool ALIGN64, bool SLAB = false>
 __global__ void __launch_bounds__(256, 4) k_superkmers_lane(uint64_t n, const uint8_t* __restrict__ bases, const uint64_t* __restrict__ boff,
                                                             const uint16_t* __restrict__ good, uint32_t nb, uint32_t pb_lo, uint32_t pb_hi,
                                                             uint32_t* __restrict__ bcount, uint32_t nbl_part, uint32_t inv_nbl,
                                                             unsigned long long* __restrict__ part_kmers, uint2* __restrict__ s_desc, uint32_t S,
                                                             uint32_t* __restrict__ o_read, uint32_t* __restrict__ o_bkt, uint32_t* __restrict__ o_meta,
-                                                            uint32_t* __restrict__ o_rank, uint64_t ov_cap, unsigned long long* __restrict__ ov_cursor) {
-    __shared__ uint2 stage_[4][64 * SMAX];
+                                                            uint32_t* __restrict__ o_rank, uint64_t ov_cap, unsigned long long* __restrict__ ov_cursor,
+                                                            uint64_t bases_bytes, uint32_t slab_cap, uint32_t* __restrict__ recs ) {
+    static_assert(!SLAB || (SMAX % 8 == 0 && 64 * REC_DWORDS * 4 + 64 * 8 <= 64 * 8 * sizeof(uint2)), "a flush round's slots hold its records");
+    __shared__ __attribute__((aligned(16))) uint2 stage_[4][64 * SMAX];
     __shared__ uint32_t spart_[4][64];
     const unsigned lane = threadIdx.x & 63, wv_ = threadIdx.x >> 6;
     const uint64_t r0 = ((uint64_t)blockIdx.x * 4 + wv_) * 64;
@@ -424,6 +495,44 @@
                 }
             }
         }
+        if constexpr (SLAB) {
+            wave_lds_fence();
+            uint32_t* s_rec = reinterpret_cast<uint32_t*>(stage + 64 * u0);
+            uint64_t* s_dst = reinterpret_cast<uint64_t*>(s_rec + 64 * REC_DWORDS);
+            unsigned long long om[8], obase = 0;
+            unsigned novf = 0;
+#pragma unroll
+            for (unsigned k = 0; k < 8; ++k) {
+                const unsigned i = lane + 64 * (u0 + k);
+                om[k] = __ballot(u0 + k < S && i < nflat && d[k].y != NONE32 && rk[k] >= slab_cap);
+                novf += (unsigned)__popcll(om[k]);
+            }
+            if (novf) {
+                if (lane == 0) obase = atomicAdd(ov_cursor, (unsigned long long)novf);
+                obase = (unsigned long long)__shfl((long long)obase, 0);
+            }
+#pragma unroll
+            for (unsigned k = 0; k < 8; ++k) {
+                const unsigned i = lane + 64 * (u0 + k);
+                uint64_t dst = ~0ull;
+                uint32_t out[REC_DWORDS] = {};
+                const bool has = u0 + k < S && i < nflat && d[k].y != NONE32;
+                const uint64_t rd = r0 + i / S;
+                if (has && rk[k] < slab_cap) {
+                    build_record(bases, bases_bytes, boff[rd], d[k].y, out);
+                    dst = ((uint64_t)d[k].x * slab_cap + rk[k]) * REC_DWORDS;
+                }
+                if (om[k]) {
+                    const unsigned long long o = obase + __popcll(om[k] & ((1ull << lane) - 1ull));
+                    if (has && rk[k] >= slab_cap && o < ov_cap) { o_read[o] = (uint32_t)rd; o_bkt[o] = d[k].x; o_meta[o] = d[k].y; o_rank[o] = rk[k]; }
+                    obase += __popcll(om[k]);
+                }
+                if (!__any(dst != ~0ull)) continue;
+                store_records_via_lds(s_rec, s_dst, lane, out, dst, recs);
+                wave_lds_fence();
+            }
+            continue;
+        }
 #pragma unroll
         for (unsigned k = 0; k < 8; ++k) {
             const unsigned i = lane + 64 * (u0 + k);
@@ -456,7 +565,8 @@
                                                           const uint8_t* __restrict__ bases,
                                                           const uint64_t* __restrict__ boff, uint64_t bases_bytes,
                                                           const uint64_t* __restrict__ bbase,
-                                                          uint32_t* __restrict__ recs) {
+                                                          uint32_t* __restrict__ recs,
+                                                          uint32_t slab_cap ) {
     __shared__ __attribute__((aligned(16))) uint32_t s_rec[4][64 * REC_DWORDS];
     __shared__ uint64_t s_dst[4][64];
     const unsigned lane = threadIdx.x & 63, wv = threadIdx.x >> 6;
@@ -476,72 +586,10 @@
     uint64_t dst = ~0ull;
     uint32_t out[REC_DWORDS] = {};
     if (valid) {
-        const uint64_t base = bbase[b];
-        const unsigned p = meta & 0xFFFFu, nk = ((meta >> 16) & 63u) + 1u;
-        const bool hasL = (meta >> 22) & 1u, hasR = (meta >> 23) & 1u;
-        const uint64_t ro = boff[r];
-        const unsigned q = p ? p - 1 : 0;
-        const uint64_t byte0 = ro + ((2 * q) >> 3);
-        const unsigned sh = (2 * q) & 7;
-        uint64_t W[5];
-#pragma unroll
-        for (unsigned j = 0; j < 5; ++j) {
-            const uint64_t a = byte0 + 8 * j;
-            uint64_t w = 0;
-            if (a + 8 <= bases_bytes) w = reinterpret_cast<const U64u*>(bases + a)->v;
-            else for (unsigned t = 0; t < 8; ++t) if (a + t < bases_bytes) w |= (uint64_t)bases[a + t] << (8 * t);
-            W[j] = w;
-        }
-        uint64_t O[4];
-#pragma unroll
-        for (unsigned j = 0; j < 4; ++j) O[j] = sh ? (W[j] >> sh) | (W[j + 1] << (64 - sh)) : W[j];
-        if (!p) {
-            O[3] = (O[3] << 2) | (O[2] >> 62); O[2] = (O[2] << 2) | (O[1] >> 62); O[1] = (O[1] << 2) | (O[0] >> 62); O[0] <<= 2;
-        }
-        unsigned nbits = 2 * (nk + 61);
-        if (!hasR) nbits -= 2;
-#pragma unroll
-        for (unsigned j = 0; j < 4; ++j) {
-            if (nbits <= 64 * j) O[j] = 0;
-            else if (nbits < 64 * (j + 1)) O[j] &= (1ull << (nbits - 64 * j)) - 1;
-        }
-        const uint32_t hdr = (nk - 1) | (hasL ? 64u : 0u) | (hasR ? 128u : 0u);
-        if constexpr (REC_HB == 8) {
-            O[3] = (O[3] << 8) | (O[2] >> 56); O[2] = (O[2] << 8) | (O[1] >> 56); O[1] = (O[1] << 8) | (O[0] >> 56);
-            O[0] = (O[0] << 8) | (uint64_t)hdr;
-#pragma unroll
-            for (unsigned j = 0; j < 4; ++j) { out[2 * j] = (uint32_t)O[j]; out[2 * j + 1] = (uint32_t)(O[j] >> 32); }
-        } else {
-            out[0] = hdr;
-#pragma unroll
-            for (unsigned j = 0; j < 4; ++j) { out[(1 + 2 * j) % REC_DWORDS] = (uint32_t)O[j]; out[(2 + 2 * j) % REC_DWORDS] = (uint32_t)(O[j] >> 32); }
-        }
-        dst = (base + slot) * REC_DWORDS;
-    }
-    if constexpr (REC_DWORDS == 8) {
-        reinterpret_cast<uint4*>(s_rec[wv])[2 * lane] = make_uint4(out[0], out[1], out[2], out[3]);
-        reinterpret_cast<uint4*>(s_rec[wv])[2 * lane + 1] = make_uint4(out[4], out[5], out[6], out[7]);
-    } else {
-#pragma unroll
-        for (unsigned j = 0; j < REC_DWORDS; ++j) s_rec[wv][lane * REC_DWORDS + j] = out[j];
-    }
-    s_dst[wv][lane] = dst;
-    wave_lds_fence();
-    if constexpr (REC_DWORDS == 8) {
-#pragma unroll
-        for (unsigned j = 0; j < 2; ++j) {
-            const unsigned idx = j * 64 + lane, rec = idx >> 1;
-            const uint64_t d = s_dst[wv][rec];
-            if (d != ~0ull) reinterpret_cast<uint4*>(recs + d)[idx & 1u] = reinterpret_cast<const uint4*>(s_rec[wv])[idx];
-        }
-    } else {
-#pragma unroll
-        for (unsigned j = 0; j < REC_DWORDS; ++j) {
-            const unsigned idx = j * 64 + lane, rec = idx / REC_DWORDS, qd = idx - rec * REC_DWORDS;
-            const uint64_t d = s_dst[wv][rec];
-            if (d != ~0ull) recs[d + qd] = s_rec[wv][idx];
-        }
-    }
+        build_record(bases, bases_bytes, boff[r], meta, out);
+        dst = (slab_cap && slot < slab_cap ? (uint64_t)b * slab_cap + slot : bbase[b] + (slot - slab_cap)) * REC_DWORDS;
+    }
+    store_records_via_lds(s_rec[wv], s_dst[wv], lane, out, dst, recs);
 }
 
 template <unsigned CAP, unsigned THREADS, bool PARK = true>
@@ -591,7 +639,7 @@
 
 template <unsigned CAP, unsigned THREADS, bool PROF = false, bool PARK = true, unsigned MINW = 1>
 __global__ void __launch_bounds__(THREADS, MINW) k_count_buckets(uint32_t nb, uint32_t b_lo, uint32_t b_hi ,
-                                                            uint32_t nseg, const uint64_t* __restrict__ roff,
+                                                            uint32_t nseg, const uint64_t* __restrict__ rbeg, const uint64_t* __restrict__ rend ,
                                                             const uint32_t* __restrict__ recs, uint32_t min_freq,
                                                             uint32_t* __restrict__ queue,
                                                             uint64_t* __restrict__ shi, uint64_t* __restrict__ slo,
@@ -633,7 +681,7 @@
     auto seg_load = [&](uint32_t bb, uint64_t& r0, uint32_t& cnt) {
         r0 = 0; cnt = 0;
         if (tid < nseg && bb < b_hi) {
-            const uint64_t a = roff[(uint64_t)tid * nb + bb], e = roff[(uint64_t)tid * nb + bb + 1];
+            const uint64_t a = rbeg[(uint64_t)tid * nb + bb], e = rend[(uint64_t)tid * nb + bb];
             r0 = a; cnt = (uint32_t)(e - a);
             if (e - a >= (1ull << 26)) { cnt = 0; counters[3] = 2; }
         }
@@ -1073,7 +1121,7 @@
 }
 
 template <unsigned THREADS, unsigned MINW, unsigned TILE_, unsigned SC_>
-__global__ void __launch_bounds__(THREADS, MINW) k_count_fp(uint32_t nb, uint32_t b_lo, uint32_t b_hi, uint32_t nseg, const uint64_t* __restrict__ roff,
+__global__ void __launch_bounds__(THREADS, MINW) k_count_fp(uint32_t nb, uint32_t b_lo, uint32_t b_hi, uint32_t nseg, const uint64_t* __restrict__ rbeg, const uint64_t* __restrict__ rend ,
                                                             const uint32_t* __restrict__ recs, uint32_t min_freq, uint32_t* __restrict__ queue,
                                                             uint64_t* __restrict__ shi, uint64_t* __restrict__ slo, uint32_t* __restrict__ scc, uint64_t solid_cap,
                                                             unsigned long long* __restrict__ counters, unsigned long long* __restrict__ ghist,
@@ -1108,7 +1156,7 @@
     auto seg_load = [&](uint32_t bb, uint64_t& r0, uint32_t& cnt) {
         r0 = 0; cnt = 0;
         if (tid < nseg && bb < b_hi) {
-            const uint64_t a = roff[(uint64_t)tid * nb + bb], e = roff[(uint64_t)tid * nb + bb + 1];
+            const uint64_t a = rbeg[(uint64_t)tid * nb + bb], e = rend[(uint64_t)tid * nb + bb];
             r0 = a; cnt = e - a < (1ull << 20) ? (uint32_t)(e - a) : (1u << 20);
         }
     };
@@ -1641,6 +1689,9 @@
 }
 
 static constexpr unsigned COUNT_CAP = 4096, COUNT_THREADS = 1024;
+#ifndef W2RAP_SLAB_DEFAULT
+#define W2RAP_SLAB_DEFAULT 1
+#endif
 static constexpr unsigned KMERS_PER_BUCKET = 4500;
 
 int count_quality(Ctx& c, uint32_t min_qual) {
@@ -1694,6 +1745,11 @@
 }
 
 
+static void k1_slots(const Ctx& c, uint32_t* spp, uint32_t* npass) {
+    const char* sv = getenv("W2RAP_SPP");
+    *spp = sv ? (uint32_t)atoi(sv) : 8;
+    *npass = c.max_len > K + 127 ? (c.max_len - (K - 1) + 127) / 128 : 1;
+}
 static bool k1_wave(uint32_t spp, uint32_t npass) {
     const char* k1v = getenv("W2RAP_K1");
     return (k1v && !strcmp(k1v, "wave")) || spp * npass > 16;
@@ -1723,16 +1779,20 @@
 static int launch_k1(Ctx& c, uint64_t nr, const uint64_t* boff, const uint16_t* good, uint32_t pb_lo, uint32_t pb_hi, uint32_t* bcount,
                      uint32_t nbl_part, uint32_t inv_nbl, unsigned long long* d_part, uint2* s_desc, uint32_t spp, uint32_t npass,
                      const uint64_t* pass_off ,
-                     uint32_t* o_read, uint32_t* o_bkt, uint32_t* o_meta, uint32_t* o_rank, uint64_t ov_cap, unsigned long long* d_ov_cur) {
+                     uint32_t* o_read, uint32_t* o_bkt, uint32_t* o_meta, uint32_t* o_rank, uint64_t ov_cap, unsigned long long* d_ov_cur,
+                     uint32_t slab_cap = 0 , uint32_t* slab_recs = nullptr,
+                     uint64_t bases_bytes = 0) {
     if (getenv("W2RAP_TRACE"))
         fprintf(stderr, "[w2rap] K1 route: %s, npass %u, spp %u, %llu reads, longest %u\n", k1_wave(spp, npass) ? "wave" : "lane",
                 npass, spp, (unsigned long long)nr, c.max_len);
+    if (slab_recs && k1_wave(spp, npass)) { c.err = "K1: the slab mode belongs to the lane kernel"; return W2RAP_E_STATE; }
     if (!k1_wave(spp, npass)) {
         const bool a64 = getenv("W2RAP_K1_ALIGN64") != nullptr;
         const dim3 grid((unsigned)((nr + 255) / 256));
-#define W2_K1L(A64) LAUNCH(c, "k_superkmers_lane", (k_superkmers_lane<16, A64>), grid, dim3(256), 0, nr, c.d_bases, boff, good, c.NB, pb_lo, pb_hi, bcount, \
-                           nbl_part, inv_nbl, d_part, s_desc, spp * npass, o_read, o_bkt, o_meta, o_rank, ov_cap, d_ov_cur)
-        if (a64) W2_K1L(true); else W2_K1L(false);
+#define W2_K1L(A64, SLAB) LAUNCH(c, "k_superkmers_lane", (k_superkmers_lane<16, A64, SLAB>), grid, dim3(256), 0, nr, c.d_bases, boff, good, c.NB, pb_lo, pb_hi, bcount, \
+                           nbl_part, inv_nbl, d_part, s_desc, spp * npass, o_read, o_bkt, o_meta, o_rank, ov_cap, d_ov_cur, bases_bytes, slab_cap, slab_recs)
+        if (slab_recs) { if (a64) W2_K1L(true, true); else W2_K1L(false, true); }
+        else if (a64) W2_K1L(true, false); else W2_K1L(false, false);
 #undef W2_K1L
         W2_HIP(hipGetLastError());
         return 0;
@@ -1772,9 +1832,8 @@
     if (n_parts > 64 || (n_parts && nbr % n_parts)) { c.err = "partition: at most 64 parts, dividing the bucket count"; return W2RAP_E_LIMIT; }
     if (n_parts) W2_ALLOC(d_part, unsigned long long, 64 * 64);
     const uint32_t nbl_part = n_parts ? nbr / n_parts : 0, inv_nbl = nbl_part > 1 ? (uint32_t)((1ull << 32) / nbl_part) : 0;
-    const char* sv = getenv("W2RAP_SPP");
-    uint32_t spp = sv ? (uint32_t)atoi(sv) : 8;
-    const uint32_t npass = c.max_len > K + 127 ? (c.max_len - (K - 1) + 127) / 128 : 1;
+    uint32_t spp, npass;
+    k1_slots(c, &spp, &npass);
     uint2* s_desc = nullptr; uint32_t *o_read = nullptr, *o_bkt = nullptr, *o_meta = nullptr, *o_rank = nullptr;
     uint64_t ov_cap = n / 8 + 1024;
     W2_ALLOC(o_read, uint32_t, ov_cap); W2_ALLOC(o_bkt, uint32_t, ov_cap); W2_ALLOC(o_meta, uint32_t, ov_cap); W2_ALLOC(o_rank, uint32_t, ov_cap);
@@ -1813,10 +1872,10 @@
         const uint64_t nthreads = nslots + nov;
         if (wave)
             LAUNCH(c, "k_scatter_records", k_scatter_records<true>, dim3((unsigned)((nthreads + 255) / 256)), dim3(256), 0, nslots, spp, pass_off, n, s_desc,
-                   nov, o_read, o_bkt, o_meta, o_rank, c.d_bases, c.d_boff, bases_bytes, c.d_bbase, c.d_recs);
+                   nov, o_read, o_bkt, o_meta, o_rank, c.d_bases, c.d_boff, bases_bytes, c.d_bbase, c.d_recs, 0u);
         else
         LAUNCH(c, "k_scatter_records", k_scatter_records<false>, dim3((unsigned)((nthreads + 255) / 256)), dim3(256), 0, nslots, npass * spp, nullptr, 0, s_desc,
-               nov, o_read, o_bkt, o_meta, o_rank, c.d_bases, c.d_boff, bases_bytes, c.d_bbase, c.d_recs);
+               nov, o_read, o_bkt, o_meta, o_rank, c.d_bases, c.d_boff, bases_bytes, c.d_bbase, c.d_recs, 0u);
         W2_HIP(hipGetLastError());
     }
     W2_HIP(hipStreamSynchronize(st));
@@ -1844,9 +1903,8 @@
     uint32_t *o_read[2] = {nullptr, nullptr}, *o_bkt[2] = {nullptr, nullptr}, *o_meta[2] = {nullptr, nullptr}, *o_rank[2] = {nullptr, nullptr};
     unsigned long long* d_ov_cur = nullptr;
     W2_ALLOC(d_ov_cur, unsigned long long, 2);
-    const char* sv = getenv("W2RAP_SPP");
-    uint32_t spp = sv ? (uint32_t)atoi(sv) : 8;
-    const uint32_t npass = c.max_len > K + 127 ? (c.max_len - (K - 1) + 127) / 128 : 1;
+    uint32_t spp, npass;
+    k1_slots(c, &spp, &npass);
     const double last_frac = getenv("W2RAP_LAST_BATCH") ? std::min(1.0, std::max(0.1, atof(getenv("W2RAP_LAST_BATCH")))) : 1.0;
     const uint64_t per_batch = n_batches > 1 ? (((uint64_t)((double)n / ((double)n_batches - 1.0 + last_frac)) + 2) & ~1ull) : ((n + 1) & ~1ull);
     uint64_t ov_cap[2] = {per_batch / 8 + 1024, per_batch / 8 + 1024};
@@ -1913,10 +1971,10 @@
             const uint64_t nthreads = nslots + nov;
             if (wave)
                 LAUNCH_ON(c, sk, "k_scatter_records", k_scatter_records<true>, dim3((unsigned)((nthreads + 255) / 256)), dim3(256), 0, nslots, spp, pass_off[b], nr, s_desc[b],
-                          nov, o_read[b], o_bkt[b], o_meta[b], o_rank[b], c.d_bases, c.d_boff + r0, bases_bytes, d_bbase[b], c.d_recs + seg_base * REC_DWORDS);
+                          nov, o_read[b], o_bkt[b], o_meta[b], o_rank[b], c.d_bases, c.d_boff + r0, bases_bytes, d_bbase[b], c.d_recs + seg_base * REC_DWORDS, 0u);
             else
             LAUNCH_ON(c, sk, "k_scatter_records", k_scatter_records<false>, dim3((unsigned)((nthreads + 255) / 256)), dim3(256), 0, nslots, npass * spp, nullptr, 0, s_desc[b],
-                      nov, o_read[b], o_bkt[b], o_meta[b], o_rank[b], c.d_bases, c.d_boff + r0, bases_bytes, d_bbase[b], c.d_recs + seg_base * REC_DWORDS);
+                      nov, o_read[b], o_bkt[b], o_meta[b], o_rank[b], c.d_bases, c.d_boff + r0, bases_bytes, d_bbase[b], c.d_recs + seg_base * REC_DWORDS, 0u);
             W2_HIP(hipGetLastError());
         }
         W2_HIP(hipEventCreateWithFlags(&ev_k2[k], hipEventDisableTiming));
@@ -1936,6 +1994,127 @@
     return 0;
 }
 
+__global__ void __launch_bounds__(256) k_slab_ranges(uint32_t nbl, uint32_t cap, const uint32_t* __restrict__ bcount, uint64_t* __restrict__ beg0,
+                                                     uint64_t* __restrict__ end0, uint32_t* __restrict__ ov_cnt, unsigned long long* __restrict__ totals) {
+    __shared__ unsigned long long s_tot[3];
+    if (threadIdx.x < 3) s_tot[threadIdx.x] = 0;
+    __syncthreads();
+    const uint32_t b = blockIdx.x * blockDim.x + threadIdx.x;
+    if (b < nbl) {
+        const uint32_t cnt = bcount[b], in = cnt < cap ? cnt : cap;
+        beg0[b] = (uint64_t)b * cap; end0[b] = (uint64_t)b * cap + in; ov_cnt[b] = cnt - in;
+        if (cnt) { atomicMax(&s_tot[0], (unsigned long long)cnt); atomicAdd(&s_tot[1], (unsigned long long)cnt); }
+        if (cnt - in) atomicAdd(&s_tot[2], (unsigned long long)(cnt - in));
+    }
+    __syncthreads();
+    if (threadIdx.x == 0 && s_tot[0]) atomicMax(&totals[0], s_tot[0]);
+    else if (threadIdx.x < 3 && s_tot[threadIdx.x]) atomicAdd(&totals[threadIdx.x], s_tot[threadIdx.x]);
+}
+__global__ void __launch_bounds__(256) k_slab_ov_ranges(uint32_t nbl, uint64_t first, const uint64_t* __restrict__ ov_off, uint64_t* __restrict__ beg1,
+                                                        uint64_t* __restrict__ end1) {
+    const uint32_t b = blockIdx.x * blockDim.x + threadIdx.x;
+    if (b < nbl) { beg1[b] = first + ov_off[b]; end1[b] = first + ov_off[b + 1]; }
+}
+
+static uint32_t slab_cap_for(uint64_t M, uint32_t NB) {
+    const uint64_t per = NB ? M / NB : 0;
+    return (uint32_t)std::min<uint64_t>(((per + 8) / 9 + 7) & ~7ull, 1u << 20) + 8;
+}
+
+int count_partition_slab(Ctx& c, uint32_t nb, uint32_t cap, bool* took, unsigned* n_seg, uint64_t** d_ranges) {
+    *took = false; *n_seg = 1; *d_ranges = nullptr;
+    const uint32_t nbl = nb;
+    if (!c.quality_done) { c.err = "partition before quality_windows"; return W2RAP_E_STATE; }
+    hipStream_t st = c.stream;
+    const uint64_t n = c.n;
+    if (n >= (1ull << 32)) { c.err = "more than 2^32 reads on one GPU (32-bit read ids in the record descriptors)"; return W2RAP_E_LIMIT; }
+    const bool trace = getenv("W2RAP_TRACE") != nullptr;
+    uint32_t spp, npass;
+    k1_slots(c, &spp, &npass);
+    const uint64_t slab_recs = (uint64_t)nbl * cap;
+    uint64_t rec_cap = slab_recs + slab_recs / 32 + 4096;
+    if (c.d_recs) { c.release(c.d_recs); c.d_recs = nullptr; }
+    {
+        size_t free_b = 0, total_b = 0, parked_b = 0;
+        for (auto& b : c.parked) parked_b += b.first;
+        const bool known = hipMemGetInfo(&free_b, &total_b) == hipSuccess;
+        if (!known) (void)hipGetLastError();
+        const bool fits = known && (double)rec_cap * REC_BYTES <= ((double)free_b + (double)parked_b) / 4.0;
+        const std::string keep = c.err;
+        uint32_t* slab = test_hook("W2RAP_TEST_SLAB_NOALLOC") || !fits ? nullptr : c.alloc<uint32_t>(rec_cap * REC_DWORDS);
+        if (!slab) {
+            if (trace) fprintf(stderr, "[w2rap] partition route: batched (no room for %llu slab records of %u buckets x %u)\n", (unsigned long long)rec_cap, nbl, cap);
+            c.err = keep;
+            return 0;
+        }
+        c.d_recs = slab;
+    }
+    *took = true;
+    c.NB = nb;
+    if (c.d_bcount) c.release(c.d_bcount);
+    if (c.d_bbase) { c.release(c.d_bbase); c.d_bbase = nullptr; }
+    W2_ALLOC(c.d_bcount, uint32_t, nbl);
+    unsigned long long* d_cur = nullptr;
+    W2_ALLOC(d_cur, unsigned long long, 4);
+    uint64_t* rng = nullptr;
+    W2_ALLOC(rng, uint64_t, 4 * (uint64_t)nbl);
+    uint32_t* ov_cnt = nullptr;
+    W2_ALLOC(ov_cnt, uint32_t, nbl);
+    uint64_t* beg = rng; uint64_t* end = rng + 2 * (uint64_t)nbl;
+    uint32_t *o_read = nullptr, *o_bkt = nullptr, *o_meta = nullptr, *o_rank = nullptr;
+    uint64_t ov_cap = n / 4 + 1024;
+    W2_ALLOC(o_read, uint32_t, ov_cap); W2_ALLOC(o_bkt, uint32_t, ov_cap); W2_ALLOC(o_meta, uint32_t, ov_cap); W2_ALLOC(o_rank, uint32_t, ov_cap);
+    uint64_t bases_bytes = 0;
+    if (n) W2_HIP(hipMemcpy(&bases_bytes, c.d_boff + n, 8, hipMemcpyDeviceToHost));
+    unsigned long long h_cur[4] = {0, 0, 0, 0};
+    uint64_t nov = 0;
+    for (;;) {
+        W2_HIP(hipMemsetAsync(c.d_bcount, 0, (size_t)nbl * 4, st));
+        W2_HIP(hipMemsetAsync(d_cur, 0, 32, st));
+        if (n) W2_TRY(launch_k1(c, n, c.d_boff, c.d_good, 0u, nb, c.d_bcount, 0u, 0u, nullptr, nullptr, spp, npass, nullptr, o_read, o_bkt, o_meta, o_rank, ov_cap, d_cur,
+                                cap, c.d_recs, bases_bytes));
+        LAUNCH(c, "k_slab_ranges", k_slab_ranges, dim3((nbl + 255) / 256), dim3(256), 0, nbl, cap, c.d_bcount, beg, end, ov_cnt, d_cur + 1);
+        W2_HIP(hipGetLastError());
+        W2_HIP(hipMemcpyAsync(h_cur, d_cur, 32, hipMemcpyDeviceToHost, st));
+        W2_HIP(hipStreamSynchronize(st));
+        nov = h_cur[0];
+        if (nov <= ov_cap) break;
+        if (trace) fprintf(stderr, "[w2rap] partition slab: %llu list entries for a list of %llu, K1 again\n", (unsigned long long)nov, (unsigned long long)ov_cap);
+        for (uint32_t* q : {o_read, o_bkt, o_meta, o_rank}) c.release(q);
+        ov_cap = nov + nov / 8 + 1024;
+        W2_ALLOC(o_read, uint32_t, ov_cap); W2_ALLOC(o_bkt, uint32_t, ov_cap); W2_ALLOC(o_meta, uint32_t, ov_cap); W2_ALLOC(o_rank, uint32_t, ov_cap);
+    }
+    c.nrec = h_cur[2];
+    const uint64_t n_beyond = h_cur[3];
+    if (nov) {
+        if (slab_recs + n_beyond > rec_cap) {
+            rec_cap = slab_recs + n_beyond;
+            uint32_t* bigger = c.alloc<uint32_t>(rec_cap * REC_DWORDS);
+            if (!bigger) return W2RAP_E_HIP;
+            W2_HIP(hipMemcpyAsync(bigger, c.d_recs, slab_recs * REC_BYTES, hipMemcpyDeviceToDevice, st));
+            W2_HIP(hipStreamSynchronize(st));
+            c.release(c.d_recs);
+            c.d_recs = bigger;
+        }
+        uint64_t* ov_off = nullptr;
+        W2_ALLOC(ov_off, uint64_t, (uint64_t)nbl + 1);
+        W2_TRY(exclusive_scan_u32_to_u64(c, ov_cnt, ov_off, nbl));
+        LAUNCH(c, "k_slab_ov_ranges", k_slab_ov_ranges, dim3((nbl + 255) / 256), dim3(256), 0, nbl, slab_recs, ov_off, beg + nbl, end + nbl);
+        W2_HIP(hipGetLastError());
+        LAUNCH(c, "k_scatter_records", k_scatter_records<false>, dim3((unsigned)((nov + 255) / 256)), dim3(256), 0, (uint64_t)0, npass * spp, nullptr, (uint64_t)0,
+               nullptr, nov, o_read, o_bkt, o_meta, o_rank, c.d_bases, c.d_boff, bases_bytes, beg + nbl, c.d_recs, cap);
+        W2_HIP(hipGetLastError());
+        W2_HIP(hipStreamSynchronize(st));
+        c.release(ov_off);
+    }
+    *n_seg = n_beyond ? 2 : 1;
+    if (trace) fprintf(stderr, "[w2rap] partition route: slab, cap %u, %u buckets, %llu records, largest bucket %llu, nov %llu, %llu beyond their slabs, nseg %u\n", cap, nbl,
+                       (unsigned long long)c.nrec, (unsigned long long)h_cur[1], (unsigned long long)nov, (unsigned long long)n_beyond, *n_seg);
+    c.release(d_cur); c.release(ov_cnt); c.release(o_read); c.release(o_bkt); c.release(o_meta); c.release(o_rank);
+    *d_ranges = rng;
+    return 0;
+}
+
 static void table_geometry(uint64_t S, uint64_t& tcap) {
     const char* lf = getenv("W2RAP_TABLE_X");
     const uint64_t mult10 = lf ? 10 * (uint64_t)atoll(lf) : (S < (1ull << 30) ? 40 : 13);
@@ -1944,7 +2123,7 @@
 }
 
 int count_buckets_launch(Ctx& c, uint32_t min_freq, uint32_t nbl, uint32_t nseg, const uint32_t* d_recs, const uint32_t* d_counts,
-                         uint64_t total_kmers, unsigned NS, bool deferred) {
+                         uint64_t total_kmers, unsigned NS, bool deferred, const uint64_t* d_beg, const uint64_t* d_end) {
     hipStream_t st = c.stream;
     if (c.cs_planned) { c.err = "count_records_begin: a sliced count is already pending"; return W2RAP_E_STATE; }
     c.min_freq = min_freq;
@@ -1954,8 +2133,12 @@
     if (nseg > 64) { c.err = "count_records: more than 64 segments"; return W2RAP_E_LIMIT; }
     const uint64_t nflat = (uint64_t)nbl * nseg;
     uint64_t* d_off = nullptr;
-    W2_ALLOC(d_off, uint64_t, nflat + 1);
-    W2_TRY(exclusive_scan_u32_to_u64(c, d_counts, d_off, nflat));
+    if (!d_beg != !d_end || !d_beg == !d_counts) { c.err = "count_records: bucket counts or record ranges, one of the two"; return W2RAP_E_ARG; }
+    if (!d_beg) {
+        W2_ALLOC(d_off, uint64_t, nflat + 1);
+        W2_TRY(exclusive_scan_u32_to_u64(c, d_counts, d_off, nflat));
+        d_beg = d_off; d_end = d_off + 1;
+    }
     unsigned long long* d_cnt = c.pass ? c.pass_cnt : nullptr;
     uint32_t chunk_cap = c.pass ? c.cs_chunk_cap : 0;
     if (!c.pass) {
@@ -1976,7 +2159,7 @@
             W2_HIP(hipMemsetAsync(c.d_chunk_cnt, 0, (size_t)chunk_cap * 4, st));
         }
     }
-    c.cs_cnt = d_cnt; c.cs_off = d_off; c.cs_chunk_cap = chunk_cap;
+    c.cs_cnt = d_cnt; c.cs_off = d_off; c.cs_beg = d_beg; c.cs_end = d_end; c.cs_chunk_cap = chunk_cap;
     W2_ALLOC(c.cs_defer, uint32_t, (uint64_t)nbl + 2);
     c.cs_planned = NS; c.cs_ns = 0; c.cs_nbl = nbl; c.cs_nseg = nseg; c.cs_recs = d_recs;
     c.cs_short_first = deferred && NS >= 3;
@@ -2016,7 +2199,7 @@
         W2_HIP(hipFuncSetAttribute(reinterpret_cast<const void*>(kern), hipFuncAttributeMaxDynamicSharedMemorySize, lds));
         unsigned grid = (unsigned)std::min<uint64_t>(b_hi - b_lo, (uint64_t)c.sm_count * blocks_per_cu);
         if (k || c.pass) W2_HIP(hipMemsetAsync(d_queue, 0, 4, st));
-        LAUNCH(c, "k_count_buckets", kern, dim3(grid ? grid : 1), dim3(threads), lds, nbl, b_lo, b_hi, nseg, c.cs_off, c.cs_recs, c.min_freq, d_queue,
+        LAUNCH(c, "k_count_buckets", kern, dim3(grid ? grid : 1), dim3(threads), lds, nbl, b_lo, b_hi, nseg, c.cs_beg, c.cs_end, c.cs_recs, c.min_freq, d_queue,
                c.d_shi, c.d_slo, c.d_scc, c.solid_cap, d_cnt + 4, d_cnt + 8, c.d_chunk_start, c.d_chunk_cnt, c.cs_chunk_cap, (const uint32_t*)nullptr, 0u);
         W2_HIP(hipGetLastError());
         return slice_done();
@@ -2031,7 +2214,7 @@
         uint32_t fill_limit = fp_limit, solid_limit = fp_sc;
         if (const char* t = getenv("W2RAP_TEST_FP_LIMIT")) { if (test_hook("W2RAP_TEST_FP_LIMIT")) fill_limit = std::min<uint32_t>(fill_limit, (uint32_t)std::max(1, atoi(t))); }
         if (const char* t = getenv("W2RAP_TEST_FP_SC")) { if (test_hook("W2RAP_TEST_FP_SC")) solid_limit = std::min<uint32_t>(solid_limit, (uint32_t)std::max(1, atoi(t))); }
-        LAUNCH(c, "k_count_fp", kern, dim3(grid ? grid : 1), dim3(threads), lds, nbl, b_lo, b_hi, nseg, c.cs_off, c.cs_recs, c.min_freq, d_queue,
+        LAUNCH(c, "k_count_fp", kern, dim3(grid ? grid : 1), dim3(threads), lds, nbl, b_lo, b_hi, nseg, c.cs_beg, c.cs_end, c.cs_recs, c.min_freq, d_queue,
                c.d_shi, c.d_slo, c.d_scc, c.solid_cap, d_cnt + 4, d_cnt + 8, c.d_chunk_start, c.d_chunk_cnt, c.cs_chunk_cap, c.cs_defer, nbl, fill_limit, solid_limit,
                c.fused_prune ? c.d_sctx : (uint8_t*)nullptr, c.fused_prune ? c.d_unres : (uint8_t*)nullptr, c.fused_prune ? (uint32_t*)c.d_nbr : (uint32_t*)nullptr);
         W2_HIP(hipGetLastError());
@@ -2039,7 +2222,7 @@
         if (k + 1 == NS) {
             const unsigned lgrid = (unsigned)std::min<uint64_t>(nbl, (uint64_t)c.sm_count);
             constexpr unsigned list_lds = K3Cfg<COUNT_CAP, COUNT_THREADS>::LDS;
-            LAUNCH(c, "k_count_buckets", list_kern, dim3(lgrid ? lgrid : 1), dim3(COUNT_THREADS), list_lds, nbl, 0u, nbl, nseg, c.cs_off,
+            LAUNCH(c, "k_count_buckets", list_kern, dim3(lgrid ? lgrid : 1), dim3(COUNT_THREADS), list_lds, nbl, 0u, nbl, nseg, c.cs_beg, c.cs_end,
                    c.cs_recs, c.min_freq, c.cs_defer + 1, c.d_shi, c.d_slo, c.d_scc, c.solid_cap, d_cnt + 4, d_cnt + 8, c.d_chunk_start, c.d_chunk_cnt, c.cs_chunk_cap,
                    (const uint32_t*)c.cs_defer, nbl);
             W2_HIP(hipGetLastError());
@@ -2083,7 +2266,7 @@
     c.cs_ns = 0; c.cs_planned = 0;
     if (c.pass + 1 < c.npass) c.pass_cnt = c.cs_cnt;
     else { c.release(c.cs_cnt); c.pass_cnt = nullptr; c.pass = 0; c.npass = 1; }
-    c.release(c.cs_off); c.cs_cnt = nullptr; c.cs_off = nullptr;
+    c.release(c.cs_off); c.cs_cnt = nullptr; c.cs_off = nullptr; c.cs_beg = nullptr; c.cs_end = nullptr;
     if (getenv("W2RAP_TRACE") && c.cs_defer) {
         uint32_t nd = 0;
         (void)hipMemcpy(&nd, c.cs_defer, 4, hipMemcpyDeviceToHost);
@@ -2121,7 +2304,7 @@
 }
 
 int count_buckets(Ctx& c, uint32_t min_freq, uint32_t nbl, uint32_t nseg, const uint32_t* d_recs, const uint32_t* d_counts,
-                  uint64_t total_kmers, bool build_table) {
+                  uint64_t total_kmers, bool build_table, const uint64_t* d_beg, const uint64_t* d_end) {
     hipStream_t st2 = c.stream2;
     const char* nsv = getenv("W2RAP_SLICES");
     unsigned NS = (build_table && !getenv("W2RAP_NO_OVERLAP") && nbl >= 4096 && st2) ? (nsv ? (unsigned)atoi(nsv) : 4) : 1;
@@ -2139,7 +2322,7 @@
             W2_HIP(hipMemsetAsync(c.d_unres, 0xFF, cap, c.stream));
         }
     }
-    W2_TRY(count_buckets_launch(c, min_freq, nbl, nseg, d_recs, d_counts, total_kmers, NS, false));
+    W2_TRY(count_buckets_launch(c, min_freq, nbl, nseg, d_recs, d_counts, total_kmers, NS, false, d_beg, d_end));
     NS = c.cs_ns;
     uint64_t s_cap = 0;
     if (NS > 1) {
@@ -2386,9 +2569,23 @@
         unsigned nseg = 1;
         c.pass = p;
         double a = now();
-        W2_TRY(count_partition_batched(c, NB, bv ? (unsigned)atoi(bv) : 4, &nseg, lo, hi));
+        const char* rv = getenv("W2RAP_PARTITION");
+        uint32_t spp_, npass_;
+        k1_slots(c, &spp_, &npass_);
+        bool slab = P == 1 && !k1_wave(spp_, npass_) && !(rv && !strcmp(rv, "batched")) && (W2RAP_SLAB_DEFAULT || (rv && !strcmp(rv, "slab")));
+        uint32_t cap = slab_cap_for(c.M, NB);
+        if (const char* t = getenv("W2RAP_TEST_SLAB_CAP")) { if (test_hook("W2RAP_TEST_SLAB_CAP")) cap = (uint32_t)std::max(1, atoi(t)); }
+        if ((uint64_t)NB * cap >= (1ull << 40)) slab = false;
+        uint64_t* ranges = nullptr;
+        if (slab) W2_TRY(count_partition_slab(c, NB, cap, &slab, &nseg, &ranges));
+        if (!slab) {
+            if (trace) fprintf(stderr, "[w2rap] partition route: batched\n");
+            W2_TRY(count_partition_batched(c, NB, bv ? (unsigned)atoi(bv) : 4, &nseg, lo, hi));
+        }
         double b = now();
-        W2_TRY(count_buckets(c, min_freq, hi - lo, nseg, c.d_recs, c.d_bcount, c.M, P == 1));
+        if (slab) W2_TRY(count_buckets(c, min_freq, NB, nseg, c.d_recs, nullptr, c.M, true, ranges, ranges + 2 * (uint64_t)NB));
+        else W2_TRY(count_buckets(c, min_freq, hi - lo, nseg, c.d_recs, c.d_bcount, c.M, P == 1));
+        if (ranges) c.release(ranges);
         c.release(c.d_recs); c.d_recs = nullptr;
         t_part += b - a; t_cnt += now() - b;
     }
```

Result: no change. 41.99 billion, median of 6 (+1.7%).
